# idiap/IdiapTTS

Measured on AMD Instinct MI355X. Metric: acoustic frames/sec (train), higher is better.
Workload: dtype f32

## Files before the change

### idiaptts_amd/csrc/context.h

```cpp
#pragma once
#include <cstdint>
#include <map>
#include <tuple>

#include "common.h"

namespace itts {

struct FreqtTables {
  double* fwdT = nullptr;
  double* invT = nullptr;
  double* frqT = nullptr;
  double* specT = nullptr;
  double* crT = nullptr;
  double* specP = nullptr;
  double* crP = nullptr;
  double* initP = nullptr;
  int kpad = 0;
  double* initT = nullptr;
  double* b1T = nullptr;
  double* p2T = nullptr;
  int m = 0, f2 = 0;
  double alpha = 0;
};

constexpr int RNG_CHUNK = 64;
constexpr int RNG_NJUMP = 26;
constexpr int RNG_TABLE_LOG2 = 20;
struct JumpTable {
  uint32_t col[RNG_NJUMP][128][4];
  uint4* states;
};

__device__ __forceinline__ uint4 rng_chunk_state(const JumpTable* __restrict__ jt, int64_t chunk) {
  uint4 st = jt->states[chunk & ((1 << RNG_TABLE_LOG2) - 1)];
  for (int k = RNG_TABLE_LOG2; k < RNG_NJUMP; ++k) {
    if ((chunk >> k) & 1) {
      const uint32_t s[4] = {st.x, st.y, st.z, st.w};
      uint32_t r0 = 0, r1 = 0, r2 = 0, r3 = 0;
      for (int j = 0; j < 128; ++j) {
        if ((s[j >> 5] >> (j & 31)) & 1u) {
          r0 ^= jt->col[k][j][0];
          r1 ^= jt->col[k][j][1];
          r2 ^= jt->col[k][j][2];
          r3 ^= jt->col[k][j][3];
        }
      }
      st = make_uint4(r0, r1, r2, r3);
    }
  }
  return st;
}

struct DeviceContext {
  int device = -1;
  double2* twiddles = nullptr;
  double2* tw_compact[16] = {nullptr};
  JumpTable* jump = nullptr;
  int64_t* pinned = nullptr;
  std::map<std::tuple<int, int, long long>, FreqtTables> freqt;
};

DeviceContext* get_context();
const FreqtTables* get_freqt(DeviceContext* ctx, int m, int f2, double alpha, bool need_fwd_frq,
                             bool need_mgc = false, bool need_spec = false);

int launch_gemm_f64_mgc2sp(const double* A, int64_t lda, const double* B, int64_t ldb, int64_t T, int N, int K,
                           float* o32, double* o64, double* opow, hipStream_t s);

const JumpTable* get_jump_table(DeviceContext* ctx);
int launch_randn_u32(DeviceContext* ctx, const int64_t* d_off, const int64_t* d_len, int n_utts,
                     int64_t max_len, uint32_t* d_R, hipStream_t s);

int launch_gemm_f64(const double* A, int64_t lda, const double* B, int64_t ldb, double* C, int64_t ldc,
                    int64_t T, int N, int K, const int* rows, hipStream_t s, bool a_has_slack = true);

int64_t* pinned_slot(DeviceContext* ctx);

int staged_upload(void* d_dst, const void* src, size_t bytes, hipStream_t s);

struct PinnedTable {
  void* p = nullptr;
  void* slot = nullptr;
};
int pinned_table_begin(const void* src, size_t bytes, PinnedTable* t);
int pinned_table_end(PinnedTable* t, hipStream_t s);

int upload_i64(const int64_t* h, int n, int64_t** d_out, hipStream_t s);

}
```

### idiaptts_amd/csrc/context.hip

```cpp
#include <cstdlib>

#include "context.h"

#include <algorithm>
#include <atomic>
#include <cmath>
#include <cstring>
#include <mutex>
#include <vector>

#include "world_dev.h"

namespace itts {

static std::mutex g_ctx_mutex;
static std::map<int, DeviceContext*> g_contexts;

static int create_context(DeviceContext* ctx) {
  const int n = wd::TW_N / 2;
  std::vector<double2> tw(n);
  for (int k = 0; k < n; ++k) {
    const long double a = 2.0L * 3.141592653589793238462643383279502884L * k / wd::TW_N;
    tw[k] = make_double2((double)cosl(a), (double)sinl(a));
  }
  ITTS_HIP_CHECK(hipMalloc((void**)&ctx->twiddles, n * sizeof(double2)));
  ITTS_HIP_CHECK(hipMemcpy(ctx->twiddles, tw.data(), n * sizeof(double2), hipMemcpyHostToDevice));
  for (int L = 5; (1 << L) <= wd::TW_N; ++L) {
    const int m = (1 << L) / 2, stride = wd::TW_N / (1 << L);
    std::vector<double2> c(m);
    for (int k = 0; k < m; ++k) c[k] = tw[(size_t)k * stride];
    ITTS_HIP_CHECK(hipMalloc((void**)&ctx->tw_compact[L], m * sizeof(double2)));
    ITTS_HIP_CHECK(hipMemcpy(ctx->tw_compact[L], c.data(), m * sizeof(double2), hipMemcpyHostToDevice));
  }
  ITTS_HIP_CHECK(hipHostMalloc((void**)&ctx->pinned, 64 * sizeof(int64_t), hipHostMallocDefault));
  return ITTS_OK;
}


}


namespace itts {

struct ScratchBlock {
  void* p;
  size_t bytes;
  hipEvent_t ev;
  hipStream_t last;
  bool busy;
};
struct ScratchCache {
  std::vector<ScratchBlock> blocks;
  size_t total = 0;
};
static std::mutex g_scratch_mutex;
static std::map<int, ScratchCache> g_scratch;

static size_t scratch_class(size_t n) {
  if (n <= ((size_t)1 << 20)) {
    size_t c = 256;
    while (c < n) c <<= 1;
    return c;
  }
  const size_t g = (size_t)2 << 20;
  return (n + g - 1) / g * g;
}

static size_t scratch_keep_bytes() {
  static const size_t keep = [] {
    size_t gb = 64;
    if (const char* e = getenv("ITTS_POOL_KEEP_GB")) gb = strtoull(e, nullptr, 10);
    return gb << 30;
  }();
  return keep;
}

static void scratch_evict(ScratchCache& c, size_t limit) {
  while (c.total > limit) {
    int pick = -1;
    for (int i = 0; i < (int)c.blocks.size(); ++i)
      if (!c.blocks[i].busy && (pick < 0 || c.blocks[i].bytes > c.blocks[pick].bytes)) pick = i;
    if (pick < 0) return;
    ScratchBlock b = c.blocks[pick];
    (void)hipEventSynchronize(b.ev);
    (void)hipFree(b.p);
    (void)hipEventDestroy(b.ev);
    c.total -= b.bytes;
    c.blocks.erase(c.blocks.begin() + pick);
  }
}

static thread_local ScratchScope* t_scope = nullptr;

ScratchScope::ScratchScope(hipStream_t s) : stream_(s), prev_(t_scope) { t_scope = this; }
ScratchScope::~ScratchScope() {
  t_scope = prev_;
  for (int i = 0; i < n_live_; ++i)
    if (live_[i]) (void)scratch_free(live_[i], stream_);
}
void ScratchScope::track(void* p) {
  if (n_live_ < 64) live_[n_live_++] = p;
}
void ScratchScope::untrack(void* p) {
  for (int i = n_live_ - 1; i >= 0; --i)
    if (live_[i] == p) {
      live_[i] = nullptr;
      while (n_live_ > 0 && live_[n_live_ - 1] == nullptr) --n_live_;
      return;
    }
  if (prev_) prev_->untrack(p);
}

static hipError_t scratch_malloc_impl(void** out, size_t bytes, hipStream_t s);
hipError_t scratch_malloc(void** out, size_t bytes, hipStream_t s) {
  const hipError_t e = scratch_malloc_impl(out, bytes, s);
  if (e == hipSuccess && *out && t_scope) t_scope->track(*out);
  return e;
}

static hipError_t scratch_malloc_impl(void** out, size_t bytes, hipStream_t s) {
  *out = nullptr;
  int dev = -1;
  hipError_t e = hipGetDevice(&dev);
  if (e != hipSuccess) return e;
  const size_t want = scratch_class(bytes);
  std::lock_guard<std::mutex> lock(g_scratch_mutex);
  ScratchCache& c = g_scratch[dev];
  int best = -1;
  for (int i = 0; i < (int)c.blocks.size(); ++i) {
    const ScratchBlock& b = c.blocks[i];
    if (b.busy || b.bytes < want) continue;
    if (want <= ((size_t)1 << 20) ? b.bytes != want : b.bytes > want + want / 4 + ((size_t)4 << 20)) continue;
    if (best < 0 || b.bytes < c.blocks[best].bytes) best = i;
  }
  if (best >= 0) {
    ScratchBlock& b = c.blocks[best];
    if (b.last != s && (e = hipStreamWaitEvent(s, b.ev, 0)) != hipSuccess) return e;
    b.busy = true;
    *out = b.p;
    return hipSuccess;
  }
  void* p = nullptr;
  e = hipMalloc(&p, want);
  if (e != hipSuccess) {
    (void)hipGetLastError();
    scratch_evict(c, 0);
    if ((e = hipMalloc(&p, want)) != hipSuccess) return e;
  }
  hipEvent_t ev;
  if ((e = hipEventCreateWithFlags(&ev, hipEventDisableTiming)) != hipSuccess) {
    (void)hipFree(p);
    return e;
  }
  c.blocks.push_back(ScratchBlock{p, want, ev, s, true});
  c.total += want;
  if (c.total > scratch_keep_bytes()) scratch_evict(c, scratch_keep_bytes());
  *out = p;
  return hipSuccess;
}

hipError_t scratch_free(void* p, hipStream_t s) {
  if (!p) return hipSuccess;
  if (t_scope) t_scope->untrack(p);
  std::lock_guard<std::mutex> lock(g_scratch_mutex);
  for (auto& kv : g_scratch)
    for (ScratchBlock& b : kv.second.blocks)
      if (b.p == p) {
        const hipError_t e = hipEventRecord(b.ev, s);
        b.last = s;
        b.busy = false;
        return e;
      }
  return hipErrorInvalidValue;
}

}

extern "C" int itts_scratch_pool_stats(int64_t* reserved, int64_t* used, int64_t* keep_threshold) {
  int dev = -1;
  ITTS_HIP_CHECK(hipGetDevice(&dev));
  size_t r = 0, u = 0;
  {
    std::lock_guard<std::mutex> lock(itts::g_scratch_mutex);
    auto it = itts::g_scratch.find(dev);
    if (it != itts::g_scratch.end())
      for (const itts::ScratchBlock& b : it->second.blocks) {
        r += b.bytes;
        if (b.busy) u += b.bytes;
      }
  }
  if (reserved) *reserved = (int64_t)r;
  if (used) *used = (int64_t)u;
  if (keep_threshold) *keep_threshold = (int64_t)itts::scratch_keep_bytes();
  return ITTS_OK;
}

extern "C" int itts_release_scratch(void) {
  int dev = -1;
  ITTS_HIP_CHECK(hipGetDevice(&dev));
  ITTS_HIP_CHECK(hipDeviceSynchronize());
  {
    std::lock_guard<std::mutex> lock(itts::g_scratch_mutex);
    auto it = itts::g_scratch.find(dev);
    if (it != itts::g_scratch.end()) itts::scratch_evict(it->second, 0);
  }
  return ITTS_OK;
}

namespace itts {

int64_t* pinned_slot(DeviceContext* ctx) {
  static std::atomic<unsigned> next{0};
  return ctx->pinned + (next.fetch_add(1) & 63u);
}

DeviceContext* get_context() {
  int dev = -1;
  if (hipGetDevice(&dev) != hipSuccess) {
    set_error("hipGetDevice failed: no HIP device (there is no CPU fallback)");
    return nullptr;
  }
  std::lock_guard<std::mutex> lock(g_ctx_mutex);
  auto it = g_contexts.find(dev);
  if (it != g_contexts.end()) return it->second;
  DeviceContext* ctx = new DeviceContext();
  ctx->device = dev;
  if (create_context(ctx) != ITTS_OK) {
    delete ctx;
    return nullptr;
  }
  g_contexts[dev] = ctx;
  return ctx;
}

struct Mat128 {
  uint32_t col[128][4];
};
static void mat_apply(const Mat128& m, const uint32_t* v, uint32_t* out) {
  uint32_t r[4] = {0, 0, 0, 0};
  for (int j = 0; j < 128; ++j)
    if ((v[j >> 5] >> (j & 31)) & 1u)
      for (int c = 0; c < 4; ++c) r[c] ^= m.col[j][c];
  std::memcpy(out, r, sizeof(r));
}
static void mat_mul(const Mat128& a, const Mat128& b, Mat128* out) {
  Mat128 r;
  for (int j = 0; j < 128; ++j) mat_apply(a, b.col[j], r.col[j]);
  *out = r;
}

__global__ __launch_bounds__(256) void rng_states_kernel(const JumpTable* __restrict__ jt) {
  const int chunk = blockIdx.x * 256 + threadIdx.x;
  uint32_t s[4] = {123456789u, 362436069u, 521288629u, 88675123u};
  for (int k = 0; k < RNG_TABLE_LOG2; ++k) {
    if ((chunk >> k) & 1) {
      uint32_t r0 = 0, r1 = 0, r2 = 0, r3 = 0;
      for (int j = 0; j < 128; ++j) {
        if ((s[j >> 5] >> (j & 31)) & 1u) {
          r0 ^= jt->col[k][j][0];
          r1 ^= jt->col[k][j][1];
          r2 ^= jt->col[k][j][2];
          r3 ^= jt->col[k][j][3];
        }
      }
      s[0] = r0; s[1] = r1; s[2] = r2; s[3] = r3;
    }
  }
  jt->states[chunk] = make_uint4(s[0], s[1], s[2], s[3]);
}

const JumpTable* get_jump_table(DeviceContext* ctx) {
  std::lock_guard<std::mutex> lock(g_ctx_mutex);
  if (ctx->jump) return ctx->jump;
  Mat128 step;
  for (int j = 0; j < 128; ++j) {
    uint32_t s[4] = {0, 0, 0, 0};
    s[j >> 5] = 1u << (j & 31);
    uint32_t x = s[0], y = s[1], z = s[2], w = s[3];
    const uint32_t t = x ^ (x << 11);
    x = y; y = z; z = w;
    w = (w ^ (w >> 19)) ^ (t ^ (t >> 8));
    step.col[j][0] = x; step.col[j][1] = y; step.col[j][2] = z; step.col[j][3] = w;
  }
  Mat128 B, pw = step;
  bool have = false;
  for (int e = 12 * RNG_CHUNK; e > 0; e >>= 1) {
    if (e & 1) {
      if (!have) { B = pw; have = true; } else mat_mul(pw, B, &B);
    }
    mat_mul(pw, pw, &pw);
  }
  std::vector<JumpTable> jt(1);
  Mat128 cur = B;
  for (int k = 0; k < RNG_NJUMP; ++k) {
    std::memcpy(jt[0].col[k], cur.col, sizeof(cur.col));
    mat_mul(cur, cur, &cur);
  }
  JumpTable* d = nullptr;
  uint4* states = nullptr;
  const int n_states = 1 << RNG_TABLE_LOG2;
  if (hipMalloc((void**)&states, sizeof(uint4) * n_states) != hipSuccess ||
      hipMalloc((void**)&d, sizeof(JumpTable)) != hipSuccess) {
    set_error("could not create the RNG jump table");
    return nullptr;
  }
  jt[0].states = states;
  if (hipMemcpy(d, jt.data(), sizeof(JumpTable), hipMemcpyHostToDevice) != hipSuccess) {
    set_error("could not create the RNG jump table");
    return nullptr;
  }
  hipLaunchKernelGGL(rng_states_kernel, dim3(n_states / 256), dim3(256), 0, 0, d);
  if (hipGetLastError() != hipSuccess || hipStreamSynchronize(0) != hipSuccess) {
    set_error("could not tabulate the RNG states");
    return nullptr;
  }
  ctx->jump = d;
  return d;
}

__global__ __launch_bounds__(256) void randn_u32_direct_kernel(const int64_t* __restrict__ off,
                                                               const int64_t* __restrict__ len,
                                                               const JumpTable* __restrict__ jt,
                                                               uint32_t* __restrict__ R) {
  const int u = blockIdx.y;
  const int64_t chunk = (int64_t)blockIdx.x * 256 + threadIdx.x;
  const int64_t n0 = chunk * RNG_CHUNK;
  const int64_t n = len[u];
  if (n0 >= n) return;
  const uint4 st = rng_chunk_state(jt, chunk);
  uint32_t x = st.x, y = st.y, z = st.z, w = st.w;
  uint32_t* out = R + off[u] + n0;
  const int cnt = (int)(n - n0 < RNG_CHUNK ? n - n0 : RNG_CHUNK);
  for (int i = 0; i < cnt; ++i) {
    uint32_t tmp = 0;
    for (int q = 0; q < 12; ++q) {
      const uint32_t t = x ^ (x << 11);
      x = y; y = z; z = w;
      w = (w ^ (w >> 19)) ^ (t ^ (t >> 8));
      tmp += w >> 4;
    }
    out[i] = tmp;
  }
}

__global__ __launch_bounds__(256) void randn_u32_kernel(const int64_t* __restrict__ off,
                                                        const int64_t* __restrict__ len,
                                                        const JumpTable* __restrict__ jt,
                                                        uint32_t* __restrict__ R) {
  constexpr int HALF = RNG_CHUNK / 2;
  __shared__ uint32_t tile[4][64 * (HALF + 1)];
  const int u = blockIdx.y;
  const int lane = threadIdx.x & 63, wv = threadIdx.x >> 6;
  const int64_t chunk0 = (int64_t)blockIdx.x * 256 + wv * 64;
  const int64_t n = len[u];
  if ((int64_t)blockIdx.x * 256 * RNG_CHUNK >= n) return;
  const int64_t chunk = chunk0 + lane;
  const bool live = chunk * RNG_CHUNK < n;
  uint32_t x = 0, y = 0, z = 0, w = 0;
  if (live) {
    const uint4 st = rng_chunk_state(jt, chunk);
    x = st.x; y = st.y; z = st.z; w = st.w;
  }
  uint32_t* t = tile[wv];
  uint32_t* out = R + off[u] + chunk0 * RNG_CHUNK;
  const int64_t rem = n - chunk0 * RNG_CHUNK;
  for (int h = 0; h < 2; ++h) {
    if (live) {
#pragma unroll 4
      for (int i = 0; i < HALF; ++i) {
        uint32_t tmp = 0;
        for (int q = 0; q < 12; ++q) {
          const uint32_t s = x ^ (x << 11);
          x = y; y = z; z = w;
          w = (w ^ (w >> 19)) ^ (s ^ (s >> 8));
          tmp += w >> 4;
        }
        t[lane * (HALF + 1) + i] = tmp;
      }
    }
    __syncthreads();
    const int col = lane & (HALF - 1), sub = lane / HALF;
    for (int r = 0; r < 64; r += 64 / HALF) {
      const int row = r + sub;
      const int64_t idx = (int64_t)row * RNG_CHUNK + h * HALF + col;
      if (idx < rem) out[idx] = t[row * (HALF + 1) + col];
    }
    __syncthreads();
  }
}

int launch_randn_u32(DeviceContext* ctx, const int64_t* d_off, const int64_t* d_len, int n_utts,
                     int64_t max_len, uint32_t* d_R, hipStream_t s) {
  const JumpTable* jt = get_jump_table(ctx);
  if (!jt) return ITTS_E_HIP;
  ITTS_REQUIRE(max_len < ((int64_t)RNG_CHUNK << RNG_NJUMP), "utterance too long for the RNG jump table");
  if (n_utts == 0 || max_len <= 0) return ITTS_OK;
  const int64_t chunks = (max_len + RNG_CHUNK - 1) / RNG_CHUNK;
  const char* direct = std::getenv("ITTS_RANDN_DIRECT");
  const dim3 grid((unsigned)((chunks + 255) / 256), n_utts);
  if (direct && direct[0] == '1')
    hipLaunchKernelGGL(randn_u32_direct_kernel, grid, dim3(256), 0, s, d_off, d_len, jt, d_R);
  else
    hipLaunchKernelGGL(randn_u32_kernel, grid, dim3(256), 0, s, d_off, d_len, jt, d_R);
  ITTS_LAUNCH_CHECK();
  return ITTS_OK;
}

static void freqt_unit(int idx, int m2, double a, double* g, double* d) {
  const double b = 1.0 - a * a;
  std::memset(g, 0, sizeof(double) * (m2 + 1));
  std::memset(d, 0, sizeof(double) * (m2 + 1));
  for (int i = -idx; i <= 0; ++i) {
    const double cin = (i == -idx) ? 1.0 : 0.0;
    d[0] = g[0];
    g[0] = cin + a * d[0];
    if (m2 >= 1) {
      d[1] = g[1];
      g[1] = b * d[0] + a * d[1];
    }
    for (int j = 2; j <= m2; ++j) {
      d[j] = g[j];
      g[j] = d[j - 1] + a * (d[j] - g[j - 1]);
    }
  }
}

static void frqtr_unit(int idx, int m2, double a, double* g, double* d) {
  std::memset(g, 0, sizeof(double) * (m2 + 1));
  std::memset(d, 0, sizeof(double) * (m2 + 1));
  for (int i = -idx; i <= 0; ++i) {
    const double cin = (i == -idx) ? 1.0 : 0.0;
    d[0] = g[0];
    g[0] = cin;
    for (int j = 1; j <= m2; ++j) {
      d[j] = g[j];
      g[j] = d[j - 1] + a * (d[j] - g[j - 1]);
    }
  }
}

static void b2c_unit(int idx, int m2, double a, double* g, double* d) {
  const double k = 1.0 - a * a;
  std::memset(g, 0, sizeof(double) * (m2 + 1));
  std::memset(d, 0, sizeof(double) * (m2 + 1));
  for (int i = -idx; i <= 0; ++i) {
    const double cin = (i == -idx) ? 1.0 : 0.0;
    d[0] = g[0];
    g[0] = cin;
    if (m2 >= 1) {
      d[1] = g[1];
      g[1] = k * d[0] + a * d[1];
    }
    for (int j = 2; j <= m2; ++j) {
      d[j] = g[j];
      g[j] = d[j - 1] + a * (d[j] - g[j - 1]);
    }
  }
}

static int upload(const std::vector<double>& h, double** d) {
  ITTS_HIP_CHECK(hipMalloc((void**)d, h.size() * sizeof(double)));
  ITTS_HIP_CHECK(hipMemcpy(*d, h.data(), h.size() * sizeof(double), hipMemcpyHostToDevice));
  return ITTS_OK;
}

const FreqtTables* get_freqt(DeviceContext* ctx, int m, int f2, double alpha, bool need_fwd_frq,
                             bool need_mgc, bool need_spec) {
  long long abits;
  std::memcpy(&abits, &alpha, sizeof(abits));
  const auto key = std::make_tuple(m, f2, abits);
  std::lock_guard<std::mutex> lock(g_ctx_mutex);
  FreqtTables& t = ctx->freqt[key];
  t.m = m;
  t.f2 = f2;
  t.alpha = alpha;
  const int m2 = 2 * m;
  std::vector<double> g(std::max(f2, m2) + 2), d(std::max(f2, m2) + 2);
  if (!t.invT) {
    std::vector<double> inv((size_t)(m + 1) * (f2 + 1));
    for (int j = 0; j <= m; ++j) {
      freqt_unit(j, f2, -alpha, g.data(), d.data());
      for (int i = 0; i <= f2; ++i) inv[(size_t)j * (f2 + 1) + i] = g[i];
    }
    if (upload(inv, &t.invT) != ITTS_OK) return nullptr;
  }
  if (need_fwd_frq && !t.fwdT) {
    std::vector<double> fwd((size_t)(f2 + 1) * (m + 1)), frq((size_t)(f2 + 1) * (m2 + 1));
    for (int i = 0; i <= f2; ++i) {
      freqt_unit(i, m, alpha, g.data(), d.data());
      for (int j = 0; j <= m; ++j) fwd[(size_t)i * (m + 1) + j] = g[j];
      frqtr_unit(i, m2, alpha, g.data(), d.data());
      for (int j = 0; j <= m2; ++j) frq[(size_t)i * (m2 + 1) + j] = g[j];
    }
    if (upload(fwd, &t.fwdT) != ITTS_OK) return nullptr;
    if (upload(frq, &t.frqT) != ITTS_OK) return nullptr;
    const int nfft = 2 * f2;
    std::vector<long double> cs(nfft);
    for (int i = 0; i < nfft; ++i) cs[i] = cosl(2.0L * 3.14159265358979323846264338327950288L * i / nfft);
    std::vector<double> crt((size_t)(f2 + 1) * (m2 + 1));
    std::vector<long double> accj(m2 + 1);
    for (int k = 0; k <= f2; ++k) {
      const long double wk = (k == 0 || k == f2) ? 1.0L : 2.0L;
      std::fill(accj.begin(), accj.end(), 0.0L);
      for (int n = 0; n <= f2; ++n) {
        const long double c = cs[(size_t)((int64_t)k * n % nfft)];
        const double* fr = frq.data() + (size_t)n * (m2 + 1);
        for (int j = 0; j <= m2; ++j) accj[j] += c * (long double)fr[j];
      }
      for (int j = 0; j <= m2; ++j) crt[(size_t)k * (m2 + 1) + j] = (double)(accj[j] * wk / nfft);
    }
    if (upload(crt, &t.crT) != ITTS_OK) return nullptr;
    if (m <= 63) {
      t.kpad = (f2 + 1 + 63) / 64 * 64;
      std::vector<double> crp((size_t)t.kpad * 128, 0.0);
      for (int k = 0; k <= f2; ++k)
        for (int j = 0; j <= m2; ++j) crp[(size_t)k * 128 + j] = crt[(size_t)k * (m2 + 1) + j];
      if (upload(crp, &t.crP) != ITTS_OK) return nullptr;
    }
    std::vector<double> ini((size_t)(f2 + 1) * (m + 1));
    std::vector<long double> accm(m + 1);
    for (int k = 0; k <= f2; ++k) {
      const long double wk = (k == 0 || k == f2) ? 1.0L : 2.0L;
      std::fill(accm.begin(), accm.end(), 0.0L);
      for (int n = 0; n <= f2; ++n) {
        const long double c = cs[(size_t)((int64_t)k * n % nfft)] * ((n == 0 || n == f2) ? 0.5L : 1.0L);
        const double* fw = fwd.data() + (size_t)n * (m + 1);
        for (int j = 0; j <= m; ++j) accm[j] += c * (long double)fw[j];
      }
      for (int j = 0; j <= m; ++j) ini[(size_t)k * (m + 1) + j] = (double)(accm[j] * wk / nfft);
    }
    if (upload(ini, &t.initT) != ITTS_OK) return nullptr;
    if (m <= 63) {
      const int kpad = (f2 + 1 + 63) / 64 * 64;
      std::vector<double> ip((size_t)kpad * 64, 0.0);
      for (int k = 0; k <= f2; ++k)
// ... 162 lines not shown
```

### idiaptts_amd/csrc/nn.hip

```cpp
#include <algorithm>
#include <atomic>
#include <cstdlib>

#include "common.h"
#include "gemm_ring.h"
#include "gemm_staged.h"

namespace itts {

constexpr int BN = 128;

template <bool ROWFORM, bool VEC, int NROWS>
__device__ __forceinline__ void load_tile(const float* __restrict__ P, int64_t ld, int64_t out0,
                                          int64_t out_dim, int64_t k0, int64_t k_end,
                                          float4 (&r)[NROWS / 32]) {
  const int tid = threadIdx.x;
#pragma unroll
  for (int i = 0; i < NROWS / 32; ++i) {
    const int idx = tid + 256 * i;
    int64_t o, k;
    if (ROWFORM) {
      o = out0 + (idx >> 3);
      k = k0 + ((idx & 7) << 2);
    } else {
      k = k0 + idx / (NROWS / 4);
      o = out0 + ((idx % (NROWS / 4)) << 2);
    }
    const int64_t c = ROWFORM ? k : o, c_end = ROWFORM ? k_end : out_dim;
    const int64_t t = ROWFORM ? o : k, t_end = ROWFORM ? out_dim : k_end;
    const bool t_ok = t < t_end;
    const int64_t tc = t_ok ? t : 0;
    if (VEC) {
      const bool ok = t_ok && (c < c_end);
      const float4 v = *reinterpret_cast<const float4*>(P + tc * ld + (ok ? c : 0));
      r[i] = ok ? v : make_float4(0.f, 0.f, 0.f, 0.f);
    } else {
      const float* row = P + tc * ld;
      const bool k0ok = t_ok && c < c_end, k1ok = t_ok && c + 1 < c_end, k2ok = t_ok && c + 2 < c_end,
                 k3ok = t_ok && c + 3 < c_end;
      const float a0 = row[k0ok ? c : 0], a1 = row[k1ok ? c + 1 : 0], a2 = row[k2ok ? c + 2 : 0],
                  a3 = row[k3ok ? c + 3 : 0];
      r[i] = make_float4(k0ok ? a0 : 0.f, k1ok ? a1 : 0.f, k2ok ? a2 : 0.f, k3ok ? a3 : 0.f);
    }
  }
}

template <bool A_ROW, bool B_ROW, bool VEC_A, bool VEC_B>
struct DenseLoader {
  const GemmArgs& g;
  template <int NROWS>
  __device__ __forceinline__ void load_a(int64_t out0, int64_t k0, int64_t k_end, float4 (&r)[NROWS / 32]) const {
    load_tile<A_ROW, VEC_A, NROWS>(g.A, g.lda, out0, g.M, k0, k_end, r);
  }
  template <int NROWS>
  __device__ __forceinline__ void load_b(int64_t out0, int64_t k0, int64_t k_end, float4 (&r)[NROWS / 32]) const {
    load_tile<B_ROW, VEC_B, NROWS>(g.B, g.ldb, out0, g.N, k0, k_end, r);
  }
};

template <bool A_ROW, bool B_ROW, int EPI, bool VEC_A, bool VEC_B, int TN, int STAGES = 2, int AF = AF_BASE>
__global__ __launch_bounds__(256, STAGES == 1 ? 4 : 2) void gemm_f32_kernel(GemmArgs g) {
  __shared__ __attribute__((aligned(16))) float lds[staged_lds_floats<B_ROW, TN, STAGES>()];
  f32x16 acc[2][TN];
  const StagedTile t =
      staged_gemm_tile<A_ROW, B_ROW, TN, STAGES>(g, DenseLoader<A_ROW, B_ROW, VEC_A, VEC_B>{g}, lds, acc);
  const int64_t m0 = t.m0;
  const int n0 = t.n0;
  const int lane = threadIdx.x & 63, wid = threadIdx.x >> 6;
  const int wm = wid >> 1, wn = wid & 1;
  float* C = g.C + (int64_t)blockIdx.z * g.slab_stride;
  const int cl = lane & 31, rh = lane >> 5;
  if (EPI == EPI_MSE) {
    float* stage = lds + wid * (32 * 36);
    const int c4 = (lane & 7) << 2, rq = lane >> 3;
    const int colb = n0 + wn * 32;
    double lsum = 0.0;
#pragma unroll
    for (int i = 0; i < 2; ++i) {
      if (i > 0) {
        __builtin_amdgcn_fence(__ATOMIC_RELEASE, "wavefront");
        __builtin_amdgcn_wave_barrier();
      }
#pragma unroll
      for (int r = 0; r < 16; ++r) stage[((r & 3) + 8 * (r >> 2) + 4 * rh) * 36 + cl] = acc[i][0][r];
      __builtin_amdgcn_fence(__ATOMIC_RELEASE, "wavefront");
      __builtin_amdgcn_wave_barrier();
      __builtin_amdgcn_fence(__ATOMIC_ACQUIRE, "wavefront");
      const int col = colb + c4;
#pragma unroll
      for (int q = 0; q < 4; ++q) {
        const int rl = rq + 8 * q;
        const int64_t row = m0 + wm * 64 + i * 32 + rl;
        const float4 v = *reinterpret_cast<const float4*>(stage + rl * 36 + c4);
        if (row >= g.M || col >= g.N) continue;
        const bool ok = g.row_valid[row] != 0;
        const float vv[4] = {v.x, v.y, v.z, v.w};
        float dz[4];
#pragma unroll
        for (int e = 0; e < 4; ++e) {
          float diff = 0.f;
          if (col + e < g.N && ok)
            diff = (vv[e] + (g.bias ? g.bias[col + e] : 0.f)) - g.aux[row * g.ldaux + col + e];
          lsum += (double)diff * (double)diff;
          dz[e] = g.gscale * diff;
        }
        if (col + 3 < g.N) {
          *reinterpret_cast<float4*>(C + row * g.ldc + col) = make_float4(dz[0], dz[1], dz[2], dz[3]);
        } else {
          for (int e = 0; e < 4 && col + e < g.N; ++e) C[row * g.ldc + col + e] = dz[e];
        }
      }
    }
    __shared__ double mse_red[16];
    lsum = block_sum(lsum, mse_red);
    if (threadIdx.x == 0) g.loss_partial[blockIdx.x] = lsum;
    return;
  }
  if (STAGES == 1 && TN == 1 && g.wide_out) {
    float* stage = lds + wid * (32 * 36);
    const int c4 = (lane & 7) << 2, rq = lane >> 3;
    const int colb = n0 + wn * 32;
#pragma unroll
    for (int i = 0; i < 2; ++i) {
      if (i > 0) {
        __builtin_amdgcn_fence(__ATOMIC_RELEASE, "wavefront");
        __builtin_amdgcn_wave_barrier();
      }
#pragma unroll
      for (int r = 0; r < 16; ++r) stage[((r & 3) + 8 * (r >> 2) + 4 * rh) * 36 + cl] = acc[i][0][r];
      __builtin_amdgcn_fence(__ATOMIC_RELEASE, "wavefront");
      __builtin_amdgcn_wave_barrier();
      __builtin_amdgcn_fence(__ATOMIC_ACQUIRE, "wavefront");
      const int col = colb + c4;
      float4 bv = make_float4(0.f, 0.f, 0.f, 0.f);
      const bool full = col + 3 < g.N;
      if (EPI == EPI_BIAS_ACT && g.bias && full) bv = *reinterpret_cast<const float4*>(g.bias + col);
#pragma unroll
      for (int q = 0; q < 4; ++q) {
        const int rl = rq + 8 * q;
        const int64_t row = m0 + wm * 64 + i * 32 + rl;
        float4 v = *reinterpret_cast<const float4*>(stage + rl * 36 + c4);
        if (row >= g.M || col >= g.N) continue;
        if (full) {
          if (EPI == EPI_BIAS_ACT) {
            v.x = act_fwd_af<AF>(v.x + bv.x, g.act); v.y = act_fwd_af<AF>(v.y + bv.y, g.act);
            v.z = act_fwd_af<AF>(v.z + bv.z, g.act); v.w = act_fwd_af<AF>(v.w + bv.w, g.act);
          }
          if (EPI == EPI_DACT) {
            const float4 a = *reinterpret_cast<const float4*>(g.aux + row * g.ldaux + col);
            v.x *= act_grad_af<AF>(a.x, g.act); v.y *= act_grad_af<AF>(a.y, g.act);
            v.z *= act_grad_af<AF>(a.z, g.act); v.w *= act_grad_af<AF>(a.w, g.act);
          }
          *reinterpret_cast<float4*>(C + row * g.ldc + col) = v;
        } else {
          const float vv[4] = {v.x, v.y, v.z, v.w};
          for (int e = 0; e < 4 && col + e < g.N; ++e) {
            float o = vv[e];
            if (EPI == EPI_BIAS_ACT) o = act_fwd_af<AF>(o + (g.bias ? g.bias[col + e] : 0.f), g.act);
            if (EPI == EPI_DACT) o *= act_grad_af<AF>(g.aux[row * g.ldaux + col + e], g.act);
            C[row * g.ldc + col + e] = o;
          }
        }
      }
    }
    return;
  }
  staged_epilogue<EPI, TN, AF>(g, t, acc, [](int64_t m) { return m; });
}

static std::atomic<int64_t> g_gemm_path[2][4];

template <bool A_ROW, bool B_ROW, int EPI, int TN, int STAGES, int AF = AF_BASE>
static int launch_gemm_tn(const GemmArgs& g, int splitk, hipStream_t s) {
  g_gemm_path[1][EPI].fetch_add(1, std::memory_order_relaxed);
  const int64_t tiles = ((g.M + BM - 1) / BM) * ((g.N + 64 * TN - 1) / (64 * TN));
  dim3 grid((unsigned)tiles, 1, (unsigned)splitk);
  const bool va = g.vecA, vb = g.vecB;
  if (va && vb)
    hipLaunchKernelGGL((gemm_f32_kernel<A_ROW, B_ROW, EPI, true, true, TN, STAGES, AF>), grid, dim3(256), 0, s, g);
  else if (va)
    hipLaunchKernelGGL((gemm_f32_kernel<A_ROW, B_ROW, EPI, true, false, TN, STAGES, AF>), grid, dim3(256), 0, s, g);
  else if (vb)
    hipLaunchKernelGGL((gemm_f32_kernel<A_ROW, B_ROW, EPI, false, true, TN, STAGES, AF>), grid, dim3(256), 0, s, g);
  else
    hipLaunchKernelGGL((gemm_f32_kernel<A_ROW, B_ROW, EPI, false, false, TN, STAGES, AF>), grid, dim3(256), 0, s, g);
  ITTS_LAUNCH_CHECK();
  return ITTS_OK;
}

static double tile_efficiency(int64_t M, int N, int splitk, int tn, double loop_eff) {
  const int bn = 64 * tn;
  const int64_t tiles = ((M + BM - 1) / BM) * ((N + bn - 1) / bn) * splitk;
  const int64_t rounds = (tiles + 511) / 512;
  const double useful = (double)N / (double)(((N + bn - 1) / bn) * bn);
  return loop_eff * useful * (double)tiles / (double)(rounds * 512);
}

constexpr int kRingGrid = 512;

template <bool A_ROW, bool B_ROW>
static bool ring_ok(const GemmArgs& g, int splitk, int epi) {
  if (!g.vecA || !g.vecB) return false;
  if (g.lda % 4 || g.ldb % 4 || g.ldc % 4 || g.slab_stride % 4 || !aligned16(g.C)) return false;
  if (epi == EPI_DACT && (g.ldaux % 4 || !aligned16(g.aux))) return false;
  const int64_t lim = (int64_t)1 << 30;
  if (g.M >= lim || g.K >= lim || g.lda >= lim / 256 || g.ldb >= lim / 256 || g.ldc >= lim / 256 ||
      g.ldaux >= lim / 256)
    return false;
  if (!A_ROW && (g.kchunk + 32) * g.lda >= lim) return false;
  if (!B_ROW && (g.kchunk + 32) * g.ldb >= lim) return false;
  if (splitk > 1 && g.kchunk % 32) return false;
  return true;
}

static int ring_group(int tiles_n, int bnt, int64_t K, bool row_row);

template <int WM>
static ring::Args ring_args(const GemmArgs& g, int splitk) {
  constexpr int BMT = 64 * WM, BNT = 32 * (4 / WM);
  ring::Args r{};
  r.A = g.A; r.B = g.B; r.C = g.C; r.bias = g.bias; r.aux = g.aux;
  r.row_valid = g.row_valid; r.loss_partial = g.loss_partial; r.bias_part = g.bias_part;
  r.slab_stride = g.slab_stride; r.bias_part_stride = g.bias_part_stride;
  r.lda = (int)g.lda; r.ldb = (int)g.ldb; r.ldc = (int)g.ldc; r.ldaux = (int)g.ldaux;
  r.M = (int)g.M; r.N = g.N; r.K = (int)g.K; r.kchunk = (int)g.kchunk; r.splitk = splitk;
  r.tiles_m = (int)((g.M + BMT - 1) / BMT);
  r.tiles_n = (g.N + BNT - 1) / BNT;
  r.gn = r.tiles_n;
  r.act = g.act; r.gscale = g.gscale;
  return r;
}

template <bool A_ROW, bool B_ROW, int EPI, int WM, int AF = AF_BASE>
static int launch_ring_wm(const GemmArgs& g, int splitk, hipStream_t s) {
  constexpr int BNT = 32 * (4 / WM);
  g_gemm_path[0][EPI].fetch_add(1, std::memory_order_relaxed);
  ring::Args r = ring_args<WM>(g, splitk);
  r.gn = ring_group(r.tiles_n, BNT, g.K, A_ROW && B_ROW);
  const int64_t ntiles = (int64_t)r.tiles_m * r.tiles_n * splitk;
  ITTS_REQUIRE(ntiles < ((int64_t)1 << 31), "too many tiles");
  const int grid = (int)std::min<int64_t>(kRingGrid, (ntiles + 7) / 8 * 8);
  if (A_ROW && B_ROW && EPI == ring::EPI_BIAS_ACT && r.gn < r.tiles_n)
    hipLaunchKernelGGL((ring::gemm_ring_kernel<A_ROW, B_ROW, EPI, WM, A_ROW && B_ROW && EPI == ring::EPI_BIAS_ACT, AF>),
                       dim3(grid), dim3(ring::THREADS), 0, s, r);
  else
    hipLaunchKernelGGL((ring::gemm_ring_kernel<A_ROW, B_ROW, EPI, WM, false, AF>), dim3(grid), dim3(ring::THREADS), 0, s, r);
  ITTS_LAUNCH_CHECK();
  return ITTS_OK;
}

static int ring_group(int tiles_n, int bnt, int64_t K, bool row_row) {
  if (!row_row) return tiles_n;
  const int64_t panel = (int64_t)bnt * K * 4;
  const int64_t gn = std::max<int64_t>(1, ((int64_t)4 << 20) / std::max<int64_t>(panel, 1));
  return (int)std::min<int64_t>(gn, tiles_n);
}

static int ring_wm(int64_t M, int N) {
  const double w2 = (double)(((M + 127) / 128) * 128) * (double)(((N + 63) / 64) * 64);
  const double w1 = (double)(((M + 63) / 64) * 64) * (double)(((N + 127) / 128) * 128);
  return w1 < w2 ? 1 : 2;
}

template <bool A_ROW, bool B_ROW, int EPI, int AF>
static int launch_ring(const GemmArgs& g, int splitk, hipStream_t s) {
  if (ring_wm(g.M, g.N) == 1) return launch_ring_wm<A_ROW, B_ROW, EPI, 1, AF>(g, splitk, s);
  return launch_ring_wm<A_ROW, B_ROW, EPI, 2, AF>(g, splitk, s);
}

template <int WM_W, int EPI_X, int AF_X = AF_BASE>
static int launch_ring_bwd_pair(const GemmArgs& gw, int splitk, const GemmArgs& gx, hipStream_t s) {
  g_gemm_path[0][EPI_STORE].fetch_add(1, std::memory_order_relaxed);
  g_gemm_path[0][EPI_X].fetch_add(1, std::memory_order_relaxed);
  const ring::Args rw = ring_args<WM_W>(gw, splitk), rx = ring_args<2>(gx, 1);
  hipLaunchKernelGGL((ring::gemm_ring_pair_kernel<false, false, EPI_STORE, WM_W, true, false, EPI_X, 2, AF_X>),
                     dim3(kRingGrid), dim3(ring::THREADS), 0, s, rw, rx);
  ITTS_LAUNCH_CHECK();
  return ITTS_OK;
}

template <bool A_ROW, bool B_ROW, int EPI, int AF = AF_BASE>
static int launch_gemm(GemmArgs g, int splitk, hipStream_t s) {
  if (g.M <= 0 || g.N <= 0) return ITTS_OK;
  if (ring_ok<A_ROW, B_ROW>(g, splitk, EPI)) return launch_ring<A_ROW, B_ROW, EPI, AF>(g, splitk, s);
  if (A_ROW) return launch_gemm_tn<A_ROW, B_ROW, EPI, 1, 1, AF>(g, splitk, s);
  const double e2 = tile_efficiency(g.M, g.N, splitk, 2, 1.0);
  const double e1 = tile_efficiency(g.M, g.N, splitk, 1, 0.90);
  if (e1 > e2) return launch_gemm_tn<A_ROW, B_ROW, EPI, 1, 2, AF>(g, splitk, s);
  return launch_gemm_tn<A_ROW, B_ROW, EPI, 2, 2, AF>(g, splitk, s);
}


__device__ __forceinline__ void reduce_slabs_vec_body(const float* __restrict__ slabs, int S, int64_t n,
                                                      float* __restrict__ out, int accumulate, int64_t block,
                                                      float4 (*part)[64]) {
  const int tx = threadIdx.x & 63, grp = threadIdx.x >> 6;
  const int64_t n4 = n >> 2;
  const int64_t c = block * 64 + tx;
  float4 s = make_float4(0.f, 0.f, 0.f, 0.f);
  if (c < n4) {
    const float4* p = reinterpret_cast<const float4*>(slabs) + c;
#pragma unroll 8
    for (int z = grp; z < S; z += 4) {
      const float4 v = p[(int64_t)z * n4];
      s.x += v.x; s.y += v.y; s.z += v.z; s.w += v.w;
    }
  }
  if (grp > 0) part[grp - 1][tx] = s;
  __syncthreads();
  if (grp == 0 && c < n4) {
#pragma unroll
    for (int g2 = 0; g2 < 3; ++g2) {
      const float4 v = part[g2][tx];
      s.x += v.x; s.y += v.y; s.z += v.z; s.w += v.w;
    }
    float4* o = reinterpret_cast<float4*>(out) + c;
    if (accumulate) {
      const float4 v = *o;
      s.x += v.x; s.y += v.y; s.z += v.z; s.w += v.w;
    }
    *o = s;
  }
}

__device__ __forceinline__ void reduce_slabs_scalar_body(const float* __restrict__ slabs, int S, int64_t n,
                                                         float* __restrict__ out, int accumulate,
                                                         int64_t block, float (*part)[64]) {
  const int tx = threadIdx.x & 63, grp = threadIdx.x >> 6;
  const int64_t c = block * 64 + tx;
  float s = 0.f;
  if (c < n) {
#pragma unroll 8
    for (int z = grp; z < S; z += 4) s += slabs[(int64_t)z * n + c];
  }
  if (grp > 0) part[grp - 1][tx] = s;
  __syncthreads();
  if (grp == 0 && c < n) {
    s += part[0][tx];
    s += part[1][tx];
    s += part[2][tx];
    out[c] = accumulate ? out[c] + s : s;
  }
}

__global__ __launch_bounds__(256) void reduce_slabs_kernel(const float* __restrict__ slabs, int S,
                                                           int64_t n, float* __restrict__ out,
                                                           int accumulate) {
  __shared__ float4 part[3][64];
  reduce_slabs_vec_body(slabs, S, n, out, accumulate, blockIdx.x, part);
}

__global__ __launch_bounds__(256) void reduce_slabs_scalar_kernel(const float* __restrict__ slabs, int S,
                                                                  int64_t n, float* __restrict__ out,
                                                                  int accumulate) {
  __shared__ float part[3][64];
  reduce_slabs_scalar_body(slabs, S, n, out, accumulate, blockIdx.x, part);
}

constexpr int kMaxDeferred = 16;
struct ReduceSeg {
  const void* src;
  void* out;
  int64_t n;
  double scale;
  int S;
  int accumulate;
  int kind;
  int first_block;
};
struct ReduceMulti {
  ReduceSeg seg[kMaxDeferred];
  int nseg;
};

__global__ __launch_bounds__(256) void reduce_multi_kernel(ReduceMulti d) {
  __shared__ float4 part4[3][64];
  __shared__ double red[16];
  int i = 0;
  while (i + 1 < d.nseg && (int)blockIdx.x >= d.seg[i + 1].first_block) ++i;
  const ReduceSeg& g = d.seg[i];
  const int64_t block = (int64_t)blockIdx.x - g.first_block;
  if (g.kind == 0) {
    reduce_slabs_vec_body(static_cast<const float*>(g.src), g.S, g.n, static_cast<float*>(g.out), g.accumulate,
                          block, part4);
  } else if (g.kind == 1) {
    reduce_slabs_scalar_body(static_cast<const float*>(g.src), g.S, g.n, static_cast<float*>(g.out),
                             g.accumulate, block, reinterpret_cast<float (*)[64]>(part4));
  } else {
    const double* partial = static_cast<const double*>(g.src);
    double s = 0.0;
    for (int k = threadIdx.x; k < (int)g.n; k += 256) s += partial[k];
    s = block_sum(s, red);
    if (threadIdx.x == 0) *static_cast<float*>(g.out) = (float)(s * g.scale);
  }
}

static thread_local bool t_defer = false;
static thread_local ReduceMulti t_pending{};

static int flush_deferred(hipStream_t s) {
  if (t_pending.nseg == 0) return ITTS_OK;
  const ReduceSeg& last = t_pending.seg[t_pending.nseg - 1];
  const int64_t per = last.kind == 0 ? (last.n / 4 + 63) / 64 : (last.kind == 1 ? (last.n + 63) / 64 : 1);
  const int64_t blocks = last.first_block + per;
  hipLaunchKernelGGL(reduce_multi_kernel, dim3((unsigned)blocks), dim3(256), 0, s, t_pending);
  t_pending.nseg = 0;
  ITTS_LAUNCH_CHECK();
  return ITTS_OK;
}

static int queue_deferred(ReduceSeg g, hipStream_t s) {
  if (t_pending.nseg == kMaxDeferred) {
    const int rc = flush_deferred(s);
    if (rc) return rc;
  }
  int64_t first = 0;
  if (t_pending.nseg > 0) {
    const ReduceSeg& p = t_pending.seg[t_pending.nseg - 1];
    first = p.first_block + (p.kind == 0 ? (p.n / 4 + 63) / 64 : (p.kind == 1 ? (p.n + 63) / 64 : 1));
  }
  ITTS_REQUIRE(first < ((int64_t)1 << 30), "too many deferred reduction blocks");
  g.first_block = (int)first;
  t_pending.seg[t_pending.nseg++] = g;
  return ITTS_OK;
}

static int launch_reduce_slabs(const float* slabs, int S, int64_t n, float* out, int accumulate,
                               hipStream_t s) {
  const bool vec = n % 4 == 0 && aligned16(slabs) && aligned16(out);
  if (t_defer) {
    ReduceSeg g{};
    g.src = slabs; g.out = out; g.n = n; g.S = S; g.accumulate = accumulate; g.kind = vec ? 0 : 1;
    return queue_deferred(g, s);
  }
  if (vec)
    hipLaunchKernelGGL(reduce_slabs_kernel, dim3((unsigned)((n / 4 + 63) / 64)), dim3(256), 0, s, slabs, S,
                       n, out, accumulate);
  else
    hipLaunchKernelGGL(reduce_slabs_scalar_kernel, dim3((unsigned)((n + 63) / 64)), dim3(256), 0, s, slabs,
                       S, n, out, accumulate);
  ITTS_LAUNCH_CHECK();
  return ITTS_OK;
}

extern "C" int itts_defer_reductions(int on) {
  ITTS_REQUIRE(on || t_pending.nseg == 0,
               "queued reductions must be run (itts_reduce_deferred) before deferral is switched off");
  t_defer = on != 0;
  return ITTS_OK;
}

extern "C" int itts_reduce_deferred(void* stream) {
  t_defer = false;
  return flush_deferred(as_stream(stream));
}

template <int AF>
__global__ void act_bwd_kernel(const float* __restrict__ dy, const float* __restrict__ y,
                               float* __restrict__ dz, int64_t n, int act) {
  if (AF == AF_BASE) {
    for (int64_t i = blockIdx.x * (int64_t)blockDim.x + threadIdx.x; i < n;
         i += (int64_t)gridDim.x * blockDim.x)
      dz[i] = dy[i] * act_grad_from_out(y[i], act);
  } else {
    with_ext_act(act, [&](auto a) {
      for (int64_t i = blockIdx.x * (int64_t)blockDim.x + threadIdx.x; i < n;
           i += (int64_t)gridDim.x * blockDim.x)
        dz[i] = dy[i] * dact1<decltype(a)::value>(y[i]);
    });
  }
}

__global__ __launch_bounds__(256) void masked_mse_kernel(
    const float* __restrict__ pred, int64_t ldp, const float* __restrict__ target, int64_t ldt,
    const uint8_t* __restrict__ valid, int64_t M, int D, float gscale, float* __restrict__ grad,
    int64_t ldg, double* __restrict__ partial) {
  __shared__ double red[16];
  const int64_t n = M * D;
  double s = 0.0;
  for (int64_t i = blockIdx.x * (int64_t)blockDim.x + threadIdx.x; i < n;
       i += (int64_t)gridDim.x * blockDim.x) {
    const int64_t r = i / D;
    const int c = (int)(i - r * D);
    float diff = 0.f;
    if (valid[r]) diff = pred[r * ldp + c] - target[r * ldt + c];
    s += (double)diff * (double)diff;
    if (grad) grad[r * ldg + c] = gscale * diff;
  }
  s = block_sum(s, red);
  if (threadIdx.x == 0) partial[blockIdx.x] = s;
}

__global__ __launch_bounds__(256) void masked_mse_final_kernel(const double* __restrict__ partial,
                                                               int nb, double scale,
                                                               float* __restrict__ loss) {
  __shared__ double red[16];
  double s = 0.0;
  for (int i = threadIdx.x; i < nb; i += 256) s += partial[i];
  s = block_sum(s, red);
  if (threadIdx.x == 0) *loss = (float)(s * scale);
}

static int launch_mse_final(const double* partial, int nb, double scale, float* loss, hipStream_t s) {
  if (t_defer) {
    ReduceSeg g{};
    g.src = partial; g.out = loss; g.n = nb; g.scale = scale; g.S = 1; g.kind = 2;
    return queue_deferred(g, s);
  }
  hipLaunchKernelGGL(masked_mse_final_kernel, dim3(1), dim3(256), 0, s, partial, nb, scale, loss);
  ITTS_LAUNCH_CHECK();
  return ITTS_OK;
}


__global__ __launch_bounds__(256) void weighted_loss_kernel(
    const float* __restrict__ pred, int64_t ldp, const float* __restrict__ target, int64_t ldt,
    const float* __restrict__ w, int64_t M, int D, int kind, float* __restrict__ grad, int64_t ldg,
    float* __restrict__ elem, int64_t lde, double* __restrict__ partial) {
  __shared__ double red[16];
  const int64_t n = M * D;
  double s = 0.0;
  for (int64_t i = blockIdx.x * (int64_t)blockDim.x + threadIdx.x; i < n;
       i += (int64_t)gridDim.x * blockDim.x) {
    const int64_t r = i / D;
    const int c = (int)(i - r * D);
    const float wr = w[r];
    const float diff = pred[r * ldp + c] - target[r * ldt + c];
    const float e = kind == 0 ? diff * diff : fabsf(diff);
    const float g = kind == 0 ? 2.f * diff : (diff > 0.f ? 1.f : (diff < 0.f ? -1.f : 0.f));
    const float v = wr == 0.f ? 0.f : wr * e;
    s += (double)v;
    if (grad) grad[r * ldg + c] = wr == 0.f ? 0.f : wr * g;
    if (elem) elem[r * lde + c] = v;
  }
  s = block_sum(s, red);
  if (threadIdx.x == 0) partial[blockIdx.x] = s;
}

__global__ void adam_kernel(float* __restrict__ p, const float* __restrict__ g,
                            float* __restrict__ m, float* __restrict__ v, int64_t n, float beta1,
                            float beta2, float eps, float wd, float step_size, float bc2_sqrt,
                            float gscale) {
  for (int64_t i = blockIdx.x * (int64_t)blockDim.x + threadIdx.x; i < n;
       i += (int64_t)gridDim.x * blockDim.x) {
    float gi = g[i] * gscale;
    float pi = p[i];
    if (wd != 0.f) gi += wd * pi;
    float mi = m[i], vi = v[i];
    mi = mi + (gi - mi) * (1.f - beta1);
    vi = vi * beta2 + (1.f - beta2) * gi * gi;
    const float denom = sqrtf(vi) / bc2_sqrt + eps;
    pi = pi - step_size * (mi / denom);
    p[i] = pi;
    m[i] = mi;
    v[i] = vi;
  }
}

__global__ void adam_fused_kernel(float* __restrict__ p, const float* __restrict__ g,
                                  float* __restrict__ m, float* __restrict__ v, int64_t n,
                                  float beta1, float beta2, float eps, float wd, float step_size,
                                  float bc2_sqrt, float gscale, const float* __restrict__ norm_accum,
                                  int norm_kind, float max_norm, float clip_value,
                                  float* __restrict__ shadow, float one_minus_decay) {
  float coef = gscale;
  if (norm_accum) {
    const float a = norm_accum[0];
    const float total = (norm_kind == 2 ? sqrtf(a) : a) * fabsf(gscale);
    coef *= fminf(1.f, max_norm / (total + 1e-6f));
  }
  for (int64_t i = blockIdx.x * (int64_t)blockDim.x + threadIdx.x; i < n;
       i += (int64_t)gridDim.x * blockDim.x) {
    float gi = g[i] * coef;
    if (clip_value > 0.f) gi = fminf(fmaxf(gi, -clip_value), clip_value);
    float pi = p[i];
    if (wd != 0.f) gi += wd * pi;
    float mi = m[i], vi = v[i];
    mi = mi + (gi - mi) * (1.f - beta1);
    vi = vi * beta2 + (1.f - beta2) * gi * gi;
    const float denom = sqrtf(vi) / bc2_sqrt + eps;
    pi = pi - step_size * (mi / denom);
    p[i] = pi;
    m[i] = mi;
    v[i] = vi;
    if (shadow) {
      const float si = shadow[i];
      shadow[i] = si - one_minus_decay * (si - pi);
    }
  }
}

constexpr int kNormBlocks = 1024;
__global__ __launch_bounds__(256) void grad_norm_partial_kernel(const float* __restrict__ x, int64_t n,
                                                               int kind, float* __restrict__ part) {
  __shared__ float red[4];
  float acc = 0.f;
  for (int64_t i = blockIdx.x * (int64_t)blockDim.x + threadIdx.x; i < n;
       i += (int64_t)gridDim.x * blockDim.x) {
    const float xi = x[i];
    acc = kind == 2 ? acc + xi * xi : fmaxf(acc, fabsf(xi));
  }
#pragma unroll
  for (int off = 32; off > 0; off >>= 1) {
    const float o = __shfl_xor(acc, off, 64);
    acc = kind == 2 ? acc + o : fmaxf(acc, o);
  }
  if ((threadIdx.x & 63) == 0) red[threadIdx.x >> 6] = acc;
  __syncthreads();
  if (threadIdx.x == 0)
    part[blockIdx.x] = kind == 2 ? (red[0] + red[1]) + (red[2] + red[3])
                                 : fmaxf(fmaxf(red[0], red[1]), fmaxf(red[2], red[3]));
}
__global__ __launch_bounds__(256) void grad_norm_final_kernel(const float* __restrict__ part, int nb,
                                                             int kind, float* __restrict__ out,
                                                             int accumulate) {
  __shared__ float red[4];
  float acc = 0.f;
  for (int i = threadIdx.x; i < nb; i += 256) acc = kind == 2 ? acc + part[i] : fmaxf(acc, part[i]);
#pragma unroll
  for (int off = 32; off > 0; off >>= 1) {
    const float o = __shfl_xor(acc, off, 64);
    acc = kind == 2 ? acc + o : fmaxf(acc, o);
  }
  if ((threadIdx.x & 63) == 0) red[threadIdx.x >> 6] = acc;
  __syncthreads();
  if (threadIdx.x == 0) {
    float r = kind == 2 ? (red[0] + red[1]) + (red[2] + red[3])
                        : fmaxf(fmaxf(red[0], red[1]), fmaxf(red[2], red[3]));
    if (accumulate) r = kind == 2 ? out[0] + r : fmaxf(out[0], r);
    out[0] = r;
  }
}

__global__ void sgd_kernel(float* __restrict__ p, const float* __restrict__ g,
                           float* __restrict__ buf, int64_t n, float lr, float momentum,
                           float dampening, float wd, int nesterov, int first, float gscale) {
  for (int64_t i = blockIdx.x * (int64_t)blockDim.x + threadIdx.x; i < n;
       i += (int64_t)gridDim.x * blockDim.x) {
    float gi = g[i] * gscale;
    float pi = p[i];
    if (wd != 0.f) gi += wd * pi;
    if (momentum != 0.f) {
      float bi = first ? gi : buf[i] * momentum + (1.f - dampening) * gi;
      buf[i] = bi;
      gi = nesterov ? gi + momentum * bi : bi;
    }
    p[i] = pi - lr * gi;
  }
}

__global__ void ema_kernel(float* __restrict__ shadow, const float* __restrict__ x, int64_t n,
                           float one_minus_decay) {
  for (int64_t i = blockIdx.x * (int64_t)blockDim.x + threadIdx.x; i < n;
       i += (int64_t)gridDim.x * blockDim.x) {
    const float sh = shadow[i];
    shadow[i] = sh - one_minus_decay * (sh - x[i]);
  }
}

constexpr int kColsumSlices = 256;

static int choose_splitk_ring(int64_t M, int N, int K) {
  const int wm = ring_wm(N, K);
  const int bmt = 64 * wm, bnt = 32 * (4 / wm);
  const int64_t tiles = (int64_t)((N + bmt - 1) / bmt) * ((K + bnt - 1) / bnt);
  int64_t s = std::max<int64_t>(1, kRingGrid / std::max<int64_t>(tiles, 1));
  s = std::min<int64_t>(s, std::max<int64_t>(1, (M + 255) / 256));
  return (int)std::min<int64_t>(s, 128);
}

static int choose_splitk(int64_t M, int N, int K) {
  const int64_t tiles = (int64_t)((N + BM - 1) / BM) * ((K + BN - 1) / BN);
  int64_t s = std::max<int64_t>(1, 512 / std::max<int64_t>(tiles, 1));
  const int64_t max_by_rows = std::max<int64_t>(1, (M + 511) / 512);
  s = std::min(s, max_by_rows);
  return (int)std::min<int64_t>(s, 128);
}

}

using namespace itts;

extern "C" int itts_linear_fwd(const float* d_x, int64_t ldx, const float* d_w, const float* d_b,
                               float* d_y, int64_t ldy, int64_t M, int N, int K, int act,
                               void* stream) {
  ITTS_REQUIRE(d_w && (M == 0 || (d_x && d_y)), "null pointer");
  ITTS_REQUIRE(M >= 0 && N > 0 && K > 0 && ldx >= K && ldy >= N, "bad sizes");
  ITTS_REQUIRE(act >= ITTS_ACT_NONE && act <= ITTS_ACT_HARDSIGMOID, "unknown activation");
  if (M == 0) return ITTS_OK;
  GemmArgs g{};
  g.A = d_x; g.lda = ldx; g.B = d_w; g.ldb = K; g.C = d_y; g.ldc = ldy;
  g.M = M; g.N = N; g.K = K; g.bias = d_b; g.act = act;
  g.kchunk = ((K + BK - 1) / BK) * BK; g.slab_stride = 0;
  g.vecA = (ldx % 4 == 0) && aligned16(d_x);
  g.vecB = (K % 4 == 0) && aligned16(d_w);
  g.wide_out = (ldy % 4 == 0) && aligned16(d_y) && (!d_b || aligned16(d_b));
  if (act_family(act) == AF_EXT) return launch_gemm<true, true, EPI_BIAS_ACT, AF_EXT>(g, 1, as_stream(stream));
  return launch_gemm<true, true, EPI_BIAS_ACT>(g, 1, as_stream(stream));
}

__global__ __launch_bounds__(256) void rows_gather_kernel(const float* __restrict__ src, int64_t ld_src, int64_t n_src,
                                                          const int64_t* __restrict__ idx, int64_t n_out, int width,
                                                          const float* __restrict__ fill, float* __restrict__ dst,
                                                          int64_t ld_dst, int dst_width, int vec) {
  const int lane = threadIdx.x & 63;
  const int64_t w0 = (int64_t)blockIdx.x * 4 + (threadIdx.x >> 6), wn = (int64_t)gridDim.x * 4;
  for (int64_t r = w0; r < n_out; r += wn) {
    const int64_t i = idx[r];
    const float* s = (i >= 0 && i < n_src) ? src + i * ld_src : fill;
    float* d = dst + r * ld_dst;
    if (vec) {
      const int w4 = width >> 2, d4 = dst_width >> 2;
      for (int c = lane; c < d4; c += 64) {
        float4 v = make_float4(0.f, 0.f, 0.f, 0.f);
        if (c < w4 && s) v = reinterpret_cast<const float4*>(s)[c];
        reinterpret_cast<float4*>(d)[c] = v;
      }
    } else {
      for (int c = lane; c < dst_width; c += 64) d[c] = (c < width && s) ? s[c] : 0.f;
    }
  }
}

extern "C" int itts_rows_gather_f32(const float* d_src, int64_t ld_src, int64_t n_src, const int64_t* d_idx,
                                    int64_t n_out, int width, const float* d_fill_row, float* d_dst, int64_t ld_dst,
                                    int dst_width, void* stream) {
  ITTS_REQUIRE(n_out == 0 || (d_idx && d_dst && (d_src || n_src == 0)), "null pointer");
  ITTS_REQUIRE(n_out >= 0 && n_src >= 0 && width >= 0 && dst_width >= width && ld_src >= width && ld_dst >= dst_width,
               "bad sizes");
  if (n_out == 0 || dst_width == 0) return ITTS_OK;
  const int vec = width % 4 == 0 && dst_width % 4 == 0 && ld_src % 4 == 0 && ld_dst % 4 == 0 && aligned16(d_src) &&
                  aligned16(d_dst) && (!d_fill_row || aligned16(d_fill_row));
  const unsigned grid = (unsigned)std::min<int64_t>((n_out + 3) / 4, 16384);
  hipLaunchKernelGGL(rows_gather_kernel, dim3(grid), dim3(256), 0, as_stream(stream), d_src, ld_src, n_src, d_idx, n_out,
                     width, d_fill_row, d_dst, ld_dst, dst_width, vec);
  ITTS_LAUNCH_CHECK();
  return ITTS_OK;
}

extern "C" int itts_gemm_path_counts(int64_t out[8]) {
  ITTS_REQUIRE(out != nullptr, "null pointer");
  for (int k = 0; k < 2; ++k)
    for (int e = 0; e < 4; ++e) out[4 * k + e] = g_gemm_path[k][e].load(std::memory_order_relaxed);
  return ITTS_OK;
}

extern "C" int64_t itts_linear_fwd_mse_workspace_bytes(int64_t M, int N) {
  const int64_t tiles = ((M + BM - 1) / BM) * ((N + 63) / 64);
  return std::max<int64_t>(tiles, kRingGrid) * 8;
}

extern "C" int itts_linear_fwd_mse(const float* d_x, int64_t ldx, const float* d_w, const float* d_b,
                                   const float* d_target, int64_t ldt, const uint8_t* d_row_valid,
                                   double n_valid, float loss_weight, int64_t M, int N, int K,
                                   float* d_loss, float* d_dz, int64_t lddz, void* d_workspace,
                                   void* stream) {
  ITTS_REQUIRE(d_w && d_loss && d_workspace && (M == 0 || (d_x && d_target && d_row_valid && d_dz)),
               "null pointer");
  ITTS_REQUIRE(M >= 0 && N > 0 && K > 0 && ldx >= K && ldt >= N && lddz >= N && n_valid > 0, "bad sizes");
  hipStream_t s = as_stream(stream);
  if (M == 0) {
    ITTS_HIP_CHECK(hipMemsetAsync(d_loss, 0, 4, s));
    return ITTS_OK;
  }
  ITTS_REQUIRE((ldx % 4 == 0) && aligned16(d_x) && (K % 4 == 0) && aligned16(d_w) && (lddz % 4 == 0) &&
                   aligned16(d_dz),
               "x, w and dz need 16-byte aligned rows (use itts_linear_fwd + itts_masked_mse otherwise)");
  GemmArgs g{};
  g.A = d_x; g.lda = ldx; g.B = d_w; g.ldb = K; g.C = d_dz; g.ldc = lddz;
  g.M = M; g.N = N; g.K = K; g.bias = d_b; g.act = 0;
  g.kchunk = ((K + BK - 1) / BK) * BK; g.slab_stride = 0;
  g.vecA = 1; g.vecB = 1; g.wide_out = 1;
  g.aux = d_target; g.ldaux = ldt; g.row_valid = d_row_valid;
  const double scale = (double)loss_weight / (n_valid * (double)N);
  g.gscale = (float)(2.0 * scale);
  g.loss_partial = reinterpret_cast<double*>(d_workspace);
  int64_t tiles = ((M + BM - 1) / BM) * ((N + 63) / 64);
  int rc;
  if (ring_ok<true, true>(g, 1, EPI_MSE)) {
    tiles = std::min<int64_t>(kRingGrid, (tiles + 7) / 8 * 8);
    rc = launch_ring_wm<true, true, EPI_MSE, 2>(g, 1, s);
  } else {
    rc = launch_gemm_tn<true, true, EPI_MSE, 1, 1>(g, 1, s);
  }
  if (rc) return rc;
  return launch_mse_final(reinterpret_cast<const double*>(d_workspace), (int)tiles, scale, d_loss, s);
}

extern "C" int itts_act_bwd(const float* d_dy, const float* d_y, float* d_dz, int64_t n_elem,
                            int act, void* stream) {
  ITTS_REQUIRE(d_dy && d_y && d_dz && n_elem >= 0, "bad arguments");
  ITTS_REQUIRE(act >= ITTS_ACT_NONE && act <= ITTS_ACT_HARDSIGMOID, "unknown activation");
  if (n_elem == 0) return ITTS_OK;
  const int blocks = (int)std::min<int64_t>((n_elem + 255) / 256, 4096);
  if (act_family(act) == AF_EXT)
    hipLaunchKernelGGL(act_bwd_kernel<AF_EXT>, dim3(blocks), dim3(256), 0, as_stream(stream), d_dy, d_y,
                       d_dz, n_elem, act);
  else
    hipLaunchKernelGGL(act_bwd_kernel<AF_BASE>, dim3(blocks), dim3(256), 0, as_stream(stream), d_dy, d_y,
                       d_dz, n_elem, act);
  ITTS_LAUNCH_CHECK();
  return ITTS_OK;
}

extern "C" int itts_linear_bwd_input(const float* d_dz, int64_t lddz, const float* d_w,
                                     float* d_dx, int64_t lddx, const float* d_yprev,
                                     int64_t ldyp, int act_prev, int64_t M, int N, int K,
                                     void* stream) {
  ITTS_REQUIRE(d_w && (M == 0 || (d_dz && d_dx)), "null pointer");
  ITTS_REQUIRE(M >= 0 && N > 0 && K > 0 && lddz >= N && lddx >= K, "bad sizes");
  ITTS_REQUIRE(!d_yprev || (act_prev >= ITTS_ACT_NONE && act_prev <= ITTS_ACT_HARDSIGMOID), "unknown activation");
  if (M == 0) return ITTS_OK;
  GemmArgs g{};
  g.A = d_dz; g.lda = lddz; g.B = d_w; g.ldb = K; g.C = d_dx; g.ldc = lddx;
  g.M = M; g.N = K; g.K = N; g.aux = d_yprev; g.ldaux = ldyp; g.act = act_prev;
  g.kchunk = ((N + BK - 1) / BK) * BK; g.slab_stride = 0;
  g.vecA = (lddz % 4 == 0) && aligned16(d_dz);
  g.vecB = (K % 4 == 0) && aligned16(d_w);
  g.wide_out = (lddx % 4 == 0) && aligned16(d_dx) && (!d_yprev || ((ldyp % 4 == 0) && aligned16(d_yprev)));
  if (d_yprev) {
    ITTS_REQUIRE(ldyp >= K, "ldyp too small");
    if (act_family(act_prev) == AF_EXT) return launch_gemm<true, false, EPI_DACT, AF_EXT>(g, 1, as_stream(stream));
    return launch_gemm<true, false, EPI_DACT>(g, 1, as_stream(stream));
  }
  return launch_gemm<true, false, EPI_STORE>(g, 1, as_stream(stream));
}

extern "C" int64_t itts_linear_bwd_weight_workspace_bytes(int64_t M, int N, int K) {
  if (M < 0 || N <= 0 || K <= 0) return 0;
  const int s = std::max(choose_splitk(M, N, K), choose_splitk_ring(M, N, K));
  return (int64_t)s * ((int64_t)N * K + N) * 4 + (int64_t)kColsumSlices * N * 4 + 8192;
}

extern "C" int itts_linear_bwd_weight(const float* d_dz, int64_t lddz, const float* d_x,
                                      int64_t ldx, float* d_dw, float* d_db, int64_t M, int N,
                                      int K, void* d_workspace, int accumulate, void* stream) {
  ITTS_REQUIRE(d_dw && d_workspace && (M == 0 || (d_dz && d_x)), "null pointer");
  ITTS_REQUIRE(M >= 0 && N > 0 && K > 0 && lddz >= N && ldx >= K, "bad sizes");
  hipStream_t s = as_stream(stream);
  if (M == 0) {
    if (!accumulate) {
      ITTS_HIP_CHECK(hipMemsetAsync(d_dw, 0, (size_t)N * K * 4, s));
      if (d_db) ITTS_HIP_CHECK(hipMemsetAsync(d_db, 0, (size_t)N * 4, s));
    }
    return ITTS_OK;
  }
  const bool vec_ok = (lddz % 4 == 0) && aligned16(d_dz) && (ldx % 4 == 0) && aligned16(d_x) && (K % 4 == 0);
  const int S = vec_ok ? choose_splitk_ring(M, N, K) : choose_splitk(M, N, K);
  int64_t kchunk = (M + S - 1) / S;
  kchunk = ((kchunk + BK - 1) / BK) * BK;
  const int S_eff = (int)((M + kchunk - 1) / kchunk);
  float* slabs = reinterpret_cast<float*>(d_workspace);
  GemmArgs g{};
  g.A = d_dz; g.lda = lddz; g.B = d_x; g.ldb = ldx; g.C = slabs; g.ldc = K;
  g.M = N; g.N = K; g.K = M; g.kchunk = kchunk; g.slab_stride = (int64_t)N * K;
  g.vecA = (lddz % 4 == 0) && aligned16(d_dz);
  g.vecB = (ldx % 4 == 0) && aligned16(d_x);
  const int64_t n = (int64_t)N * K;
  if (d_db) {
    const bool merged = d_db == d_dw + n && N % 4 == 0 && n % 4 == 0;
    const int64_t stride = merged ? n + N : n;
    g.slab_stride = stride;
    g.bias_part = merged ? slabs + n : slabs + (int64_t)S_eff * n;
    g.bias_part_stride = merged ? stride : N;
    int rc = launch_gemm<false, false, EPI_STORE>(g, S_eff, s);
    if (rc) return rc;
    if (merged) return launch_reduce_slabs(slabs, S_eff, n + N, d_dw, accumulate, s);
    rc = launch_reduce_slabs(slabs, S_eff, n, d_dw, accumulate, s);
    if (rc) return rc;
    return launch_reduce_slabs(g.bias_part, S_eff, (int64_t)N, d_db, accumulate, s);
  }
  int rc = launch_gemm<false, false, EPI_STORE>(g, S_eff, s);
  if (rc) return rc;
  return launch_reduce_slabs(slabs, S_eff, n, d_dw, accumulate, s);
}

extern "C" int itts_linear_bwd(const float* d_dz, int64_t lddz, const float* d_x, int64_t ldx,
                               const float* d_w, float* d_dw, float* d_db, float* d_dx, int64_t lddx,
                               const float* d_yprev, int64_t ldyp, int act_prev, int64_t M, int N, int K,
                               void* d_workspace, int accumulate, void* stream) {
  ITTS_REQUIRE(d_w && d_dw && d_workspace && (M == 0 || (d_dz && d_x && d_dx)), "null pointer");
  ITTS_REQUIRE(M >= 0 && N > 0 && K > 0 && lddz >= N && ldx >= K && lddx >= K, "bad sizes");
  ITTS_REQUIRE(!d_yprev || ldyp >= K, "ldyp too small");
  ITTS_REQUIRE(!d_yprev || (act_prev >= ITTS_ACT_NONE && act_prev <= ITTS_ACT_HARDSIGMOID), "unknown activation");
  hipStream_t s = as_stream(stream);
  const bool vec_ok = (lddz % 4 == 0) && aligned16(d_dz) && (ldx % 4 == 0) && aligned16(d_x) && (K % 4 == 0) &&
                      aligned16(d_w);
  const int64_t n = (int64_t)N * K;
  const bool merged = d_db && d_db == d_dw + n && N % 4 == 0 && n % 4 == 0;
  bool fused = vec_ok && M > 0 && (lddx % 4 == 0) && aligned16(d_dx) &&
               (!d_yprev || ((ldyp % 4 == 0) && aligned16(d_yprev)));
  GemmArgs gw{}, gx{};
  int S_eff = 1;
  if (fused) {
    const int S = choose_splitk_ring(M, N, K);
    int64_t kchunk = (M + S - 1) / S;
    kchunk = ((kchunk + BK - 1) / BK) * BK;
    S_eff = (int)((M + kchunk - 1) / kchunk);
    float* slabs = reinterpret_cast<float*>(d_workspace);
    gw.A = d_dz; gw.lda = lddz; gw.B = d_x; gw.ldb = ldx; gw.C = slabs; gw.ldc = K;
    gw.M = N; gw.N = K; gw.K = M; gw.kchunk = kchunk; gw.vecA = gw.vecB = 1;
    const int64_t stride = merged ? n + N : n;
    gw.slab_stride = stride;
    if (merged) { gw.bias_part = slabs + n; gw.bias_part_stride = stride; }
    else if (d_db) { gw.bias_part = slabs + (int64_t)S_eff * n; gw.bias_part_stride = N; }
    gx.A = d_dz; gx.lda = lddz; gx.B = d_w; gx.ldb = K; gx.C = d_dx; gx.ldc = lddx;
    gx.M = M; gx.N = K; gx.K = N; gx.aux = d_yprev; gx.ldaux = ldyp; gx.act = act_prev;
    gx.kchunk = ((N + BK - 1) / BK) * BK; gx.vecA = gx.vecB = 1;
    fused = ring_ok<false, false>(gw, S_eff, EPI_STORE) && ring_ok<true, false>(gx, 1, d_yprev ? EPI_DACT : EPI_STORE);
  }
  if (!fused) {
    int rc = itts_linear_bwd_weight(d_dz, lddz, d_x, ldx, d_dw, d_db, M, N, K, d_workspace, accumulate, stream);
    if (rc) return rc;
    return itts_linear_bwd_input(d_dz, lddz, d_w, d_dx, lddx, d_yprev, ldyp, act_prev, M, N, K, stream);
  }
  int rc;
  const int wm = ring_wm(gw.M, gw.N);
  if (d_yprev && act_family(act_prev) == AF_EXT)
    rc = wm == 1 ? launch_ring_bwd_pair<1, EPI_DACT, AF_EXT>(gw, S_eff, gx, s)
                 : launch_ring_bwd_pair<2, EPI_DACT, AF_EXT>(gw, S_eff, gx, s);
  else if (d_yprev) rc = wm == 1 ? launch_ring_bwd_pair<1, EPI_DACT>(gw, S_eff, gx, s) : launch_ring_bwd_pair<2, EPI_DACT>(gw, S_eff, gx, s);
  else rc = wm == 1 ? launch_ring_bwd_pair<1, EPI_STORE>(gw, S_eff, gx, s) : launch_ring_bwd_pair<2, EPI_STORE>(gw, S_eff, gx, s);
  if (rc) return rc;
  float* slabs = reinterpret_cast<float*>(d_workspace);
  rc = launch_reduce_slabs(slabs, S_eff, merged ? n + N : n, d_dw, accumulate, s);
  if (rc || merged || !d_db) return rc;
  return launch_reduce_slabs(slabs + (int64_t)S_eff * n, S_eff, (int64_t)N, d_db, accumulate, s);
}

static int mse_blocks(int64_t M, int D) {
  return (int)std::max<int64_t>(1, std::min<int64_t>((M * D + 255) / 256, 2048));
}

extern "C" int64_t itts_masked_mse_workspace_bytes(int64_t M, int D) {
  if (M < 0 || D <= 0) return 0;
  return (int64_t)mse_blocks(M, D) * 8;
}

extern "C" int itts_masked_mse(const float* d_pred, int64_t ldp, const float* d_target,
                               int64_t ldt, const uint8_t* d_row_valid, int64_t M, int D,
                               double n_valid, float loss_weight, float* d_loss, float* d_grad,
                               int64_t ldg, void* d_workspace, void* stream) {
  ITTS_REQUIRE(d_pred && d_target && d_row_valid && d_loss && d_workspace, "null pointer");
  ITTS_REQUIRE(M >= 0 && D > 0 && ldp >= D && ldt >= D && n_valid > 0, "bad sizes");
  ITTS_REQUIRE(!d_grad || ldg >= D, "ldg too small");
  hipStream_t s = as_stream(stream);
  if (M == 0) {
    ITTS_HIP_CHECK(hipMemsetAsync(d_loss, 0, 4, s));
    return ITTS_OK;
  }
  const int nb = mse_blocks(M, D);
  const double scale = (double)loss_weight / (n_valid * (double)D);
  hipLaunchKernelGGL(masked_mse_kernel, dim3(nb), dim3(256), 0, s, d_pred, ldp, d_target, ldt,
                     d_row_valid, M, D, (float)(2.0 * scale), d_grad, ldg,
                     reinterpret_cast<double*>(d_workspace));
  ITTS_LAUNCH_CHECK();
  return launch_mse_final(reinterpret_cast<const double*>(d_workspace), nb, scale, d_loss, s);
}

extern "C" int itts_weighted_loss(const float* d_pred, int64_t ldp, const float* d_target, int64_t ldt,
                                  const float* d_row_weight, int64_t M, int D, int kind,
                                  float* d_loss, float* d_grad, int64_t ldg, float* d_elem,
                                  int64_t lde, void* d_workspace, void* stream) {
  ITTS_REQUIRE(d_pred && d_target && d_row_weight && d_loss && d_workspace, "null pointer");
  ITTS_REQUIRE(M >= 0 && D > 0 && ldp >= D && ldt >= D && (kind == 0 || kind == 1), "bad sizes");
  ITTS_REQUIRE((!d_grad || ldg >= D) && (!d_elem || lde >= D), "leading dimension too small");
  hipStream_t s = as_stream(stream);
  if (M == 0) {
    ITTS_HIP_CHECK(hipMemsetAsync(d_loss, 0, 4, s));
    return ITTS_OK;
  }
  const int nb = mse_blocks(M, D);
  hipLaunchKernelGGL(weighted_loss_kernel, dim3(nb), dim3(256), 0, s, d_pred, ldp, d_target, ldt,
                     d_row_weight, M, D, kind, d_grad, ldg, d_elem, lde,
                     reinterpret_cast<double*>(d_workspace));
  ITTS_LAUNCH_CHECK();
  hipLaunchKernelGGL(masked_mse_final_kernel, dim3(1), dim3(256), 0, s,
                     reinterpret_cast<const double*>(d_workspace), nb, 1.0, d_loss);
  ITTS_LAUNCH_CHECK();
  return ITTS_OK;
}

extern "C" int itts_adam_step(float* d_param, const float* d_grad, float* d_exp_avg,
                              float* d_exp_avg_sq, int64_t n, float lr, float beta1, float beta2,
                              float eps, float weight_decay, int64_t step, float grad_scale,
                              void* stream) {
  ITTS_REQUIRE(d_param && d_grad && d_exp_avg && d_exp_avg_sq, "null pointer");
  ITTS_REQUIRE(n >= 0 && step >= 1, "bad sizes (step counts from 1)");
  if (n == 0) return ITTS_OK;
  const double bc1 = 1.0 - pow((double)beta1, (double)step);
  const double bc2 = 1.0 - pow((double)beta2, (double)step);
  const float step_size = (float)((double)lr / bc1);
  const float bc2_sqrt = (float)sqrt(bc2);
  const int blocks = (int)std::min<int64_t>((n + 255) / 256, 4096);
  hipLaunchKernelGGL(adam_kernel, dim3(blocks), dim3(256), 0, as_stream(stream), d_param, d_grad,
                     d_exp_avg, d_exp_avg_sq, n, beta1, beta2, eps, weight_decay, step_size,
                     bc2_sqrt, grad_scale);
  ITTS_LAUNCH_CHECK();
  return ITTS_OK;
}

extern "C" int itts_grad_norm_accum(const float* d_x, int64_t n, int norm_kind, float* d_accum,
                                    int accumulate, void* d_workspace, void* stream) {
  ITTS_REQUIRE(d_accum && d_workspace && (n == 0 || d_x), "null pointer");
  ITTS_REQUIRE(n >= 0 && (norm_kind == 2 || norm_kind == 0), "norm_kind must be 2 or 0 (infinity)");
  const int nb = (int)std::min<int64_t>((n + 255) / 256, kNormBlocks);
  hipStream_t s = as_stream(stream);
  float* part = static_cast<float*>(d_workspace);
  if (nb > 0) {
    hipLaunchKernelGGL(grad_norm_partial_kernel, dim3(nb), dim3(256), 0, s, d_x, n, norm_kind, part);
    ITTS_LAUNCH_CHECK();
  }
  hipLaunchKernelGGL(grad_norm_final_kernel, dim3(1), dim3(256), 0, s, part, nb, norm_kind, d_accum,
                     accumulate);
  ITTS_LAUNCH_CHECK();
  return ITTS_OK;
}

extern "C" int itts_adam_step_fused(float* d_param, const float* d_grad, float* d_exp_avg,
                                    float* d_exp_avg_sq, int64_t n, float lr, float beta1,
                                    float beta2, float eps, float weight_decay, int64_t step,
                                    float grad_scale, const float* d_norm_accum, int norm_kind,
                                    float clip_max_norm, float clip_value, float* d_ema_shadow,
                                    float ema_decay, void* stream) {
  ITTS_REQUIRE(d_param && d_grad && d_exp_avg && d_exp_avg_sq, "null pointer");
  ITTS_REQUIRE(n >= 0 && step >= 1, "bad sizes (step counts from 1)");
  ITTS_REQUIRE(!d_norm_accum || ((norm_kind == 2 || norm_kind == 0) && clip_max_norm > 0.f),
               "norm clipping needs norm_kind 2 or 0 and a positive max norm");
  if (n == 0) return ITTS_OK;
  const double bc1 = 1.0 - pow((double)beta1, (double)step);
  const double bc2 = 1.0 - pow((double)beta2, (double)step);
  const int blocks = (int)std::min<int64_t>((n + 255) / 256, 4096);
  hipLaunchKernelGGL(adam_fused_kernel, dim3(blocks), dim3(256), 0, as_stream(stream), d_param,
                     d_grad, d_exp_avg, d_exp_avg_sq, n, beta1, beta2, eps, weight_decay,
                     (float)(lr / bc1), (float)sqrt(bc2), grad_scale, d_norm_accum, norm_kind,
                     clip_max_norm, clip_value, d_ema_shadow, 1.f - ema_decay);
  ITTS_LAUNCH_CHECK();
  return ITTS_OK;
}

extern "C" int itts_sgd_step(float* d_param, const float* d_grad, float* d_momentum_buf, int64_t n,
                             float lr, float momentum, float dampening, float weight_decay,
                             int nesterov, int first_step, float grad_scale, void* stream) {
  ITTS_REQUIRE(d_param && d_grad, "null pointer");
  ITTS_REQUIRE(momentum == 0.f || d_momentum_buf, "momentum needs a buffer");
  ITTS_REQUIRE(n >= 0, "bad size");
  if (n == 0) return ITTS_OK;
  const int blocks = (int)std::min<int64_t>((n + 255) / 256, 4096);
  hipLaunchKernelGGL(sgd_kernel, dim3(blocks), dim3(256), 0, as_stream(stream), d_param, d_grad,
                     d_momentum_buf, n, lr, momentum, dampening, weight_decay, nesterov,
                     first_step, grad_scale);
  ITTS_LAUNCH_CHECK();
  return ITTS_OK;
}

extern "C" int itts_ema_update(float* d_shadow, const float* d_param, int64_t n, float decay,
                               void* stream) {
  ITTS_REQUIRE(d_shadow && d_param, "null pointer");
  ITTS_REQUIRE(n >= 0, "bad size");
  if (n == 0) return ITTS_OK;
  const int blocks = (int)std::min<int64_t>((n + 255) / 256, 4096);
  hipLaunchKernelGGL(ema_kernel, dim3(blocks), dim3(256), 0, as_stream(stream), d_shadow, d_param,
                     n, 1.f - decay);
  ITTS_LAUNCH_CHECK();
  return ITTS_OK;
}
```

### idiaptts_amd/lib.py

```python
import ctypes
import os
from ctypes import POINTER, c_char_p, c_double, c_float, c_int, c_int64, c_uint8, c_void_p

_HERE = os.path.dirname(os.path.abspath(__file__))
LIB_PATH = os.path.join(_HERE, "_lib", "libidiaptts_amd.so")

_lib = None


class IttsError(RuntimeError):
    pass


_P = c_void_p

_SIGNATURES = {
    "itts_abi_version": (c_int, []),
    "itts_last_error": (c_char_p, []),
    "itts_device_count": (c_int, []),
    "itts_release_scratch": (c_int, []),
    "itts_defer_reductions": (c_int, [c_int]),
    "itts_reduce_deferred": (c_int, [_P]),
    "itts_scratch_pool_stats": (c_int, [POINTER(c_int64), POINTER(c_int64), POINTER(c_int64)]),
    "itts_comm_version": (c_int, []),
    "itts_comm_unique_id": (c_int, [_P]),
    "itts_comm_init_rank": (c_int, [_P, c_int, c_int, POINTER(c_void_p)]),
    "itts_comm_destroy": (c_int, [c_void_p]),
    "itts_allreduce_flat": (c_int, [_P, c_int64, c_int, c_int, c_void_p, _P]),
    "itts_cheaptrick_fft_size": (c_int, [c_int, c_double]),
    "itts_num_aperiodicities": (c_int, [c_int]),
    "itts_mcep_alpha": (c_double, [c_int]),
    "itts_world_num_frames": (c_int64, [c_int64, c_int, c_double]),
    "itts_world_synth_length": (c_int64, [c_int64, c_int, c_double]),
    "itts_wav_info": (c_int, [c_char_p, POINTER(c_int), POINTER(c_int64)]),
    "itts_wav_read_batch": (c_int, [POINTER(c_char_p), c_int, POINTER(c_int64), c_double, _P,
                                    c_int]),
    "itts_write_feature_archives": (c_int, [_P, c_int64, POINTER(c_int64), c_int,
                                            POINTER(c_char_p), c_int, POINTER(c_int),
                                            POINTER(c_int), POINTER(c_int), POINTER(c_char_p),
                                            c_int, _P]),
    "itts_questions_load": (c_int, [c_char_p, POINTER(c_void_p), POINTER(c_int), POINTER(c_int)]),
    "itts_questions_free": (None, [c_void_p]),
    "itts_questions_vector": (c_int, [c_void_p, c_char_p, _P]),
    "itts_labels_count_frames": (c_int, [POINTER(c_char_p), c_int, POINTER(c_int64), c_int]),
    "itts_labels_generate": (c_int, [c_void_p, POINTER(c_char_p), c_int, POINTER(c_int64), _P,
                                     c_int64, c_int]),
    "itts_normalise_rows_f32": (c_int, [_P, c_int64, c_int, _P, _P, _P]),
    "itts_mlpg_scratch_bytes": (c_int64, [c_int64, c_int]),
    "itts_mlpg_generation": (c_int, [_P, c_int64, c_int, c_int, _P, POINTER(c_int64), c_int, _P,
                                     c_int64, c_int, _P, _P]),
    "itts_mlpg_scratch_bytes_f32": (c_int64, [c_int64, c_int]),
    "itts_mlpg_generation_f32": (c_int, [_P, c_int64, c_int, c_int, _P, POINTER(c_int64), c_int, _P,
                                         c_int64, c_int, _P, _P]),
    "itts_lf0_vuv": (c_int, [_P, POINTER(c_int64), c_int, c_double, c_float, _P, _P, _P]),
    "itts_interpolate_lin_f32": (c_int, [_P, POINTER(c_int64), c_int, _P, _P, _P]),
    "itts_assemble_cmp_f32": (c_int, [_P, c_int64, c_int, _P, _P, _P, c_int64, c_int,
                                      POINTER(c_int64), c_int, c_int, _P, c_int64, _P]),
    "itts_feature_stats_workspace_bytes": (c_int64, [c_int, c_int]),
    "itts_feature_stats": (c_int, [_P, c_int64, c_int64, c_int, c_int, c_int, c_int, _P, _P, _P,
                                   _P]),
    "itts_linear_fwd": (c_int, [_P, c_int64, _P, _P, _P, c_int64, c_int64, c_int, c_int, c_int,
                                _P]),
    "itts_rows_gather_f32": (c_int, [_P, c_int64, c_int64, _P, c_int64, c_int, _P, _P, c_int64, c_int, _P]),
    "itts_mlpg_plan_create": (c_int, [_P, c_int, POINTER(c_void_p)]),
    "itts_mlpg_plan_destroy": (None, [_P]),
    "itts_mlpg_plan_frames": (c_int64, [_P]),
    "itts_mlpg_generation_planned": (c_int, [_P, _P, c_int, c_int64, c_int, c_int, _P, _P, c_int64, c_int, _P, _P]),
    "itts_mlpg_choose_form": (c_int, [c_int, c_int, c_int64, c_int64, c_int]),
    "itts_mlpg_set_override": (c_int, [c_int, c_int, c_int]),
    "itts_mlpg_get_override": (c_int, [POINTER(c_int), POINTER(c_int), POINTER(c_int)]),
    "itts_mlpg_last_form": (c_int, []),
    "itts_sqrt_inplace_f64": (c_int, [_P, c_int64, _P]),
    "itts_square_inplace_f64": (c_int, [_P, c_int64, _P]),
    "itts_stft": (c_int, [_P, POINTER(c_int64), POINTER(c_int64), POINTER(c_int64), c_int, c_int, c_int, c_int, _P,
                          c_int, _P, c_int64, _P]),
    "itts_stft_mel": (c_int, [_P, POINTER(c_int64), POINTER(c_int64), POINTER(c_int64), c_int, c_int, c_int, c_int,
                              _P, _P, _P, c_int, _P, c_int64, _P]),
    "itts_mel_project": (c_int, [_P, c_int64, c_int, c_int64, _P, _P, c_int, _P, c_int64, _P]),
    "itts_griffinlim": (c_int, [_P, _P, _P, _P, POINTER(c_int64), c_int, c_int, c_int, c_int, _P, c_int, c_double,
                                c_int, _P, _P]),
    "itts_griffinlim_tile_frames": (c_int, [c_int, c_int]),
    "itts_mel_inverse": (c_int, [_P, c_int64, c_int, c_int64, c_int, c_int, _P, _P, _P, _P, c_double, c_double, c_int,
                                 c_int, _P, c_int64, c_int, _P, _P]),
    "itts_batch_pad_gather_f32": (c_int, [_P, c_int64, c_int64, _P, _P, c_int, c_int64, c_int, c_int, _P, c_int64, _P,
                                          _P, c_int64, _P, _P]),
    "itts_batch_pack_rows_f32": (c_int, [_P, c_int64, _P, _P, c_int, c_int64, c_int, c_int, _P, c_int64, c_int,
                                         c_int64, c_int64, _P]),
    "itts_batch_concat_rows_f32": (c_int, [_P, c_int64, c_int64, _P, _P, _P, c_int, c_int64, c_int, _P, c_int64, c_int,
                                           _P]),
    "itts_batch_pad_colsum_workspace_bytes": (c_int64, [c_int64, c_int]),
    "itts_batch_pad_colsum_f32": (c_int, [_P, c_int64, _P, c_int, c_int64, c_int, c_int, _P, c_int, _P, _P]),
    "itts_linear_fwd_mse_workspace_bytes": (c_int64, [c_int64, c_int]),
    "itts_linear_fwd_mse": (c_int, [_P, c_int64, _P, _P, _P, c_int64, _P, c_double, c_float, c_int64,
                                    c_int, c_int, _P, _P, c_int64, _P, _P]),
    "itts_act_bwd": (c_int, [_P, _P, _P, c_int64, c_int, _P]),
    "itts_linear_bwd_input": (c_int, [_P, c_int64, _P, _P, c_int64, _P, c_int64, c_int, c_int64,
                                      c_int, c_int, _P]),
    "itts_linear_bwd_weight_workspace_bytes": (c_int64, [c_int64, c_int, c_int]),
    "itts_linear_bwd_weight": (c_int, [_P, c_int64, _P, c_int64, _P, _P, c_int64, c_int, c_int,
                                       _P, c_int, _P]),
    "itts_linear_bwd": (c_int, [_P, c_int64, _P, c_int64, _P, _P, _P, _P, c_int64, _P, c_int64, c_int,
                                c_int64, c_int, c_int, _P, c_int, _P]),
    "itts_conv1d_fwd": (c_int, [_P, c_int64, _P, _P, _P, c_int64, c_int, c_int, c_int, c_int, c_int,
                                c_int, c_int, c_int, c_int, _P]),
    "itts_conv1d_bwd_input": (c_int, [_P, c_int64, _P, _P, c_int64, _P, c_int64, c_int, c_int, c_int,
                                      c_int, c_int, c_int, c_int, c_int, c_int, _P]),
    "itts_conv1d_bwd_weight_workspace_bytes": (c_int64, [c_int, c_int, c_int, c_int, c_int, c_int,
                                                         c_int]),
    "itts_conv1d_bwd_weight": (c_int, [_P, c_int64, _P, c_int64, _P, _P, c_int, c_int, c_int, c_int,
                                       c_int, c_int, c_int, c_int, _P, c_int, _P]),
    "itts_conv1d_plan": (c_int, [c_int, c_int, c_int, c_int, c_int, c_int, c_int, c_int, c_int, POINTER(c_int),
                                 POINTER(c_int), POINTER(c_int64)]),
    "itts_layernorm_fwd": (c_int, [_P, c_int64, _P, _P, _P, c_int64, _P, _P, c_int64, c_int, c_double, c_int, _P]),
    "itts_layernorm_workspace_bytes": (c_int64, [c_int64, c_int]),
    "itts_layernorm_bwd": (c_int, [_P, c_int64, _P, c_int64, _P, c_int64, _P, _P, _P, _P, c_int64, _P, _P, c_int64,
                                   c_int, c_int, _P, _P]),
    "itts_masked_mse_workspace_bytes": (c_int64, [c_int64, c_int]),
    "itts_masked_mse": (c_int, [_P, c_int64, _P, c_int64, _P, c_int64, c_int, c_double, c_float,
                                _P, _P, c_int64, _P, _P]),
    "itts_weighted_loss": (c_int, [_P, c_int64, _P, c_int64, _P, c_int64, c_int, c_int, _P, _P,
                                   c_int64, _P, c_int64, _P, _P]),
    "itts_cheaptrick_mcep": (c_int, [_P, POINTER(c_int64), _P, POINTER(c_int64), c_int, c_int,
                                     c_double, c_int, c_double, _P, c_int, c_double, c_double,
                                     c_int, c_int, c_double, _P, c_int64, _P, _P, _P]),
    "itts_mcep": (c_int, [_P, c_int64, c_int, c_int, c_double, c_double, c_int, c_int, c_double,
                          _P, c_int64, _P, _P, _P]),
    "itts_mgc2sp": (c_int, [_P, c_int64, c_int, c_double, c_int, _P, _P, _P, _P]),
    "itts_mgcep": (c_int, [_P, c_int, c_int64, c_int, c_int, c_double, c_double, c_double, c_int,
                           c_int, c_double, _P, c_int64, _P, _P, _P]),
    "itts_mgc2sp_gamma": (c_int, [_P, c_int64, c_int, c_double, c_double, c_int, _P, _P, _P, _P]),
    "itts_code_aperiodicity": (c_int, [_P, c_int64, c_int, c_int, _P, _P, _P]),
    "itts_decode_aperiodicity": (c_int, [_P, c_int64, c_int, c_int, _P, _P]),
    "itts_decode_aperiodicity_voiced": (c_int, [_P, _P, c_int64, c_int, c_int, _P, _P]),
    "itts_stonemask": (c_int, [_P, POINTER(c_int64), _P, POINTER(c_int64), c_int, c_int, c_double,
                               _P, _P]),
    "itts_d4c": (c_int, [_P, POINTER(c_int64), _P, POINTER(c_int64), c_int, c_int, c_double, c_int,
                         c_double, _P, _P, _P, c_int64, _P]),
    "itts_dio": (c_int, [_P, POINTER(c_int64), POINTER(c_int64), c_int, c_int, c_double, c_double,
                         c_double, c_double, c_double, _P, _P]),
    "itts_harvest_num_frames": (c_int64, [c_int64, c_int, c_double]),
    "itts_harvest": (c_int, [_P, POINTER(c_int64), POINTER(c_int64), c_int, c_int, c_double, c_double,
                             c_double, _P, _P, _P, _P, _P, _P]),
    "itts_wav2world": (c_int, [_P, POINTER(c_int64), POINTER(c_int64), c_int, c_int, c_double, c_int,
                               _P, _P, _P, _P]),
    "itts_world_synthesize": (c_int, [_P, _P, _P, POINTER(c_int64), POINTER(c_int64), c_int, c_int,
                                      c_double, c_int, c_double, _P, _P, _P]),
    "itts_world_synthesize_after": (c_int, [_P, _P, _P, POINTER(c_int64), POINTER(c_int64), c_int, c_int,
                                      c_double, c_int, c_double, _P, _P, _P, _P, _P]),
    "itts_lstm_state_bytes": (c_int64, [c_int, c_int, c_int]),
    "itts_lstm_layer_fwd": (c_int, [_P, _P, _P, _P, _P, _P, _P, _P, c_int, c_int, c_int, c_int, _P,
                                    _P, _P, _P, _P, _P, _P]),
    "itts_lstm_layer_bwd": (c_int, [_P, _P, _P, _P, _P, _P, _P, _P, c_int, c_int, c_int, c_int, _P,
                                    _P, _P, _P]),
    "itts_gru_state_bytes": (c_int64, [c_int, c_int, c_int]),
    "itts_gru_layer_fwd": (c_int, [_P, _P, _P, _P, _P, _P, _P, _P, c_int, c_int, c_int, c_int, _P,
                                   _P, _P, _P, _P]),
    "itts_gru_layer_bwd": (c_int, [_P, _P, _P, _P, _P, _P, _P, c_int, c_int, c_int, c_int, _P,
                                   _P, _P, _P, _P]),
    "itts_rnn_path_counts": (c_int, [POINTER(c_int64)]),
    "itts_gemm_path_counts": (c_int, [POINTER(c_int64)]),
    "itts_adam_step": (c_int, [_P, _P, _P, _P, c_int64, c_float, c_float, c_float, c_float,
                               c_float, c_int64, c_float, _P]),
    "itts_grad_norm_accum": (c_int, [_P, c_int64, c_int, _P, c_int, _P, _P]),
    "itts_adam_step_fused": (c_int, [_P, _P, _P, _P, c_int64, c_float, c_float, c_float, c_float,
                                     c_float, c_int64, c_float, _P, c_int, c_float, c_float, _P,
                                     c_float, _P]),
    "itts_sgd_step": (c_int, [_P, _P, _P, c_int64, c_float, c_float, c_float, c_float, c_int,
                              c_int, c_float, _P]),
    "itts_ema_update": (c_int, [_P, _P, c_int64, c_float, _P]),
}


def declared_symbols():
    return sorted(_SIGNATURES)


def load():
    global _lib
    if _lib is not None:
        return _lib
    if not os.path.exists(LIB_PATH):
        raise IttsError(
            "HIP library {} is missing. Build it with `python -m idiaptts_amd.build` "
            "(there is no CPU fallback).".format(LIB_PATH))
    try:
        import torch
    except ImportError:
        pass
    lib = ctypes.CDLL(LIB_PATH)
    for name, (res, args) in _SIGNATURES.items():
        fn = getattr(lib, name)
        fn.restype = res
        fn.argtypes = args
    _lib = lib
    return lib


def check(status, what=""):
    if status != 0:
        msg = load().itts_last_error()
        raise IttsError("{} failed with status {}: {}".format(
            what or "libidiaptts_amd call", status, msg.decode() if msg else ""))


def offsets_array(offsets):
    import numpy as np
    arr = np.array(offsets, dtype=np.int64, order="C", ndmin=1)
    if arr.ndim != 1:
        raise ValueError("offsets must be one-dimensional")
    return (c_int64 * arr.shape[0]).from_buffer(arr)


def normalise_rows(sample, sub, div):
    import numpy as np
    sub, div = np.asarray(sub), np.asarray(div)
    if (isinstance(sample, np.ndarray) and sample.dtype == np.float32 and sample.ndim == 2
            and sample.flags.c_contiguous and sub.dtype == np.float64 and div.dtype == np.float64
            and sub.shape == (sample.shape[1],) and div.shape == (sample.shape[1],)):
        try:
            L = load()
        except Exception:
            L = None
        if L is not None:
            sub, div = np.ascontiguousarray(sub), np.ascontiguousarray(div)
            out = np.empty_like(sample)
            check(L.itts_normalise_rows_f32(sample.ctypes.data, sample.shape[0], sample.shape[1],
                                            sub.ctypes.data, div.ctypes.data, out.ctypes.data),
                  "itts_normalise_rows_f32")
            return out
    return ((sample - sub) / div).astype(np.float32, copy=False)


def current_stream():
    import torch
    return torch.cuda.current_stream().cuda_stream


def require_gpu():
    import torch
    if not torch.cuda.is_available():
        raise IttsError("No HIP device visible: the idiaptts_amd hot path only runs on an "
                        "MI355X-class GPU (there is no CPU fallback).")
    load()
```

### idiaptts_amd/native_ff.py

```python
import math

import torch

from . import ops


def _pad4(n):
    return (n + 3) // 4 * 4


class FlatFFModel:

    def __init__(self, dims=(425, 512, 512, 187), acts=("tanh", "tanh", None), device="cuda",
                 seed=0, state_dict=None):
        assert len(acts) == len(dims) - 1
        self.dims = tuple(int(d) for d in dims)
        self.acts = [ops.act_code(a) for a in acts]
        self.device = torch.device(device)
        self.in_pitch = _pad4(self.dims[0])
        self.layout = []
        off = 0
        for li, (K, N) in enumerate(zip(self.dims[:-1], self.dims[1:])):
            kp = _pad4(K) if li == 0 else K
            w_off = off
            off += _pad4(N * kp)
            b_off = off
            off += _pad4(N)
            self.layout.append((w_off, b_off, N, K, kp))
        self.numel = off
        self.params = torch.zeros(off, dtype=torch.float32, device=self.device)
        self.grads = torch.zeros_like(self.params)
        self.exp_avg = torch.zeros_like(self.params)
        self.exp_avg_sq = torch.zeros_like(self.params)
        self.step_count = 0
        self._buffers = {}
        if state_dict is None:
            state_dict = self.reference_init(self.dims, seed)
        self.load_layers(state_dict)

    @staticmethod
    def reference_init(dims, seed):
        g = torch.Generator().manual_seed(seed)
        layers = []
        for K, N in zip(dims[:-1], dims[1:]):
            bound = 1.0 / math.sqrt(K)
            w = (torch.rand(N, K, generator=g) * 2 - 1) * bound
            b = (torch.rand(N, generator=g) * 2 - 1) * bound
            layers.append((w, b))
        return layers

    @staticmethod
    def from_module(model, device=None):
        from .nn.modules import LinearAct
        inner = getattr(model, "model", model)
        layers, acts = [], []
        for group in getattr(inner, "layer_groups", []):
            seq = getattr(group, "module", None)
            if not isinstance(seq, torch.nn.Sequential):
                return None
            for m in seq:
                if isinstance(m, LinearAct):
                    layers.append((m.weight.detach(), m.bias.detach()))
                    acts.append(ops.ACT_TORCH_NAME.get(m.act))
                elif isinstance(m, (torch.nn.Dropout, torch.nn.Conv1d)):
                    return None
                elif type(m).__name__ != "FusedActivation":
                    return None
        if not layers:
            return None
        dims = [layers[0][0].shape[1]] + [w.shape[0] for w, _ in layers]
        device = device if device is not None else layers[0][0].device
        return FlatFFModel(dims, acts, device=device, state_dict=layers)

    def store_to_module(self, model, buf=None):
        from .nn.modules import LinearAct
        inner = getattr(model, "model", model)
        mods = [m for g in inner.layer_groups for m in g.module if isinstance(m, LinearAct)]
        with torch.no_grad():
            for i, m in enumerate(mods):
                m.weight.copy_(self.weight(i, buf))
                m.bias.copy_(self.bias(i, buf))
        return mods

    def load_layers(self, layers):
        for i, (w, b) in enumerate(layers):
            self.weight(i).copy_(w.to(self.device))
            self.bias(i).copy_(b.to(self.device))

    def weight_padded(self, i, buf=None):
        w_off, _, N, K, kp = self.layout[i]
        return (self.params if buf is None else buf)[w_off:w_off + N * kp].view(N, kp)

    def weight(self, i, buf=None):
        K = self.layout[i][3]
        return self.weight_padded(i, buf)[:, :K]

    def bias(self, i, buf=None):
        _, b_off, N, _, _ = self.layout[i]
        return (self.params if buf is None else buf)[b_off:b_off + N]

    def pack_input(self, x):
        if x.shape[1] == self.in_pitch:
            return x
        xp = torch.zeros((x.shape[0], self.in_pitch), dtype=torch.float32, device=x.device)
        xp[:, :x.shape[1]] = x
        return xp

    def layers(self):
        return [(self.weight(i).clone(), self.bias(i).clone()) for i in range(len(self.layout))]

    def _rows_buffer(self, name, M, width):
        pitch = _pad4(width)
        buf = self._buffers.get(name)
        if buf is None or buf.shape[0] < M:
            buf = torch.zeros((M, pitch), dtype=torch.float32, device=self.device)
            self._buffers[name] = buf
        return buf[:M, :width]

    def forward(self, x, n_layers=None):
        acts = []
        h = self.pack_input(x)
        M = h.shape[0]
        for i in range(len(self.layout) if n_layers is None else n_layers):
            h = ops.linear_fwd(h, self.weight_padded(i), self.bias(i), self.acts[i],
                               out=self._rows_buffer("h%d" % i, M, self.layout[i][2]))
            acts.append(h)
        return acts

    def loss_and_backward(self, x, target, row_valid, n_valid_global, reduce_group=None, reduce=False):
        self._pending = []
        x = self.pack_input(x)
        if reduce:
            return self._loss_and_backward(x, target, row_valid, n_valid_global, reduce_group, reduce)
        with ops.deferred_reductions():
            return self._loss_and_backward(x, target, row_valid, n_valid_global, reduce_group, False)

    def _loss_and_backward(self, x, target, row_valid, n_valid_global, reduce_group, reduce):
        M = x.shape[0]
        n = len(self.layout)
        if self.acts[-1] in (None, ops.ACT_NONE) and n > 1:
            hs = self.forward(x, n_layers=n - 1)
            loss, dz = ops.linear_fwd_mse(hs[-1], self.weight_padded(n - 1), self.bias(n - 1), target,
                                          row_valid, n_valid_global,
                                          grad=self._rows_buffer("dz_out", M, self.dims[-1]))
            hs.append(None)
        else:
            hs = self.forward(x)
            loss, dz = ops.masked_mse(hs[-1], target, row_valid, n_valid_global,
                                      grad=self._rows_buffer("dz_out", M, self.dims[-1]))
            if self.acts[-1] != ops.ACT_NONE:
                dz = ops.act_bwd(dz, hs[-1], self.acts[-1])
        for i in range(n - 1, -1, -1):
            inp = hs[i - 1] if i > 0 else x
            dz_in = None
            if i > 0:
                dz_in = self._rows_buffer("dz%d" % (i & 1), M, self.layout[i][3])
                ops.linear_bwd(dz, inp, self.weight_padded(i), self.weight_padded(i, self.grads),
                               self.bias(i, self.grads), dz_in, yprev=hs[i - 1], act_prev=self.acts[i - 1])
            else:
                ops.linear_bwd_weight(dz, inp, dw=self.weight_padded(i, self.grads),
                                      db=self.bias(i, self.grads))
            if reduce:
                from .parallel import allreduce_flat_
                w_off, b_off, N, _, _ = self.layout[i]
                work = allreduce_flat_(self.grads[w_off:b_off + _pad4(N)], reduce_group, async_op=True)
                if work is not None:
                    self._pending.append(work)
            if i > 0:
                dz = dz_in
        return loss

    def train_step(self, x, target, row_valid, n_valid_global, lr=1e-3, betas=(0.9, 0.999),
                   eps=1e-8, weight_decay=0.0, process_group=None, world_size=1,
                   clip_norm_kind=None, clip_max_norm=0.0, clip_value=None, ema_shadow=None,
                   ema_decay=0.0):
        from . import parallel
        dist_on = world_size > 1 or parallel._active(process_group)
        loss = self.loss_and_backward(x, target, row_valid, n_valid_global, reduce_group=process_group,
                                      reduce=dist_on)
        for work in self._pending:
            work.wait()
        self._pending = []
        self.step_count += 1
        if clip_norm_kind is None and not clip_value and ema_shadow is None:
            ops.adam_step(self.params, self.grads, self.exp_avg, self.exp_avg_sq, self.step_count,
                          lr=lr, betas=betas, eps=eps, weight_decay=weight_decay)
            return loss
        accum = None
        if clip_norm_kind is not None:
            if getattr(self, "_norm_accum", None) is None:
                self._norm_accum = torch.zeros(1, dtype=torch.float32, device=self.device)
            accum = ops.grad_norm_accum(self.grads, self._norm_accum, clip_norm_kind)
        ops.adam_step_fused(self.params, self.grads, self.exp_avg, self.exp_avg_sq,
                            self.step_count, lr=lr, betas=betas, eps=eps,
                            weight_decay=weight_decay, norm_accum=accum,
                            norm_kind=clip_norm_kind if clip_norm_kind is not None else 2,
                            clip_max_norm=clip_max_norm, clip_value=clip_value or 0.0,
                            ema_shadow=ema_shadow, ema_decay=ema_decay)
        return loss


def flops_per_frame(dims, skip_first_dgrad=True):
    f = 0
    for i, (K, N) in enumerate(zip(dims[:-1], dims[1:])):
        f += 2 * N * K * (2 if (i == 0 and skip_first_dgrad) else 3)
    return f
```

### idiaptts_amd/ops.py

```python
import collections
import contextlib
import ctypes
import threading

import torch

from . import lib as _lib

ACT_NONE, ACT_TANH, ACT_RELU = 0, 1, 2
(ACT_SIGMOID, ACT_LOGSIGMOID, ACT_SOFTPLUS, ACT_SOFTSIGN, ACT_LEAKY_RELU, ACT_ELU, ACT_CELU, ACT_SELU, ACT_HARDTANH,
 ACT_RELU6, ACT_HARDSIGMOID) = range(3, 14)
ACT_TORCH_NAME = {ACT_TANH: "Tanh", ACT_RELU: "ReLU", ACT_SIGMOID: "Sigmoid", ACT_LOGSIGMOID: "LogSigmoid",
                  ACT_SOFTPLUS: "Softplus", ACT_SOFTSIGN: "Softsign", ACT_LEAKY_RELU: "LeakyReLU", ACT_ELU: "ELU",
                  ACT_CELU: "CELU", ACT_SELU: "SELU", ACT_HARDTANH: "Hardtanh", ACT_RELU6: "ReLU6",
                  ACT_HARDSIGMOID: "Hardsigmoid"}
ACT_BY_NAME = {None: ACT_NONE, "none": ACT_NONE, "linear": ACT_NONE}
ACT_BY_NAME.update({name.lower(): code for code, name in ACT_TORCH_NAME.items()})
CONV_ACTS = (ACT_NONE, ACT_TANH, ACT_RELU)


def act_code(act, allowed=None, where="Linear"):
    code = act if isinstance(act, int) else ACT_BY_NAME.get(act.lower() if isinstance(act, str) else act)
    if code is None or code not in (allowed if allowed is not None else range(ACT_HARDSIGMOID + 1)):
        raise NotImplementedError("{} activation {!r} is not implemented".format(where, act))
# ... 394 lines not shown
def batch_pad_gather(rows, starts, lens, n_utts, t_max, batch_first, fill_row=None, want_mask=False, width=None,
                     rep_pos=-1, rep_row=None):
    L = _lib.load()
    _need(rows, torch.float32, "rows")
    assert rows.dim() == 2 and (rows.shape[1] <= 1 or rows.stride(1) == 1)
    assert starts.dtype == torch.int64 and lens.dtype == torch.int64 and starts.is_cuda and lens.is_cuda
    assert starts.numel() >= n_utts and lens.numel() >= n_utts and starts.is_contiguous() and lens.is_contiguous()
    width = rows.shape[1] if width is None else int(width)
    shape = (n_utts, int(t_max), width) if batch_first else (int(t_max), n_utts, width)
    out = torch.empty(shape, dtype=torch.float32, device=rows.device)
    mask = torch.empty(shape[:2] + (1,), dtype=torch.float32, device=rows.device) if want_mask else None
    fill = fill_row.contiguous() if fill_row is not None else None
    rep = rep_row.contiguous() if rep_row is not None and rep_pos >= 0 else None
    ld_src = rows.stride(0) if rows.shape[0] > 1 else max(rows.shape[1], 1)
    _lib.check(L.itts_batch_pad_gather_f32(_ptr(rows), ld_src, rows.shape[0], _ptr(starts), _ptr(lens), n_utts,
                                           int(t_max), width, 1 if batch_first else 0,
                                           _ptr(fill) if fill is not None else None,
                                           int(rep_pos) if rep is not None else -1, _ptr(rep), _ptr(out), max(width, 1),
                                           _ptr(mask) if mask is not None else None, _stream()),
               "itts_batch_pad_gather_f32")
    return out, mask


def batch_pack_rows(padded, starts, lens, batch_first, n_rows, out_width=None, out=None, rep_pos=-1, rep_dst_row=-1):
    L = _lib.load()
    _need(padded, torch.float32, "padded")
    ld = _batch_rows_2d(padded, "padded")
    n_utts, t_max = (padded.shape[0], padded.shape[1]) if batch_first else (padded.shape[1], padded.shape[0])
    width = padded.shape[2]
    out_width = width if out_width is None else int(out_width)
    if out is None:
        out = torch.empty((int(n_rows), out_width), dtype=torch.float32, device=padded.device)
    assert out.dim() == 2 and out.shape[0] >= n_rows and out.shape[1] >= out_width and \
        (out.shape[1] <= 1 or out.stride(1) == 1)
    ld_dst = out.stride(0) if out.shape[0] > 1 else max(out.shape[1], 1)
    _lib.check(L.itts_batch_pack_rows_f32(_ptr(padded), ld, _ptr(starts), _ptr(lens), n_utts, t_max, width,
                                          1 if batch_first else 0, _ptr(out), ld_dst, out_width, int(rep_pos),
                                          int(rep_dst_row), _stream()),
               "itts_batch_pack_rows_f32")
    return out


def batch_concat_rows(rows, table, n_out, t_max, width=None, out_width=None):
    L = _lib.load()
    _need(rows, torch.float32, "rows")
    assert rows.dim() == 2 and (rows.shape[1] <= 1 or rows.stride(1) == 1)
    assert table.dtype == torch.int64 and table.is_cuda and table.dim() == 2 and table.shape[0] == 3 and \
        table.is_contiguous()
    width = rows.shape[1] if width is None else int(width)
    out_width = width if out_width is None else int(out_width)
    out = torch.empty((int(n_out), out_width), dtype=torch.float32, device=rows.device)
    ld_src = rows.stride(0) if rows.shape[0] > 1 else max(rows.shape[1], 1)
    _lib.check(L.itts_batch_concat_rows_f32(_ptr(rows), ld_src, rows.shape[0], _ptr(table[0]), _ptr(table[1]),
                                            _ptr(table[2]), table.shape[1], int(t_max), width, _ptr(out),
                                            max(out_width, 1), out_width, _stream()), "itts_batch_concat_rows_f32")
    return out


def batch_pad_colsum(padded, lens, batch_first, out=None):
    L = _lib.load()
    _need(padded, torch.float32, "padded")
    ld = _batch_rows_2d(padded, "padded")
    n_utts, t_max = (padded.shape[0], padded.shape[1]) if batch_first else (padded.shape[1], padded.shape[0])
    width = padded.shape[2]
    if out is None:
        out = torch.empty(width, dtype=torch.float32, device=padded.device)
    assert out.dim() == 1 and out.is_contiguous() and out.numel() >= width
    ws = torch.empty(max(int(L.itts_batch_pad_colsum_workspace_bytes(n_utts * t_max, width)), 4), dtype=torch.uint8,
                     device=padded.device)
    _lib.check(L.itts_batch_pad_colsum_f32(_ptr(padded), ld, _ptr(lens), n_utts, t_max, width,
                                           1 if batch_first else 0, _ptr(out), out.numel(), _ptr(ws), _stream()),
               "itts_batch_pad_colsum_f32")
    return out


def linear_bwd_input(dz, w, yprev=None, act_prev=ACT_NONE, out=None):
    L = _lib.load()
    _need(dz, torch.float32, "dz")
    M, N = dz.shape
    K = w.shape[1]
    if out is None:
        out = torch.empty((M, K), dtype=torch.float32, device=dz.device)
    _lib.check(L.itts_linear_bwd_input(_ptr(dz), _rows(dz, "dz"), _ptr(w), _ptr(out),
                                       _rows(out, "out"), _ptr(yprev),
                                       _rows(yprev, "yprev") if yprev is not None else 0,
                                       act_prev, M, N, K, _stream()), "itts_linear_bwd_input")
    return out


_ws_cache = {}
class _DeferState(threading.local):
    on = False
    next = 0


_defer = _DeferState()


def _workspace(nbytes, device):
    key = (device.index if device.index is not None else torch.cuda.current_device(),
           torch.cuda.current_stream(device).cuda_stream)
    if _defer.on:
        key = key + (_defer.next,)
        _defer.next += 1
    buf = _ws_cache.get(key)
    if buf is None or buf.numel() < nbytes:
        buf = torch.empty(max(int(nbytes), 1 << 20), dtype=torch.uint8, device=device)
        _ws_cache[key] = buf
    return buf


class deferred_reductions:

    def __enter__(self):
        if _defer.on:
            raise RuntimeError("deferred_reductions() blocks do not nest")
        _lib.check(_lib.load().itts_defer_reductions(1), "itts_defer_reductions")
        _defer.on, _defer.next = True, 0
        return self

    def __exit__(self, exc_type, exc, tb):
        _defer.on = False
        _lib.check(_lib.load().itts_reduce_deferred(_stream()), "itts_reduce_deferred")
        return False


def linear_bwd_weight(dz, x, dw=None, db=None, accumulate=False, want_bias=True):
    L = _lib.load()
    _need(dz, torch.float32, "dz")
    _need(x, torch.float32, "x")
    M, N = dz.shape
    K = x.shape[1]
    if dw is None:
        dw = torch.empty((N, K), dtype=torch.float32, device=dz.device)
    if db is None and want_bias:
        db = torch.empty((N,), dtype=torch.float32, device=dz.device)
    ws = _workspace(L.itts_linear_bwd_weight_workspace_bytes(M, N, K), dz.device)
    _lib.check(L.itts_linear_bwd_weight(_ptr(dz), _rows(dz, "dz"), _ptr(x), _rows(x, "x"),
                                        _ptr(dw), _ptr(db), M, N, K, _ptr(ws),
                                        1 if accumulate else 0, _stream()),
               "itts_linear_bwd_weight")
    return dw, db


def conv1d_out_len(T_in, kernel_size, padding, dilation):
    return T_in + 2 * padding - dilation * (kernel_size - 1)


def _conv_rows(t, name):
    if t.dim() != 3:
        raise ValueError("{} must be 3-D [B, T, C] (batch_first) or [T, B, C]".format(name))
    C = t.shape[2]
    ld = t.stride(1) if t.shape[1] > 1 else (t.stride(0) if t.shape[0] > 1 else C)
    ok = (t.stride(2) == 1 or C == 1) and ld >= C and (t.shape[0] == 1 or t.stride(0) == t.shape[1] * ld)
    if ok and ld != C and ld % 4 == 0:
        ok = t.storage_offset() + t.shape[0] * t.shape[1] * ld <= t.untyped_storage().nbytes() // 4
    if ok:
        return t, ld
    return t.clone(memory_format=torch.contiguous_format), C


def _conv_dims(x, batch_first):
    return (x.shape[0], x.shape[1]) if batch_first else (x.shape[1], x.shape[0])


def _conv_geometry(w, padding, dilation, T_in):
    if w.dim() != 3 or not w.is_contiguous():
        raise ValueError("w must be contiguous [Cout, Cin, Kw]")
    Cout, Cin, Kw = w.shape
    padding, dilation = int(padding), int(dilation)
    if padding < 0 or dilation < 1:
        raise ValueError("padding must be >= 0 and dilation >= 1, got {} / {}".format(padding, dilation))
    T_out = conv1d_out_len(T_in, Kw, padding, dilation)
    if T_out <= 0:
        raise ValueError("Conv1d output length T_in + 2 padding - dilation (kernel_size - 1) = {} + 2 * {} - {} * {} "
                         "= {} is not positive".format(T_in, padding, dilation, Kw - 1, T_out))
    return Cout, Cin, Kw, padding, dilation, T_out


def _conv_out(like, batch_first, B, T, C):
    shape = (B, T, C) if batch_first else (T, B, C)
    return torch.empty(shape, dtype=torch.float32, device=like.device)


def _conv_out_rows(out, shape, name="out"):
    C = shape[2]
    if tuple(out.shape) == tuple(shape) and out.dtype == torch.float32:
        ld = out.stride(1) if shape[1] > 1 else (out.stride(0) if shape[0] > 1 else C)
        if (out.stride(2) == 1 or C == 1) and ld >= C and (shape[0] == 1 or out.stride(0) == shape[1] * ld):
            return ld
    raise ValueError("{} must be a float32 {} tensor with contiguous rows of one pitch".format(name, tuple(shape)))


CONV_FWD, CONV_BWD_INPUT, CONV_BWD_WEIGHT = 0, 1, 2


def conv1d_plan(product, B, T_in, Cin, Cout, kernel_size, padding, dilation, vec=True):
    tile, slabs, kchunk = ctypes.c_int(0), ctypes.c_int(0), ctypes.c_int64(0)
    rc = _lib.load().itts_conv1d_plan(int(product), int(B), int(T_in), int(Cin), int(Cout), int(kernel_size),
                                      int(padding), int(dilation), 1 if vec else 0, ctypes.byref(tile),
                                      ctypes.byref(slabs), ctypes.byref(kchunk))
    if rc != 0:
        raise ValueError("no Conv1d plan for product {} B {} T_in {} Cin {} Cout {} kernel {} padding {} dilation {}"
                         .format(product, B, T_in, Cin, Cout, kernel_size, padding, dilation))
    return tile.value, slabs.value, kchunk.value


def conv1d_fwd(x, w, b, padding, dilation, batch_first, act=ACT_NONE, out=None):
    L = _lib.load()
    _need(x, torch.float32, "x")
    _need(w, torch.float32, "w")
    B, T_in = _conv_dims(x, batch_first)
    Cout, Cin, Kw, padding, dilation, T_out = _conv_geometry(w, padding, dilation, T_in)
    if x.shape[2] != Cin:
        raise ValueError("x has {} channels, w expects {}".format(x.shape[2], Cin))
    if b is not None:
        _need(b, torch.float32, "b")
        if b.shape != (Cout,) or not b.is_contiguous():
            raise ValueError("b must be contiguous [Cout]")
    x, ldx = _conv_rows(x, "x")
    shape = (B, T_out, Cout) if batch_first else (T_out, B, Cout)
    if out is None:
        out = _conv_out(x, batch_first, B, T_out, Cout)
    ldy = _conv_out_rows(out, shape)
    _lib.check(L.itts_conv1d_fwd(_ptr(x), ldx, _ptr(w), _ptr(b), _ptr(out), ldy, B, T_in, Cin, Cout, Kw, padding,
                                 dilation, 1 if batch_first else 0, act, _stream()), "itts_conv1d_fwd")
    return out


def conv1d_bwd_input(dz, w, T_in, padding, dilation, batch_first, yprev=None, act_prev=ACT_NONE, out=None):
    L = _lib.load()
    _need(dz, torch.float32, "dz")
    _need(w, torch.float32, "w")
    B, T_dz = _conv_dims(dz, batch_first)
    Cout, Cin, Kw, padding, dilation, T_out = _conv_geometry(w, padding, dilation, int(T_in))
    if T_dz != T_out or dz.shape[2] != Cout:
        raise ValueError("dz must have {} steps and {} channels, got {}".format(T_out, Cout, tuple(dz.shape)))
    shape = (B, T_in, Cin) if batch_first else (T_in, B, Cin)
    dz, lddz = _conv_rows(dz, "dz")
    ldyp = 0
    if yprev is not None:
        _need(yprev, torch.float32, "yprev")
        if tuple(yprev.shape) != shape:
            raise ValueError("yprev must be {}".format(shape))
        yprev, ldyp = _conv_rows(yprev, "yprev")
    if out is None:
        out = _conv_out(dz, batch_first, B, T_in, Cin)
    lddx = _conv_out_rows(out, shape)
    _lib.check(L.itts_conv1d_bwd_input(_ptr(dz), lddz, _ptr(w), _ptr(out), lddx, _ptr(yprev), ldyp, act_prev, B,
                                       int(T_in), Cin, Cout, Kw, padding, dilation, 1 if batch_first else 0,
                                       _stream()), "itts_conv1d_bwd_input")
    return out


def conv1d_bwd_weight(dz, x, kernel_size, padding, dilation, batch_first, dw=None, db=None, accumulate=False,
                      want_bias=True):
    L = _lib.load()
    _need(dz, torch.float32, "dz")
    _need(x, torch.float32, "x")
    B, T_in = _conv_dims(x, batch_first)
    Cin, Cout, Kw = x.shape[2], dz.shape[2], int(kernel_size)
    T_out = conv1d_out_len(T_in, Kw, int(padding), int(dilation))
    if Kw < 1 or int(padding) < 0 or int(dilation) < 1 or T_out <= 0:
        raise ValueError("Conv1d output length {} (T_in {}, kernel {}, padding {}, dilation {}) is not positive"
                         .format(T_out, T_in, Kw, padding, dilation))
    if _conv_dims(dz, batch_first) != (B, T_out):
        raise ValueError("dz must have batch {} and {} steps, got {}".format(B, T_out, tuple(dz.shape)))
    x, ldx = _conv_rows(x, "x")
    dz, lddz = _conv_rows(dz, "dz")
    if dw is None:
        dw = (torch.zeros if accumulate else torch.empty)((Cout, Cin, Kw), dtype=torch.float32, device=dz.device)
    if db is None and want_bias:
        db = (torch.zeros if accumulate else torch.empty)((Cout,), dtype=torch.float32, device=dz.device)
    if tuple(dw.shape) != (Cout, Cin, Kw) or not dw.is_contiguous():
        raise ValueError("dw must be contiguous [{}, {}, {}]".format(Cout, Cin, Kw))
    if db is not None and (tuple(db.shape) != (Cout,) or not db.is_contiguous()):
        raise ValueError("db must be contiguous [{}]".format(Cout))
    ws = _workspace(L.itts_conv1d_bwd_weight_workspace_bytes(B, T_in, Cin, Cout, Kw, int(padding), int(dilation)),
                    dz.device)
    _lib.check(L.itts_conv1d_bwd_weight(_ptr(dz), lddz, _ptr(x), ldx, _ptr(dw), _ptr(db), B, T_in, Cin, Cout, Kw,
                                        int(padding), int(dilation), 1 if batch_first else 0, _ptr(ws),
                                        1 if accumulate else 0, _stream()), "itts_conv1d_bwd_weight")
    return dw, db


def linear_bwd(dz, x, w, dw, db, dx, yprev=None, act_prev=ACT_NONE, accumulate=False):
    L = _lib.load()
    _need(dz, torch.float32, "dz")
    _need(x, torch.float32, "x")
    _need(w, torch.float32, "w")
    M, N = dz.shape
    K = x.shape[1]
    if w.shape != (N, K) or not w.is_contiguous() or not dw.is_contiguous() or dw.shape != (N, K):
        raise ValueError("w and dw must be contiguous [N, K]")
    ws = _workspace(L.itts_linear_bwd_weight_workspace_bytes(M, N, K), dz.device)
    _lib.check(L.itts_linear_bwd(_ptr(dz), _rows(dz, "dz"), _ptr(x), _rows(x, "x"), _ptr(w), _ptr(dw),
                                 _ptr(db), _ptr(dx), _rows(dx, "dx"), _ptr(yprev),
                                 _rows(yprev, "yprev") if yprev is not None else 0,
                                 int(act_prev if act_prev is not None else ACT_NONE), M, N, K, _ptr(ws),
                                 1 if accumulate else 0, _stream()), "itts_linear_bwd")
    return dw, db, dx


def masked_mse(pred, target, row_valid, n_valid, loss_weight=1.0, want_grad=True, grad=None):
    L = _lib.load()
    _need(pred, torch.float32, "pred")
    _need(target, torch.float32, "target")
    _need(row_valid, torch.uint8, "row_valid")
    M, D = pred.shape
    loss = torch.empty((1,), dtype=torch.float32, device=pred.device)
    if want_grad and grad is None:
        grad = torch.empty((M, D), dtype=torch.float32, device=pred.device)
    ws = _workspace(max(L.itts_masked_mse_workspace_bytes(M, D), 8), pred.device)
    _lib.check(L.itts_masked_mse(_ptr(pred), _rows(pred, "pred"), _ptr(target),
                                 _rows(target, "target"), _ptr(row_valid), M, D, float(n_valid),
                                 float(loss_weight), _ptr(loss),
                                 _ptr(grad) if want_grad else None,
                                 _rows(grad, "grad") if want_grad else 0, _ptr(ws), _stream()),
               "itts_masked_mse")
    return loss, (grad if want_grad else None)


LAYER_NORM_MAX_WIDTH = 4096


def layer_norm_fwd(x, gamma, beta, eps=1e-5, act=ACT_NONE, out=None):
    L = _lib.load()
    _need(x, torch.float32, "x")
    ldx = _rows(x, "x")
    N, D = x.shape
    for name, t in (("gamma", gamma), ("beta", beta)):
        if t is not None:
            _need(t, torch.float32, name)
            if t.shape != (D,) or not t.is_contiguous():
                raise ValueError("{} must be a contiguous [{}] vector".format(name, D))
    if out is None:
        out = torch.empty((N, D), dtype=torch.float32, device=x.device)
    stats = torch.empty((2, N), dtype=torch.float32, device=x.device)
    _lib.check(L.itts_layernorm_fwd(_ptr(x), ldx, _ptr(gamma), _ptr(beta), _ptr(out), _rows(out, "out"),
                                    _ptr(stats[0]), _ptr(stats[1]), N, D, float(eps), int(act), _stream()),
               "itts_layernorm_fwd")
    return out, stats[0], stats[1]


def layer_norm_bwd(dy, x, mean, rstd, gamma, y=None, act=ACT_NONE, want_gamma=True, want_beta=True, dx=None):
    L = _lib.load()
    _need(dy, torch.float32, "dy")
    _need(x, torch.float32, "x")
    N, D = x.shape
    if dy.shape != x.shape:
        raise ValueError("dy must have the shape of x")
    if act != ACT_NONE and y is None:
        raise ValueError("layer_norm_bwd under an activation needs the forward's output y")
    if dx is None:
        dx = torch.empty((N, D), dtype=torch.float32, device=x.device)
    dgamma = torch.empty((D,), dtype=torch.float32, device=x.device) if want_gamma else None
    dbeta = torch.empty((D,), dtype=torch.float32, device=x.device) if want_beta else None
    ws = None
    if want_gamma or want_beta:
        ws = _workspace(max(L.itts_layernorm_workspace_bytes(N, D), 8), x.device)
    _lib.check(L.itts_layernorm_bwd(_ptr(dy), _rows(dy, "dy"), _ptr(x), _rows(x, "x"),
                                    _ptr(y) if act != ACT_NONE else None,
                                    _rows(y, "y") if act != ACT_NONE else 0, _ptr(mean), _ptr(rstd), _ptr(gamma),
                                    _ptr(dx), _rows(dx, "dx"), _ptr(dgamma), _ptr(dbeta), N, D, int(act), _ptr(ws),
                                    _stream()), "itts_layernorm_bwd")
    return dx, dgamma, dbeta


def weighted_loss(pred, target, row_weight, kind, want_grad=True, want_elem=False):
    L = _lib.load()
    _need(pred, torch.float32, "pred")
    _need(target, torch.float32, "target")
    _need(row_weight, torch.float32, "row_weight")
    M, D = pred.shape
    loss = torch.empty((1,), dtype=torch.float32, device=pred.device)
    grad = torch.empty((M, D), dtype=torch.float32, device=pred.device) if want_grad else None
    elem = torch.empty((M, D), dtype=torch.float32, device=pred.device) if want_elem else None
    ws = torch.empty(max(L.itts_masked_mse_workspace_bytes(M, D), 8), dtype=torch.uint8,
                     device=pred.device)
    _lib.check(L.itts_weighted_loss(_ptr(pred), _rows(pred, "pred"), _ptr(target),
                                    _rows(target, "target"), _ptr(row_weight.contiguous()), M, D,
                                    int(kind), _ptr(loss), _ptr(grad), D if want_grad else 0,
                                    _ptr(elem), D if want_elem else 0, _ptr(ws), _stream()),
               "itts_weighted_loss")
    return loss, grad, elem


def adam_step(param, grad, exp_avg, exp_avg_sq, step, lr=1e-3, betas=(0.9, 0.999), eps=1e-8,
              weight_decay=0.0, grad_scale=1.0):
    L = _lib.load()
    for t, n in ((param, "param"), (grad, "grad"), (exp_avg, "exp_avg"),
                 (exp_avg_sq, "exp_avg_sq")):
        _need(t, torch.float32, n)
        if not t.is_contiguous():
            raise ValueError(n + " must be contiguous")
    _lib.check(L.itts_adam_step(_ptr(param), _ptr(grad), _ptr(exp_avg), _ptr(exp_avg_sq),
                                param.numel(), lr, betas[0], betas[1], eps, weight_decay,
                                int(step), grad_scale, _stream()), "itts_adam_step")


def grad_norm_accum(x, accum, norm_kind=2, accumulate=False):
    L = _lib.load()
    _need(x, torch.float32, "x")
    _need(accum, torch.float32, "accum")
    if not x.is_contiguous():
        raise ValueError("x must be contiguous")
    _lib.check(L.itts_grad_norm_accum(_ptr(x), x.numel(), int(norm_kind), _ptr(accum),
                                      int(bool(accumulate)), _ptr(_workspace(4096, x.device)),
                                      _stream()), "itts_grad_norm_accum")
    return accum


def adam_step_fused(param, grad, exp_avg, exp_avg_sq, step, lr=1e-3, betas=(0.9, 0.999), eps=1e-8,
                    weight_decay=0.0, grad_scale=1.0, norm_accum=None, norm_kind=2,
                    clip_max_norm=0.0, clip_value=0.0, ema_shadow=None, ema_decay=0.0):
    L = _lib.load()
    for t, n in ((param, "param"), (grad, "grad"), (exp_avg, "exp_avg"),
                 (exp_avg_sq, "exp_avg_sq")) + \
            (((ema_shadow, "ema_shadow"),) if ema_shadow is not None else ()):
        _need(t, torch.float32, n)
        if not t.is_contiguous() or t.numel() != param.numel():
            raise ValueError(n + " must be contiguous and as long as param")
    _lib.check(L.itts_adam_step_fused(
        _ptr(param), _ptr(grad), _ptr(exp_avg), _ptr(exp_avg_sq), param.numel(), lr, betas[0],
        betas[1], eps, weight_decay, int(step), grad_scale,
        _ptr(norm_accum) if norm_accum is not None else None, int(norm_kind),
        float(clip_max_norm), float(clip_value or 0.0),
        _ptr(ema_shadow) if ema_shadow is not None else None, float(ema_decay), _stream()),
        "itts_adam_step_fused")


def sgd_step(param, grad, momentum_buf=None, first_step=False, lr=1e-3, momentum=0.0,
             dampening=0.0, weight_decay=0.0, nesterov=False, grad_scale=1.0):
    L = _lib.load()
    for t, n in ((param, "param"), (grad, "grad")) + \
            (((momentum_buf, "momentum_buf"),) if momentum_buf is not None else ()):
        _need(t, torch.float32, n)
        if not t.is_contiguous():
            raise ValueError(n + " must be contiguous")
    _lib.check(L.itts_sgd_step(_ptr(param), _ptr(grad),
                               _ptr(momentum_buf) if momentum_buf is not None else None,
                               param.numel(), lr, momentum, dampening, weight_decay,
                               int(bool(nesterov)), int(bool(first_step)), grad_scale,
                               _stream()), "itts_sgd_step")


def ema_update(shadow, param, decay):
    L = _lib.load()
    for t, n in ((shadow, "shadow"), (param, "param")):
        _need(t, torch.float32, n)
        if not t.is_contiguous():
            raise ValueError(n + " must be contiguous")
    _lib.check(L.itts_ema_update(_ptr(shadow), _ptr(param), shadow.numel(), float(decay),
                                 _stream()), "itts_ema_update")


GemmPathCounts = collections.namedtuple("GemmPathCounts", "ring staged")


def gemm_path_counts():
    out = (ctypes.c_int64 * 8)()
    _lib.check(_lib.load().itts_gemm_path_counts(out), "itts_gemm_path_counts")
    v = [int(x) for x in out]
    return GemmPathCounts(tuple(v[:4]), tuple(v[4:]))


RnnPathCounts = collections.namedtuple("RnnPathCounts", "fwd_ran fwd_declined fwd_gave_up bwd_ran bwd_declined bwd_gave_up")


def rnn_path_counts():
    out = (ctypes.c_int64 * 6)()
    _lib.check(_lib.load().itts_rnn_path_counts(out), "itts_rnn_path_counts")
    return RnnPathCounts(*[int(v) for v in out])



def _c_int_ptr(t):
    return ctypes.c_void_p(t.data_ptr()) if t is not None else None


def cheaptrick_mcep(x, x_off, f0, f_off, fs, frame_period=5.0, fft_size=None, q1=-0.15,
                    want_sp=True, order=None, alpha=None, eps=1e-8, miniter=2, maxiter=30,
                    threshold=1e-3, mc_dtype=torch.float32, want_iters=False):
    L = _lib.load()
    _need(x, torch.float64, "x")
    _need(f0, torch.float64, "f0")
    fft_size = fft_size or L.itts_cheaptrick_fft_size(fs, 71.0)
    T = int(f_off[-1])
    K = fft_size // 2 + 1
    sp = torch.empty((T, K), dtype=torch.float64, device=x.device) if want_sp else None
    mc32 = mc64 = iters = None
    if order is not None:
        if mc_dtype == torch.float32:
            mc32 = torch.empty((T, order + 1), dtype=torch.float32, device=x.device)
        else:
            mc64 = torch.empty((T, order + 1), dtype=torch.float64, device=x.device)
        if want_iters:
            iters = torch.empty((T,), dtype=torch.int32, device=x.device)
    _lib.check(L.itts_cheaptrick_mcep(_ptr(x), _lib.offsets_array(x_off), _ptr(f0),
                                      _lib.offsets_array(f_off), len(x_off) - 1, fs,
                                      float(frame_period), fft_size, q1, _ptr(sp),
                                      order if order is not None else 0,
                                      float(alpha) if alpha is not None else 0.0, eps, miniter,
                                      maxiter, threshold, _ptr(mc32), (order or 0) + 1, _ptr(mc64),
                                      _ptr(iters), _stream()), "itts_cheaptrick_mcep")
    return sp, (mc32 if mc32 is not None else mc64), iters


def mcep(amp_sp, order, alpha, eps=1e-8, miniter=2, maxiter=30, threshold=1e-3,
         dtype=torch.float32, want_iters=False):
    L = _lib.load()
    _need(amp_sp, torch.float64, "amp_sp")
    amp_sp = amp_sp.contiguous()
    T, K = amp_sp.shape
    out = torch.empty((T, order + 1), dtype=dtype, device=amp_sp.device)
    iters = torch.empty((T,), dtype=torch.int32, device=amp_sp.device) if want_iters else None
    f32 = out if dtype == torch.float32 else None
    f64 = out if dtype == torch.float64 else None
    _lib.check(L.itts_mcep(_ptr(amp_sp), T, K, order, float(alpha), eps, miniter, maxiter,
                           threshold, _ptr(f32), order + 1, _ptr(f64), _ptr(iters), _stream()),
               "itts_mcep")
    return (out, iters) if want_iters else out


def mgc2sp(mc, alpha, fftlen, want_logamp=False, want_pow=False):
    L = _lib.load()
    _need(mc, torch.float64, "mc")
    mc = mc.contiguous()
    T, m1 = mc.shape
    K = fftlen // 2 + 1
    out32 = None if (want_logamp or want_pow) else torch.empty((T, K), dtype=torch.float32,
                                                               device=mc.device)
    out64 = torch.empty((T, K), dtype=torch.float64, device=mc.device) if want_logamp else None
    outpw = torch.empty((T, K), dtype=torch.float64, device=mc.device) if want_pow else None
    _lib.check(L.itts_mgc2sp(_ptr(mc), T, m1 - 1, float(alpha), fftlen, _ptr(out32), _ptr(out64),
                             _ptr(outpw), _stream()), "itts_mgc2sp")
    return out64 if want_logamp else (outpw if want_pow else out32)


def mgcep(sp, order, alpha, gamma, eps=1e-8, miniter=2, maxiter=30, threshold=1e-3,
          dtype=torch.float32, want_iters=False, input_is_power=False):
    L = _lib.load()
    _need(sp, torch.float64, "sp")
    sp = sp.contiguous()
    T, K = sp.shape
    out = torch.empty((T, order + 1), dtype=dtype, device=sp.device)
    iters = torch.empty((T,), dtype=torch.int32, device=sp.device) if want_iters else None
    f32 = out if dtype == torch.float32 else None
    f64 = out if dtype == torch.float64 else None
    _lib.check(L.itts_mgcep(_ptr(sp), 1 if input_is_power else 0, T, K, order, float(alpha),
                            float(gamma), eps, miniter, maxiter, threshold, _ptr(f32), order + 1,
                            _ptr(f64), _ptr(iters), _stream()), "itts_mgcep")
    return (out, iters) if want_iters else out


def mgc2sp_gamma(mgc, alpha, gamma, fftlen, want_logamp=False, want_pow=False):
    L = _lib.load()
    _need(mgc, torch.float64, "mgc")
    mgc = mgc.contiguous()
    T, m1 = mgc.shape
    K = fftlen // 2 + 1
    out32 = None if (want_logamp or want_pow) else torch.empty((T, K), dtype=torch.float32,
                                                               device=mgc.device)
    out64 = torch.empty((T, K), dtype=torch.float64, device=mgc.device) if want_logamp else None
    outpw = torch.empty((T, K), dtype=torch.float64, device=mgc.device) if want_pow else None
    _lib.check(L.itts_mgc2sp_gamma(_ptr(mgc), T, m1 - 1, float(alpha), float(gamma), fftlen,
                                   _ptr(out32), _ptr(out64), _ptr(outpw), _stream()),
               "itts_mgc2sp_gamma")
    return out64 if want_logamp else (outpw if want_pow else out32)


def code_aperiodicity(ap, fs, dtype=torch.float64):
    L = _lib.load()
    _need(ap, torch.float64, "ap")
    ap = ap.contiguous()
    T, K = ap.shape
    nap = L.itts_num_aperiodicities(fs)
    out = torch.empty((T, nap), dtype=dtype, device=ap.device)
    _lib.check(L.itts_code_aperiodicity(_ptr(ap), T, (K - 1) * 2, fs,
                                        _ptr(out) if dtype == torch.float64 else None,
                                        _ptr(out) if dtype == torch.float32 else None, _stream()),
               "itts_code_aperiodicity")
    return out


def decode_aperiodicity(bap, fs, fft_size, voiced_f0=None):
    L = _lib.load()
    _need(bap, torch.float64, "bap")
    bap = bap.contiguous()
    T = bap.shape[0]
    out = torch.empty((T, fft_size // 2 + 1), dtype=torch.float64, device=bap.device)
    if voiced_f0 is not None:
        _need(voiced_f0, torch.float64, "voiced_f0")
        if voiced_f0.numel() != T:
            raise ValueError("voiced_f0 and bap differ in frames")
        _lib.check(L.itts_decode_aperiodicity_voiced(_ptr(bap), _ptr(voiced_f0.contiguous()), T, fs, fft_size,
                                                     _ptr(out), _stream()), "itts_decode_aperiodicity_voiced")
        return out
    _lib.check(L.itts_decode_aperiodicity(_ptr(bap), T, fs, fft_size, _ptr(out), _stream()),
               "itts_decode_aperiodicity")
    return out


def dio(x, x_off, f_off, fs, frame_period=5.0, f0_floor=71.0, f0_ceil=800.0,
        channels_in_octave=2.0, allowed_range=0.1):
    L = _lib.load()
# ... 118 lines not shown
```

### include/idiaptts_amd.h

```cpp
#ifndef IDIAPTTS_AMD_H
#define IDIAPTTS_AMD_H

#include <stdint.h>

#ifdef __cplusplus
extern "C" {
#endif

#define ITTS_OK 0
#define ITTS_E_INVALID (-1)
#define ITTS_E_HIP (-2)
#define ITTS_E_UNSUPPORTED (-3)

int itts_abi_version(void);
const char* itts_last_error(void);
int itts_device_count(void);
int itts_scratch_pool_stats(int64_t* reserved, int64_t* used, int64_t* keep_threshold);

int itts_release_scratch(void);

int itts_defer_reductions(int on);
int itts_reduce_deferred(void* stream);

#define ITTS_F32 0
#define ITTS_F64 1
#define ITTS_REDUCE_SUM 0
#define ITTS_REDUCE_MAX 1
#define ITTS_REDUCE_AVG 2
int itts_comm_version(void);
int itts_comm_unique_id(void* h_id128);
int itts_comm_init_rank(const void* h_id128, int n_ranks, int rank, void** comm_out);
int itts_comm_destroy(void* comm);
int itts_allreduce_flat(void* d_buf, int64_t n, int dtype, int op, void* comm, void* stream);

int itts_cheaptrick_fft_size(int fs, double f0_floor);
int itts_num_aperiodicities(int fs);
double itts_mcep_alpha(int fs);
int64_t itts_world_num_frames(int64_t n_samples, int fs, double frame_period_ms);
int64_t itts_world_synth_length(int64_t n_frames, int fs, double frame_period_ms);

int itts_wav_info(const char* h_path, int* fs, int64_t* n_samples);
int itts_wav_read_batch(const char* const* h_paths, int n_files, const int64_t* h_offsets,
                        double preemphasis, double* h_out, int n_threads);
int itts_write_feature_archives(const float* h_feat, int64_t ld, const int64_t* h_f_off, int n_utts,
                                const char* const* h_paths, int n_streams, const int* h_col0,
                                const int* h_width, const int* h_parts, const char* const* h_keys,
                                int n_threads, unsigned char* h_needs_merge);

int itts_normalise_rows_f32(const float* h_x, int64_t rows, int cols, const double* h_sub,
                            const double* h_div, float* h_out);

int itts_questions_load(const char* h_path, void** handle, int* n_binary, int* n_continuous);
void itts_questions_free(void* handle);
int itts_questions_vector(void* handle, const char* h_label, double* h_out);
int itts_labels_count_frames(const char* const* h_paths, int n_files, int64_t* h_frames, int n_threads);
int itts_labels_generate(void* handle, const char* const* h_paths, int n_files,
                         const int64_t* h_frame_off, double* h_out, int64_t ld_out, int n_threads);

int64_t itts_mlpg_scratch_bytes(int64_t t_total, int dim);
int itts_mlpg_generation(const double* d_feat, int64_t ld_feat, int col0, int dim,
                         const double* d_var, const int64_t* h_offsets, int n_utts,
                         double* d_out, int64_t ld_out, int ocol0, void* d_scratch,
                         void* stream);
int64_t itts_mlpg_scratch_bytes_f32(int64_t t_total, int dim);
int itts_mlpg_generation_f32(const float* d_feat, int64_t ld_feat, int col0, int dim,
                             const double* d_var, const int64_t* h_offsets, int n_utts,
                             double* d_out, int64_t ld_out, int ocol0, void* d_scratch,
                             void* stream);

int itts_mlpg_plan_create(const int64_t* h_offsets, int n_utts, void** plan_out);
void itts_mlpg_plan_destroy(void* plan);
int64_t itts_mlpg_plan_frames(const void* plan);
int itts_mlpg_generation_planned(const void* plan, const void* d_feat, int feat_is_f32, int64_t ld_feat, int col0,
                                 int dim, const double* d_var, double* d_out, int64_t ld_out, int ocol0,
                                 void* d_scratch, void* stream);

#define ITTS_MLPG_FORM_SWEEPS 1
#define ITTS_MLPG_FORM_STREAM 2
#define ITTS_MLPG_FORM_RING 3
#define ITTS_MLPG_FORM_SOLVE_MASK 3
#define ITTS_MLPG_FORM_WIDE 4
#define ITTS_MLPG_FORM_F32_ROWS 8
#define ITTS_MLPG_FORM_NT_IN 16
#define ITTS_MLPG_FORM_WIDENED_COPY 32
int itts_mlpg_choose_form(int n_utts, int dim, int64_t t_max, int64_t t_total, int rows_f32);
#define ITTS_MLPG_FORCE_OFF 1
#define ITTS_MLPG_FORCE_ON 2
int itts_mlpg_set_override(int solve, int width, int nt);
int itts_mlpg_get_override(int* solve, int* width, int* nt);
int itts_mlpg_last_form(void);


int itts_lf0_vuv(const double* d_f0, const int64_t* h_f_off, int n_utts,
                 double f0_silence_threshold, float lf0_zero, float* d_lf0, float* d_vuv,
                 void* stream);
int itts_sqrt_inplace_f64(double* d_x, int64_t n, void* stream);
int itts_square_inplace_f64(double* d_x, int64_t n, void* stream);

int itts_stft(const double* d_x, const int64_t* h_x_off, const int64_t* h_f_off, const int64_t* h_first,
              int n_utts, int n_fft, int hop, int pad_mode, const double* d_window, int out_kind,
              void* d_out, int64_t ld_out, void* stream);
int itts_stft_mel(const double* d_x, const int64_t* h_x_off, const int64_t* h_f_off, const int64_t* h_first,
                  int n_utts, int n_fft, int hop, int pad_mode, const double* d_window,
                  const int* d_mel_tab, const float* d_mel_w, int n_mels, float* d_out, int64_t ld_out,
                  void* stream);
int itts_mel_project(const double* d_amp, int64_t T, int K, int64_t ld_amp, const int* d_mel_tab,
                     const float* d_mel_w, int n_mels, float* d_out, int64_t ld_out, void* stream);

int itts_griffinlim(const void* d_S, void* d_ang_a, void* d_ang_b, void* d_tprev, const int64_t* h_f_off,
                    int n_utts, int n_fft, int hop, int pad_mode, const double* d_window, int n_iter,
                    double momentum, int is_f64, void* d_y, void* stream);
int itts_griffinlim_tile_frames(int n_fft, int hop);

int itts_mel_inverse(const void* d_mel, int64_t n_frames, int n_mels, int64_t ld_mel, int mel_f64, int n_fft,
                     const int* d_bin_j, const double* d_bin_w, const int* d_filt, const double* d_pinv_t,
                     double inv_lipschitz, double tol, int max_iter, int check_every, void* d_out, int64_t ld_out,
                     int out_f64, int* d_iters, void* stream);

int itts_interpolate_lin_f32(const float* d_in, const int64_t* h_off, int n_utts, float* d_ip,
                             float* d_vuv, void* stream);
int itts_assemble_cmp_f32(const float* d_sp, int64_t ld_sp, int n_sp, const float* d_lf0,
                          const float* d_vuv, const float* d_bap, int64_t ld_bap, int n_bap,
                          const int64_t* h_f_off, int n_utts, int add_deltas, float* d_out,
                          int64_t ld_out, void* stream);
int64_t itts_feature_stats_workspace_bytes(int width, int want_cov);
int itts_feature_stats(const float* d_x, int64_t ld_x, int64_t n_rows, int col0, int width,
                       int want_cov, int accumulate, double* d_sum, double* d_second,
                       void* d_workspace, void* stream);

int itts_rows_gather_f32(const float* d_src, int64_t ld_src, int64_t n_src, const int64_t* d_idx, int64_t n_out,
                         int width, const float* d_fill_row, float* d_dst, int64_t ld_dst, int dst_width,
                         void* stream);

int itts_batch_pad_gather_f32(const float* d_src, int64_t ld_src, int64_t n_src, const int64_t* d_starts,
                              const int64_t* d_lens, int n_utts, int64_t t_max, int width, int batch_first,
                              const float* d_fill_row, int64_t rep_pos, const float* d_rep_row, float* d_dst,
                              int64_t ld_dst, float* d_mask, void* stream);
int itts_batch_pack_rows_f32(const float* d_src, int64_t ld_src, const int64_t* d_starts, const int64_t* d_lens,
                             int n_utts, int64_t t_max, int width, int batch_first, float* d_dst, int64_t ld_dst,
                             int dst_width, int64_t rep_pos, int64_t rep_dst_row, void* stream);
int itts_batch_concat_rows_f32(const float* d_src, int64_t ld_src, int64_t n_src, const int64_t* d_src_starts,
                               const int64_t* d_dst_starts, const int64_t* d_lens, int n_utts, int64_t t_max, int width,
                               float* d_dst, int64_t ld_dst, int dst_width, void* stream);
int64_t itts_batch_pad_colsum_workspace_bytes(int64_t n_rows, int width);
int itts_batch_pad_colsum_f32(const float* d_x, int64_t ld_x, const int64_t* d_lens, int n_utts, int64_t t_max,
                              int width, int batch_first, float* d_out, int out_width, void* d_workspace,
                              void* stream);

#define ITTS_ACT_NONE 0
#define ITTS_ACT_TANH 1
#define ITTS_ACT_RELU 2
#define ITTS_ACT_SIGMOID 3
#define ITTS_ACT_LOGSIGMOID 4
#define ITTS_ACT_SOFTPLUS 5
#define ITTS_ACT_SOFTSIGN 6
#define ITTS_ACT_LEAKY_RELU 7
#define ITTS_ACT_ELU 8
#define ITTS_ACT_CELU 9
#define ITTS_ACT_SELU 10
#define ITTS_ACT_HARDTANH 11
#define ITTS_ACT_RELU6 12
#define ITTS_ACT_HARDSIGMOID 13
int itts_linear_fwd(const float* d_x, int64_t ldx, const float* d_w, const float* d_b,
                    float* d_y, int64_t ldy, int64_t M, int N, int K, int act, void* stream);
int64_t itts_linear_fwd_mse_workspace_bytes(int64_t M, int N);
int itts_linear_fwd_mse(const float* d_x, int64_t ldx, const float* d_w, const float* d_b,
                        const float* d_target, int64_t ldt, const uint8_t* d_row_valid, double n_valid,
                        float loss_weight, int64_t M, int N, int K, float* d_loss, float* d_dz,
                        int64_t lddz, void* d_workspace, void* stream);

int itts_act_bwd(const float* d_dy, const float* d_y, float* d_dz, int64_t n_elem, int act,
                 void* stream);
int itts_linear_bwd_input(const float* d_dz, int64_t lddz, const float* d_w, float* d_dx,
                          int64_t lddx, const float* d_yprev, int64_t ldyp, int act_prev,
                          int64_t M, int N, int K, void* stream);
int64_t itts_linear_bwd_weight_workspace_bytes(int64_t M, int N, int K);
int itts_linear_bwd_weight(const float* d_dz, int64_t lddz, const float* d_x, int64_t ldx,
                           float* d_dw, float* d_db, int64_t M, int N, int K,
                           void* d_workspace, int accumulate, void* stream);
int itts_linear_bwd(const float* d_dz, int64_t lddz, const float* d_x, int64_t ldx, const float* d_w,
                    float* d_dw, float* d_db, float* d_dx, int64_t lddx, const float* d_yprev,
                    int64_t ldyp, int act_prev, int64_t M, int N, int K, void* d_workspace,
                    int accumulate, void* stream);

int itts_conv1d_fwd(const float* d_x, int64_t ldx, const float* d_w, const float* d_b, float* d_y,
                    int64_t ldy, int B, int T_in, int Cin, int Cout, int Kw, int pad, int dil,
                    int batch_first, int act, void* stream);
int itts_conv1d_bwd_input(const float* d_dz, int64_t lddz, const float* d_w, float* d_dx, int64_t lddx,
                          const float* d_yprev, int64_t ldyp, int act_prev, int B, int T_in, int Cin,
                          int Cout, int Kw, int pad, int dil, int batch_first, void* stream);
int64_t itts_conv1d_bwd_weight_workspace_bytes(int B, int T_in, int Cin, int Cout, int Kw, int pad, int dil);
int itts_conv1d_bwd_weight(const float* d_dz, int64_t lddz, const float* d_x, int64_t ldx, float* d_dw,
                           float* d_db, int B, int T_in, int Cin, int Cout, int Kw, int pad, int dil,
                           int batch_first, void* d_workspace, int accumulate, void* stream);
int itts_conv1d_plan(int product, int B, int T_in, int Cin, int Cout, int Kw, int pad, int dil, int vec,
                     int* tile_cols, int* slabs, int64_t* kchunk);

int itts_layernorm_fwd(const float* d_x, int64_t ldx, const float* d_gamma, const float* d_beta,
                       float* d_y, int64_t ldy, float* d_mean, float* d_rstd, int64_t N, int D,
                       double eps, int act, void* stream);
int64_t itts_layernorm_workspace_bytes(int64_t N, int D);
int itts_layernorm_bwd(const float* d_dy, int64_t lddy, const float* d_x, int64_t ldx,
                       const float* d_y, int64_t ldy, const float* d_mean, const float* d_rstd,
                       const float* d_gamma, float* d_dx, int64_t lddx, float* d_dgamma,
                       float* d_dbeta, int64_t N, int D, int act, void* d_workspace, void* stream);

int64_t itts_masked_mse_workspace_bytes(int64_t M, int D);
int itts_masked_mse(const float* d_pred, int64_t ldp, const float* d_target, int64_t ldt,
                    const uint8_t* d_row_valid, int64_t M, int D, double n_valid,
                    float loss_weight, float* d_loss, float* d_grad, int64_t ldg,
                    void* d_workspace, void* stream);

int itts_weighted_loss(const float* d_pred, int64_t ldp, const float* d_target, int64_t ldt,
                       const float* d_row_weight, int64_t M, int D, int kind, float* d_loss,
                       float* d_grad, int64_t ldg, float* d_elem, int64_t lde, void* d_workspace,
                       void* stream);

int itts_adam_step(float* d_param, const float* d_grad, float* d_exp_avg, float* d_exp_avg_sq,
                   int64_t n, float lr, float beta1, float beta2, float eps, float weight_decay,
                   int64_t step, float grad_scale, void* stream);

int itts_grad_norm_accum(const float* d_x, int64_t n, int norm_kind, float* d_accum,
                         int accumulate, void* d_workspace, void* stream);

int itts_adam_step_fused(float* d_param, const float* d_grad, float* d_exp_avg,
                         float* d_exp_avg_sq, int64_t n, float lr, float beta1, float beta2,
                         float eps, float weight_decay, int64_t step, float grad_scale,
                         const float* d_norm_accum, int norm_kind, float clip_max_norm,
                         float clip_value, float* d_ema_shadow, float ema_decay, void* stream);

int itts_sgd_step(float* d_param, const float* d_grad, float* d_momentum_buf, int64_t n, float lr,
                  float momentum, float dampening, float weight_decay, int nesterov,
                  int first_step, float grad_scale, void* stream);

int itts_ema_update(float* d_shadow, const float* d_param, int64_t n, float decay, void* stream);


int itts_cheaptrick_mcep(const double* d_x, const int64_t* h_x_off, const double* d_f0,
                         const int64_t* h_f_off, int n_utts, int fs, double frame_period_ms,
                         int fft_size, double q1, double* d_sp, int order, double alpha, double eps,
                         int miniter, int maxiter, double threshold, float* d_mc_f32, int64_t ld_mc,
                         double* d_mc_f64, int* d_iters, void* stream);

int itts_mcep(const double* d_amp_sp, int64_t T, int K, int order, double alpha, double eps,
              int miniter, int maxiter, double threshold, float* d_mc_f32, int64_t ld_mc,
              double* d_mc_f64, int* d_iters, void* stream);

int itts_mgc2sp(const double* d_mc, int64_t T, int order, double alpha, int fftlen,
                float* d_amp_f32, double* d_logamp_f64, double* d_pow_f64, void* stream);

int itts_mgcep(const double* d_amp_sp, int input_is_power, int64_t T, int K, int order, double alpha,
               double gamma, double eps, int miniter, int maxiter, double threshold,
               float* d_mgc_f32, int64_t ld_mgc, double* d_mgc_f64, int* d_iters, void* stream);
int itts_mgc2sp_gamma(const double* d_mgc, int64_t T, int order, double alpha, double gamma,
                      int fftlen, float* d_amp_f32, double* d_logamp_f64, double* d_pow_f64,
                      void* stream);

int itts_code_aperiodicity(const double* d_ap, int64_t T, int fft_size, int fs, double* d_bap_f64,
                           float* d_bap_f32, void* stream);
int itts_decode_aperiodicity(const double* d_bap, int64_t T, int fs, int fft_size, double* d_ap,
                             void* stream);
int itts_decode_aperiodicity_voiced(const double* d_bap, const double* d_f0, int64_t T, int fs,
                                    int fft_size, double* d_ap, void* stream);

int itts_stonemask(const double* d_x, const int64_t* h_x_off, const double* d_f0_in,
                   const int64_t* h_f_off, int n_utts, int fs, double frame_period_ms,
                   double* d_f0_out, void* stream);

int itts_d4c(const double* d_x, const int64_t* h_x_off, const double* d_f0, const int64_t* h_f_off,
             int n_utts, int fs, double frame_period_ms, int fft_size, double threshold,
             double* d_ap, double* d_bap_f64, float* d_bap_f32, int64_t ld_bap, void* stream);

int itts_dio(const double* d_x, const int64_t* h_x_off, const int64_t* h_f_off, int n_utts, int fs,
             double frame_period_ms, double f0_floor, double f0_ceil, double channels_in_octave,
             double allowed_range, double* d_f0, void* stream);

int64_t itts_harvest_num_frames(int64_t n_samples, int fs, double frame_period_ms);
int itts_harvest(const double* d_x, const int64_t* h_x_off, const int64_t* h_f_off, int n_utts,
                 int fs, double frame_period_ms, double f0_floor, double f0_ceil, double* d_f0,
                 double* d_dbg_raw, double* d_dbg_cand, double* d_dbg_score, double* d_dbg_best,
                 void* stream);

int itts_wav2world(const double* d_x, const int64_t* h_x_off, const int64_t* h_f_off, int n_utts,
                   int fs, double frame_period_ms, int fft_size, double* d_f0, double* d_sp,
                   double* d_ap, void* stream);

int itts_world_synthesize(const double* d_f0, const double* d_sp, const double* d_ap,
                          const int64_t* h_f_off, const int64_t* h_y_off, int n_utts, int fs,
                          double frame_period_ms, int fft_size, double preemphasis, float* d_y_f32,
                          double* d_y_f64, void* stream);
int itts_world_synthesize_after(const double* d_f0, const double* d_sp, const double* d_ap,
                                const int64_t* h_f_off, const int64_t* h_y_off, int n_utts, int fs,
                                double frame_period_ms, int fft_size, double preemphasis,
                                float* d_y_f32, double* d_y_f64, void* stream, void* envelope_ready_event,
                                void* aperiodicity_ready_event);

int64_t itts_lstm_state_bytes(int B, int H, int ndir);
int itts_lstm_layer_fwd(const float* d_gin, const float* d_whh, const float* d_h0, const float* d_c0,
                        const int* d_lengths, const int* h_lengths, const int* d_row_off,
                        const int* d_rev_row, int T, int B, int H, int ndir, float* d_y,
                        float* d_gates, float* d_csave, float* d_hn, float* d_cn, void* d_state,
                        void* stream);
int itts_lstm_layer_bwd(const float* d_dy, const float* d_whh, const float* d_c0,
                        const float* d_gates, const float* d_csave, const int* h_lengths,
                        const int* d_row_off, const int* d_rev_row, int T, int B, int H, int ndir,
                        float* d_dg, float* d_dc0, void* d_state, void* stream);

int64_t itts_gru_state_bytes(int B, int H, int ndir);
int itts_gru_layer_fwd(const float* d_gin, const float* d_whh, const float* d_bhh,
                       const float* d_h0, const int* d_lengths, const int* h_lengths,
                       const int* d_row_off, const int* d_rev_row, int T, int B, int H, int ndir,
                       float* d_y, float* d_gates, float* d_hn, void* d_state, void* stream);
int itts_gru_layer_bwd(const float* d_dy, const float* d_whh, const float* d_gates,
                       const float* d_hprev, const int* h_lengths,
                       const int* d_row_off, const int* d_rev_row, int T, int B, int H, int ndir,
                       float* d_dgi, float* d_dgh, float* d_dh0, void* d_state, void* stream);

int itts_gemm_path_counts(int64_t out[8]);

int itts_rnn_path_counts(int64_t out[6]);

#ifdef __cplusplus
}
#endif
#endif
```

Measured before the change: 38.60 million.

## Add native fused feed-forward train step with optional two-range side-stream split

Adds a single native entry point that runs the whole feed-forward training step (forward, fused output MSE, backward GEMMs and slab reductions) in one call. The Python model uses it by default for fused-output models, which replaces many per-layer Python and ctypes launches and batches the final loss and gradient reductions. An optional mode splits the rows into two ranges run on a side stream with a thread-local ring grid size; by default it is off because the auto part count is 1. The cost is a large new code path with its own workspace planning, slab placement offsets, and a cached layer table keyed on buffer pointers.

```diff
diff --git a/idiaptts_amd/csrc/context.h b/idiaptts_amd/csrc/context.h
--- a/idiaptts_amd/csrc/context.h
+++ b/idiaptts_amd/csrc/context.h
@@ -58,6 +58,9 @@
   double2* tw_compact[16] = {nullptr};
   JumpTable* jump = nullptr;
   int64_t* pinned = nullptr;
+  hipStream_t side_stream = nullptr;
+  hipEvent_t side_fork = nullptr, side_join = nullptr;
+  bool side_busy = false;
   std::map<std::tuple<int, int, long long>, FreqtTables> freqt;
 };
 
@@ -75,6 +78,14 @@
 int launch_gemm_f64(const double* A, int64_t lda, const double* B, int64_t ldb, double* C, int64_t ldc,
                     int64_t T, int N, int K, const int* rows, hipStream_t s, bool a_has_slack = true);
 
+struct SideStream {
+  hipStream_t stream = nullptr;
+  hipEvent_t fork = nullptr, join = nullptr;
+  DeviceContext* ctx = nullptr;
+};
+int side_stream_acquire(SideStream* out);
+void side_stream_release(SideStream* s);
+
 int64_t* pinned_slot(DeviceContext* ctx);
 
 int staged_upload(void* d_dst, const void* src, size_t bytes, hipStream_t s);
diff --git a/idiaptts_amd/csrc/context.hip b/idiaptts_amd/csrc/context.hip
--- a/idiaptts_amd/csrc/context.hip
+++ b/idiaptts_amd/csrc/context.hip
@@ -5,6 +5,7 @@
 #include <algorithm>
 #include <atomic>
 #include <cmath>
+#include <condition_variable>
 #include <cstring>
 #include <mutex>
 #include <vector>
@@ -231,6 +232,49 @@
   }
   g_contexts[dev] = ctx;
   return ctx;
+}
+
+static std::mutex g_side_mutex;
+static std::condition_variable g_side_free;
+
+int side_stream_acquire(SideStream* out) {
+  DeviceContext* ctx = get_context();
+  if (!ctx) return ITTS_E_HIP;
+  std::unique_lock<std::mutex> lock(g_side_mutex);
+  g_side_free.wait(lock, [&] { return !ctx->side_busy; });
+  if (!ctx->side_stream) {
+    hipStream_t st = nullptr;
+    hipEvent_t fork = nullptr, join = nullptr;
+    hipError_t e = hipStreamCreateWithFlags(&st, hipStreamNonBlocking);
+    if (e == hipSuccess) e = hipEventCreateWithFlags(&fork, hipEventDisableTiming);
+    if (e == hipSuccess) e = hipEventCreateWithFlags(&join, hipEventDisableTiming);
+    if (e != hipSuccess) {
+      if (join) (void)hipEventDestroy(join);
+      if (fork) (void)hipEventDestroy(fork);
+      if (st) (void)hipStreamDestroy(st);
+      set_error(std::string("side_stream_acquire: could not create the side stream: ") + hipGetErrorString(e));
+      return ITTS_E_HIP;
+    }
+    ctx->side_stream = st;
+    ctx->side_fork = fork;
+    ctx->side_join = join;
+  }
+  ctx->side_busy = true;
+  out->stream = ctx->side_stream;
+  out->fork = ctx->side_fork;
+  out->join = ctx->side_join;
+  out->ctx = ctx;
+  return ITTS_OK;
+}
+
+void side_stream_release(SideStream* s) {
+  if (!s->ctx) return;
+  {
+    std::lock_guard<std::mutex> lock(g_side_mutex);
+    s->ctx->side_busy = false;
+  }
+  s->ctx = nullptr;
+  g_side_free.notify_all();
 }
 
 struct Mat128 {
diff --git a/idiaptts_amd/csrc/nn.hip b/idiaptts_amd/csrc/nn.hip
--- a/idiaptts_amd/csrc/nn.hip
+++ b/idiaptts_amd/csrc/nn.hip
@@ -1,8 +1,10 @@
 #include <algorithm>
 #include <atomic>
 #include <cstdlib>
+#include <vector>
 
 #include "common.h"
+#include "context.h"
 #include "gemm_ring.h"
 #include "gemm_staged.h"
 
@@ -197,6 +199,7 @@
 }
 
 constexpr int kRingGrid = 512;
+static thread_local int t_ring_grid = kRingGrid;
 
 template <bool A_ROW, bool B_ROW>
 static bool ring_ok(const GemmArgs& g, int splitk, int epi) {
@@ -239,7 +242,7 @@
   r.gn = ring_group(r.tiles_n, BNT, g.K, A_ROW && B_ROW);
   const int64_t ntiles = (int64_t)r.tiles_m * r.tiles_n * splitk;
   ITTS_REQUIRE(ntiles < ((int64_t)1 << 31), "too many tiles");
-  const int grid = (int)std::min<int64_t>(kRingGrid, (ntiles + 7) / 8 * 8);
+  const int grid = (int)std::min<int64_t>(t_ring_grid, (ntiles + 7) / 8 * 8);
   if (A_ROW && B_ROW && EPI == ring::EPI_BIAS_ACT && r.gn < r.tiles_n)
     hipLaunchKernelGGL((ring::gemm_ring_kernel<A_ROW, B_ROW, EPI, WM, A_ROW && B_ROW && EPI == ring::EPI_BIAS_ACT, AF>),
                        dim3(grid), dim3(ring::THREADS), 0, s, r);
@@ -274,7 +277,7 @@
   g_gemm_path[0][EPI_X].fetch_add(1, std::memory_order_relaxed);
   const ring::Args rw = ring_args<WM_W>(gw, splitk), rx = ring_args<2>(gx, 1);
   hipLaunchKernelGGL((ring::gemm_ring_pair_kernel<false, false, EPI_STORE, WM_W, true, false, EPI_X, 2, AF_X>),
-                     dim3(kRingGrid), dim3(ring::THREADS), 0, s, rw, rx);
+                     dim3(t_ring_grid), dim3(ring::THREADS), 0, s, rw, rx);
   ITTS_LAUNCH_CHECK();
   return ITTS_OK;
 }
@@ -750,17 +753,18 @@
   return std::max<int64_t>(tiles, kRingGrid) * 8;
 }
 
-extern "C" int itts_linear_fwd_mse(const float* d_x, int64_t ldx, const float* d_w, const float* d_b,
-                                   const float* d_target, int64_t ldt, const uint8_t* d_row_valid,
-                                   double n_valid, float loss_weight, int64_t M, int N, int K,
-                                   float* d_loss, float* d_dz, int64_t lddz, void* d_workspace,
-                                   void* stream) {
-  ITTS_REQUIRE(d_w && d_loss && d_workspace && (M == 0 || (d_x && d_target && d_row_valid && d_dz)),
+static int linear_fwd_mse_impl(const float* d_x, int64_t ldx, const float* d_w, const float* d_b,
+                               const float* d_target, int64_t ldt, const uint8_t* d_row_valid,
+                               double n_valid, float loss_weight, int64_t M, int N, int K,
+                               float* d_loss, float* d_dz, int64_t lddz, void* d_workspace,
+                               void* stream, int* n_partial) {
+  ITTS_REQUIRE(d_w && (d_loss || n_partial) && d_workspace && (M == 0 || (d_x && d_target && d_row_valid && d_dz)),
                "null pointer");
   ITTS_REQUIRE(M >= 0 && N > 0 && K > 0 && ldx >= K && ldt >= N && lddz >= N && n_valid > 0, "bad sizes");
   hipStream_t s = as_stream(stream);
   if (M == 0) {
-    ITTS_HIP_CHECK(hipMemsetAsync(d_loss, 0, 4, s));
+    if (n_partial) *n_partial = 0;
+    else ITTS_HIP_CHECK(hipMemsetAsync(d_loss, 0, 4, s));
     return ITTS_OK;
   }
   ITTS_REQUIRE((ldx % 4 == 0) && aligned16(d_x) && (K % 4 == 0) && aligned16(d_w) && (lddz % 4 == 0) &&
@@ -778,13 +782,26 @@
   int64_t tiles = ((M + BM - 1) / BM) * ((N + 63) / 64);
   int rc;
   if (ring_ok<true, true>(g, 1, EPI_MSE)) {
-    tiles = std::min<int64_t>(kRingGrid, (tiles + 7) / 8 * 8);
+    tiles = std::min<int64_t>(t_ring_grid, (tiles + 7) / 8 * 8);
     rc = launch_ring_wm<true, true, EPI_MSE, 2>(g, 1, s);
   } else {
     rc = launch_gemm_tn<true, true, EPI_MSE, 1, 1>(g, 1, s);
   }
   if (rc) return rc;
+  if (n_partial) {
+    *n_partial = (int)tiles;
+    return ITTS_OK;
+  }
   return launch_mse_final(reinterpret_cast<const double*>(d_workspace), (int)tiles, scale, d_loss, s);
+}
+
+extern "C" int itts_linear_fwd_mse(const float* d_x, int64_t ldx, const float* d_w, const float* d_b,
+                                   const float* d_target, int64_t ldt, const uint8_t* d_row_valid,
+                                   double n_valid, float loss_weight, int64_t M, int N, int K,
+                                   float* d_loss, float* d_dz, int64_t lddz, void* d_workspace,
+                                   void* stream) {
+  return linear_fwd_mse_impl(d_x, ldx, d_w, d_b, d_target, ldt, d_row_valid, n_valid, loss_weight, M, N, K, d_loss,
+                             d_dz, lddz, d_workspace, stream, nullptr);
 }
 
 extern "C" int itts_act_bwd(const float* d_dy, const float* d_y, float* d_dz, int64_t n_elem,
@@ -832,9 +849,21 @@
   return (int64_t)s * ((int64_t)N * K + N) * 4 + (int64_t)kColsumSlices * N * 4 + 8192;
 }
 
-extern "C" int itts_linear_bwd_weight(const float* d_dz, int64_t lddz, const float* d_x,
-                                      int64_t ldx, float* d_dw, float* d_db, int64_t M, int N,
-                                      int K, void* d_workspace, int accumulate, void* stream) {
+struct SlabPlace {
+  int z0, total;
+};
+
+static int bwd_weight_slabs(int64_t M, int N, int K, bool ring, int64_t* kchunk) {
+  const int S = ring ? choose_splitk_ring(M, N, K) : choose_splitk(M, N, K);
+  int64_t kc = (M + S - 1) / S;
+  kc = ((kc + BK - 1) / BK) * BK;
+  *kchunk = kc;
+  return (int)((M + kc - 1) / kc);
+}
+
+static int linear_bwd_weight_impl(const float* d_dz, int64_t lddz, const float* d_x,
+                                  int64_t ldx, float* d_dw, float* d_db, int64_t M, int N,
+                                  int K, void* d_workspace, int accumulate, void* stream, const SlabPlace* place) {
   ITTS_REQUIRE(d_dw && d_workspace && (M == 0 || (d_dz && d_x)), "null pointer");
   ITTS_REQUIRE(M >= 0 && N > 0 && K > 0 && lddz >= N && ldx >= K, "bad sizes");
   hipStream_t s = as_stream(stream);
@@ -846,13 +875,12 @@
     return ITTS_OK;
   }
   const bool vec_ok = (lddz % 4 == 0) && aligned16(d_dz) && (ldx % 4 == 0) && aligned16(d_x) && (K % 4 == 0);
-  const int S = vec_ok ? choose_splitk_ring(M, N, K) : choose_splitk(M, N, K);
-  int64_t kchunk = (M + S - 1) / S;
-  kchunk = ((kchunk + BK - 1) / BK) * BK;
-  const int S_eff = (int)((M + kchunk - 1) / kchunk);
+  int64_t kchunk;
+  const int S_eff = bwd_weight_slabs(M, N, K, vec_ok, &kchunk);
+  const int z0 = place ? place->z0 : 0, S_all = place ? place->total : S_eff;
   float* slabs = reinterpret_cast<float*>(d_workspace);
   GemmArgs g{};
-  g.A = d_dz; g.lda = lddz; g.B = d_x; g.ldb = ldx; g.C = slabs; g.ldc = K;
+  g.A = d_dz; g.lda = lddz; g.B = d_x; g.ldb = ldx; g.ldc = K;
   g.M = N; g.N = K; g.K = M; g.kchunk = kchunk; g.slab_stride = (int64_t)N * K;
   g.vecA = (lddz % 4 == 0) && aligned16(d_dz);
   g.vecB = (ldx % 4 == 0) && aligned16(d_x);
@@ -861,24 +889,33 @@
     const bool merged = d_db == d_dw + n && N % 4 == 0 && n % 4 == 0;
     const int64_t stride = merged ? n + N : n;
     g.slab_stride = stride;
-    g.bias_part = merged ? slabs + n : slabs + (int64_t)S_eff * n;
+    g.C = slabs + z0 * stride;
+    float* bias_slabs = merged ? slabs + n : slabs + (int64_t)S_all * n;
     g.bias_part_stride = merged ? stride : N;
+    g.bias_part = bias_slabs + z0 * g.bias_part_stride;
     int rc = launch_gemm<false, false, EPI_STORE>(g, S_eff, s);
-    if (rc) return rc;
+    if (rc || place) return rc;
     if (merged) return launch_reduce_slabs(slabs, S_eff, n + N, d_dw, accumulate, s);
     rc = launch_reduce_slabs(slabs, S_eff, n, d_dw, accumulate, s);
     if (rc) return rc;
-    return launch_reduce_slabs(g.bias_part, S_eff, (int64_t)N, d_db, accumulate, s);
-  }
+    return launch_reduce_slabs(bias_slabs, S_eff, (int64_t)N, d_db, accumulate, s);
+  }
+  g.C = slabs + z0 * n;
   int rc = launch_gemm<false, false, EPI_STORE>(g, S_eff, s);
-  if (rc) return rc;
+  if (rc || place) return rc;
   return launch_reduce_slabs(slabs, S_eff, n, d_dw, accumulate, s);
 }
 
-extern "C" int itts_linear_bwd(const float* d_dz, int64_t lddz, const float* d_x, int64_t ldx,
-                               const float* d_w, float* d_dw, float* d_db, float* d_dx, int64_t lddx,
-                               const float* d_yprev, int64_t ldyp, int act_prev, int64_t M, int N, int K,
-                               void* d_workspace, int accumulate, void* stream) {
+extern "C" int itts_linear_bwd_weight(const float* d_dz, int64_t lddz, const float* d_x,
+                                      int64_t ldx, float* d_dw, float* d_db, int64_t M, int N,
+                                      int K, void* d_workspace, int accumulate, void* stream) {
+  return linear_bwd_weight_impl(d_dz, lddz, d_x, ldx, d_dw, d_db, M, N, K, d_workspace, accumulate, stream, nullptr);
+}
+
+static int linear_bwd_impl(const float* d_dz, int64_t lddz, const float* d_x, int64_t ldx,
+                           const float* d_w, float* d_dw, float* d_db, float* d_dx, int64_t lddx,
+                           const float* d_yprev, int64_t ldyp, int act_prev, int64_t M, int N, int K,
+                           void* d_workspace, int accumulate, void* stream, const SlabPlace* place) {
   ITTS_REQUIRE(d_w && d_dw && d_workspace && (M == 0 || (d_dz && d_x && d_dx)), "null pointer");
   ITTS_REQUIRE(M >= 0 && N > 0 && K > 0 && lddz >= N && ldx >= K && lddx >= K, "bad sizes");
   ITTS_REQUIRE(!d_yprev || ldyp >= K, "ldyp too small");
@@ -891,26 +928,26 @@
   bool fused = vec_ok && M > 0 && (lddx % 4 == 0) && aligned16(d_dx) &&
                (!d_yprev || ((ldyp % 4 == 0) && aligned16(d_yprev)));
   GemmArgs gw{}, gx{};
-  int S_eff = 1;
+  int S_eff = 1, S_all = 1;
   if (fused) {
-    const int S = choose_splitk_ring(M, N, K);
-    int64_t kchunk = (M + S - 1) / S;
-    kchunk = ((kchunk + BK - 1) / BK) * BK;
-    S_eff = (int)((M + kchunk - 1) / kchunk);
+    int64_t kchunk;
+    S_eff = bwd_weight_slabs(M, N, K, true, &kchunk);
+    const int z0 = place ? place->z0 : 0;
+    S_all = place ? place->total : S_eff;
     float* slabs = reinterpret_cast<float*>(d_workspace);
-    gw.A = d_dz; gw.lda = lddz; gw.B = d_x; gw.ldb = ldx; gw.C = slabs; gw.ldc = K;
+    const int64_t stride = merged ? n + N : n;
+    gw.A = d_dz; gw.lda = lddz; gw.B = d_x; gw.ldb = ldx; gw.C = slabs + z0 * stride; gw.ldc = K;
     gw.M = N; gw.N = K; gw.K = M; gw.kchunk = kchunk; gw.vecA = gw.vecB = 1;
-    const int64_t stride = merged ? n + N : n;
     gw.slab_stride = stride;
-    if (merged) { gw.bias_part = slabs + n; gw.bias_part_stride = stride; }
-    else if (d_db) { gw.bias_part = slabs + (int64_t)S_eff * n; gw.bias_part_stride = N; }
+    if (merged) { gw.bias_part = slabs + n + z0 * stride; gw.bias_part_stride = stride; }
+    else if (d_db) { gw.bias_part = slabs + (int64_t)S_all * n + (int64_t)z0 * N; gw.bias_part_stride = N; }
     gx.A = d_dz; gx.lda = lddz; gx.B = d_w; gx.ldb = K; gx.C = d_dx; gx.ldc = lddx;
     gx.M = M; gx.N = K; gx.K = N; gx.aux = d_yprev; gx.ldaux = ldyp; gx.act = act_prev;
     gx.kchunk = ((N + BK - 1) / BK) * BK; gx.vecA = gx.vecB = 1;
     fused = ring_ok<false, false>(gw, S_eff, EPI_STORE) && ring_ok<true, false>(gx, 1, d_yprev ? EPI_DACT : EPI_STORE);
   }
   if (!fused) {
-    int rc = itts_linear_bwd_weight(d_dz, lddz, d_x, ldx, d_dw, d_db, M, N, K, d_workspace, accumulate, stream);
+    int rc = linear_bwd_weight_impl(d_dz, lddz, d_x, ldx, d_dw, d_db, M, N, K, d_workspace, accumulate, stream, place);
     if (rc) return rc;
     return itts_linear_bwd_input(d_dz, lddz, d_w, d_dx, lddx, d_yprev, ldyp, act_prev, M, N, K, stream);
   }
@@ -921,11 +958,241 @@
                  : launch_ring_bwd_pair<2, EPI_DACT, AF_EXT>(gw, S_eff, gx, s);
   else if (d_yprev) rc = wm == 1 ? launch_ring_bwd_pair<1, EPI_DACT>(gw, S_eff, gx, s) : launch_ring_bwd_pair<2, EPI_DACT>(gw, S_eff, gx, s);
   else rc = wm == 1 ? launch_ring_bwd_pair<1, EPI_STORE>(gw, S_eff, gx, s) : launch_ring_bwd_pair<2, EPI_STORE>(gw, S_eff, gx, s);
-  if (rc) return rc;
+  if (rc || place) return rc;
   float* slabs = reinterpret_cast<float*>(d_workspace);
   rc = launch_reduce_slabs(slabs, S_eff, merged ? n + N : n, d_dw, accumulate, s);
   if (rc || merged || !d_db) return rc;
   return launch_reduce_slabs(slabs + (int64_t)S_eff * n, S_eff, (int64_t)N, d_db, accumulate, s);
+}
+
+extern "C" int itts_linear_bwd(const float* d_dz, int64_t lddz, const float* d_x, int64_t ldx,
+                               const float* d_w, float* d_dw, float* d_db, float* d_dx, int64_t lddx,
+                               const float* d_yprev, int64_t ldyp, int act_prev, int64_t M, int N, int K,
+                               void* d_workspace, int accumulate, void* stream) {
+  return linear_bwd_impl(d_dz, lddz, d_x, ldx, d_w, d_dw, d_db, d_dx, lddx, d_yprev, ldyp, act_prev, M, N, K,
+                         d_workspace, accumulate, stream, nullptr);
+}
+
+constexpr int kFFStepRanges = 2;
+constexpr int kFFStepAutoParts = 1;
+static std::atomic<int64_t> g_ff_steps[kFFStepRanges];
+
+struct FFStepPlan {
+  int parts = 1;
+  int64_t m0[kFFStepRanges + 1] = {0, 0, 0};
+};
+
+static int64_t ff_step_split(int64_t M) {
+  const int64_t m = (M / 2 + 64) / 128 * 128;
+  return (m <= 0 || m >= M) ? 0 : m;
+}
+
+static bool ff_step_feeds_chip(const itts_ff_layer* layers, int n_layers, int64_t rows) {
+  int n_min = layers[0].N;
+  for (int i = 1; i < n_layers; ++i) n_min = std::min(n_min, layers[i].N);
+  const int64_t tiles = ((rows + 127) / 128) * ((n_min + 63) / 64);
+  return tiles >= kRingGrid / kFFStepRanges;
+}
+
+static FFStepPlan ff_step_plan(const itts_ff_layer* layers, int n_layers, int64_t M, int parts) {
+  FFStepPlan p;
+  const int64_t m = ff_step_split(M);
+  if (parts == 0)
+    parts = (kFFStepAutoParts > 1 && m > 0 && ff_step_feeds_chip(layers, n_layers, std::min(m, M - m))) ? kFFStepAutoParts
+                                                                                                       : 1;
+  p.parts = (parts > 1 && m > 0) ? kFFStepRanges : 1;
+  p.m0[1] = p.parts > 1 ? m : M;
+  p.m0[2] = M;
+  return p;
+}
+
+static int64_t align64f(int64_t floats) { return (floats + 63) / 64 * 64; }
+
+extern "C" int64_t itts_ff_train_step_workspace_bytes(const itts_ff_layer* layers, int n_layers, int64_t M,
+                                                      int parts) {
+  if (!layers || n_layers < 1 || M < 0 || parts < 0 || parts > kFFStepRanges) return 0;
+  const FFStepPlan p = ff_step_plan(layers, n_layers, M, parts);
+  int64_t floats = 0, partials = 0;
+  for (int r = 0; r < p.parts; ++r) {
+    const int64_t rows = p.m0[r + 1] - p.m0[r];
+    for (int i = 0; i < n_layers; ++i) {
+      const int S = std::max(choose_splitk(rows, layers[i].N, layers[i].K), choose_splitk_ring(rows, layers[i].N, layers[i].K));
+      floats += (int64_t)S * ((int64_t)layers[i].N * layers[i].K + layers[i].N);
+    }
+    partials += itts_linear_fwd_mse_workspace_bytes(rows, layers[n_layers - 1].N) / 8;
+  }
+  return (floats + 64 * (int64_t)n_layers) * 4 + partials * 8 + 256;
+}
+
+extern "C" int itts_ff_step_counts(int64_t out[2]) {
+  ITTS_REQUIRE(out != nullptr, "null pointer");
+  for (int k = 0; k < kFFStepRanges; ++k) out[k] = g_ff_steps[k].load(std::memory_order_relaxed);
+  return ITTS_OK;
+}
+
+namespace {
+struct FFStepArgs {
+  const itts_ff_layer* layers;
+  int n;
+  const float* params;
+  float* grads;
+  const float* x;
+  int64_t ldx;
+  const float* target;
+  int64_t ldt;
+  const uint8_t* row_valid;
+  double n_valid;
+};
+}
+
+static int ff_step_issue(const FFStepArgs& a, const FFStepPlan& p, const std::vector<SlabPlace>* place,
+                         const std::vector<float*>& slabs, double* partial, int* n_partial_all, const int* grid,
+                         hipStream_t const* streams) {
+  const int n = a.n;
+  int rc = ITTS_OK;
+  for (int i = 0; i < n && !rc; ++i) {
+    const itts_ff_layer& L = a.layers[i];
+    for (int r = 0; r < p.parts && !rc; ++r) {
+      const int64_t r0 = p.m0[r], rows = p.m0[r + 1] - r0;
+      const float* in = i == 0 ? a.x + r0 * a.ldx : a.layers[i - 1].h + r0 * a.layers[i - 1].ldh;
+      const int64_t ldin = i == 0 ? a.ldx : a.layers[i - 1].ldh;
+      t_ring_grid = grid[r];
+      if (i < n - 1) {
+        rc = itts_linear_fwd(in, ldin, a.params + L.w_off, a.params + L.b_off, L.h + r0 * L.ldh, L.ldh, rows, L.N,
+                             L.K, L.act, streams[r]);
+      } else {
+        int np = 0;
+        rc = linear_fwd_mse_impl(in, ldin, a.params + L.w_off, a.params + L.b_off, a.target + r0 * a.ldt, a.ldt,
+                                 a.row_valid + r0, a.n_valid, 1.0f, rows, L.N, L.K, nullptr, L.dz + r0 * L.lddz,
+                                 L.lddz, partial + *n_partial_all, streams[r], &np);
+        *n_partial_all += np;
+      }
+    }
+  }
+  for (int i = n - 1; i >= 0 && !rc; --i) {
+    const itts_ff_layer& L = a.layers[i];
+    for (int r = 0; r < p.parts && !rc; ++r) {
+      const int64_t r0 = p.m0[r], rows = p.m0[r + 1] - r0;
+      const float* dz = L.dz + r0 * L.lddz;
+      t_ring_grid = grid[r];
+      if (i > 0) {
+        const itts_ff_layer& P = a.layers[i - 1];
+        rc = linear_bwd_impl(dz, L.lddz, P.h + r0 * P.ldh, P.ldh, a.params + L.w_off, a.grads + L.w_off,
+                             a.grads + L.b_off, P.dz + r0 * P.lddz, P.lddz, P.h + r0 * P.ldh, P.ldh, P.act, rows, L.N,
+                             L.K, slabs[i], 0, streams[r], &place[r][i]);
+      } else {
+        rc = linear_bwd_weight_impl(dz, L.lddz, a.x + r0 * a.ldx, a.ldx, a.grads + L.w_off, a.grads + L.b_off, rows,
+                                    L.N, L.K, slabs[i], 0, streams[r], &place[r][i]);
+      }
+    }
+  }
+  t_ring_grid = kRingGrid;
+  return rc;
+}
+
+extern "C" int itts_ff_train_step(const itts_ff_layer* layers, int n_layers, const float* d_params, float* d_grads,
+                                  const float* d_x, int64_t ldx, const float* d_target, int64_t ldt,
+                                  const uint8_t* d_row_valid, int64_t M, double n_valid, float* d_loss,
+                                  void* d_workspace, int64_t workspace_bytes, int parts, int grid, void* stream) {
+  ITTS_REQUIRE(layers && d_params && d_grads && d_x && d_target && d_row_valid && d_loss && d_workspace, "null pointer");
+  ITTS_REQUIRE(n_layers >= 2 && M > 0 && n_valid > 0, "bad sizes");
+  ITTS_REQUIRE(parts >= 0 && parts <= kFFStepRanges, "parts must be 0 (the library chooses), 1 or 2");
+  ITTS_REQUIRE(grid == 0 || (grid > 0 && grid <= kRingGrid && grid % 8 == 0),
+               "grid must be 0 or a multiple of 8 up to the number of persistent workgroups");
+  ITTS_REQUIRE(!t_defer && t_pending.nseg == 0, "not inside a deferred-reduction block");
+  ITTS_REQUIRE(aligned16(d_workspace), "workspace must be 16-byte aligned");
+  for (int i = 0; i < n_layers; ++i) {
+    const itts_ff_layer& L = layers[i];
+    ITTS_REQUIRE(L.N > 0 && L.K > 0 && L.w_off >= 0 && L.b_off >= 0 && L.dz && L.lddz >= L.N, "bad layer table");
+    ITTS_REQUIRE(L.act >= ITTS_ACT_NONE && L.act <= ITTS_ACT_HARDSIGMOID, "unknown activation");
+    ITTS_REQUIRE(i == n_layers - 1 ? L.act == ITTS_ACT_NONE : (L.h && L.ldh >= L.N),
+                 "hidden layers need an output buffer, the output layer has no activation (its loss is fused)");
+    ITTS_REQUIRE(i == 0 ? ldx >= L.K : L.K == layers[i - 1].N, "layer widths do not chain");
+  }
+  ITTS_REQUIRE(ldt >= layers[n_layers - 1].N, "ldt too small");
+  hipStream_t s = as_stream(stream);
+  const FFStepPlan p = ff_step_plan(layers, n_layers, M, parts);
+
+  std::vector<SlabPlace> place[kFFStepRanges];
+  std::vector<float*> slabs(n_layers);
+  std::vector<int> s_all(n_layers);
+  float* ws = reinterpret_cast<float*>(d_workspace);
+  int64_t off = 0;
+  for (int i = 0; i < n_layers; ++i) {
+    const itts_ff_layer& L = layers[i];
+    const float* in = i == 0 ? d_x : layers[i - 1].h;
+    const int64_t ldin = i == 0 ? ldx : layers[i - 1].ldh;
+    const bool vec_ok = (L.lddz % 4 == 0) && aligned16(L.dz) && (ldin % 4 == 0) && aligned16(in) && (L.K % 4 == 0);
+    int total = 0;
+    for (int r = 0; r < p.parts; ++r) {
+      int64_t kchunk;
+      place[r].push_back(SlabPlace{total, 0});
+      total += bwd_weight_slabs(p.m0[r + 1] - p.m0[r], L.N, L.K, vec_ok, &kchunk);
+    }
+    for (int r = 0; r < p.parts; ++r) place[r][i].total = total;
+    s_all[i] = total;
+    slabs[i] = ws + off;
+    off = align64f(off + (int64_t)total * ((int64_t)L.N * L.K + L.N));
+  }
+  double* partial = reinterpret_cast<double*>(ws + off);
+  int64_t need = off * 4;
+  for (int r = 0; r < p.parts; ++r)
+    need += itts_linear_fwd_mse_workspace_bytes(p.m0[r + 1] - p.m0[r], layers[n_layers - 1].N);
+  ITTS_REQUIRE(need <= workspace_bytes, "workspace too small (itts_ff_train_step_workspace_bytes)");
+
+  const FFStepArgs a{layers, n_layers, d_params, d_grads, d_x, ldx, d_target, ldt, d_row_valid, n_valid};
+  hipStream_t streams[kFFStepRanges] = {s, s};
+  int grids[kFFStepRanges] = {kRingGrid, kRingGrid};
+  int n_partial = 0, rc;
+  if (p.parts > 1) {
+    SideStream side;
+    rc = side_stream_acquire(&side);
+    if (rc) return rc;
+    streams[1] = side.stream;
+    if (grid) grids[0] = grids[1] = grid;
+    hipError_t e = hipEventRecord(side.fork, s);
+    if (e == hipSuccess) e = hipStreamWaitEvent(side.stream, side.fork, 0);
+    if (e != hipSuccess) {
+      side_stream_release(&side);
+      set_error(std::string("itts_ff_train_step (fork): ") + hipGetErrorString(e));
+      return ITTS_E_HIP;
+    }
+    rc = ff_step_issue(a, p, place, slabs, partial, &n_partial, grids, streams);
+    e = hipEventRecord(side.join, side.stream);
+    if (e == hipSuccess) e = hipStreamWaitEvent(s, side.join, 0);
+    if (e != hipSuccess) (void)hipStreamSynchronize(side.stream);
+    side_stream_release(&side);
+    if (rc) return rc;
+    if (e != hipSuccess) {
+      set_error(std::string("itts_ff_train_step (join): ") + hipGetErrorString(e));
+      return ITTS_E_HIP;
+    }
+  } else {
+    rc = ff_step_issue(a, p, place, slabs, partial, &n_partial, grids, streams);
+    if (rc) return rc;
+  }
+
+  const itts_ff_layer& out = layers[n_layers - 1];
+  t_defer = true;
+  rc = launch_mse_final(partial, n_partial, 1.0 / (n_valid * (double)out.N), d_loss, s);
+  for (int i = n_layers - 1; i >= 0 && !rc; --i) {
+    const itts_ff_layer& L = layers[i];
+    const int64_t n = (int64_t)L.N * L.K;
+    float* dw = d_grads + L.w_off;
+    float* db = d_grads + L.b_off;
+    const bool merged = db == dw + n && L.N % 4 == 0 && n % 4 == 0;
+    rc = launch_reduce_slabs(slabs[i], s_all[i], merged ? n + L.N : n, dw, 0, s);
+    if (!rc && !merged) rc = launch_reduce_slabs(slabs[i] + (int64_t)s_all[i] * n, s_all[i], (int64_t)L.N, db, 0, s);
+  }
+  t_defer = false;
+  if (rc) {
+    t_pending.nseg = 0;
+    return rc;
+  }
+  rc = flush_deferred(s);
+  if (rc) return rc;
+  g_ff_steps[p.parts - 1].fetch_add(1, std::memory_order_relaxed);
+  return ITTS_OK;
 }
 
 static int mse_blocks(int64_t M, int D) {
diff --git a/idiaptts_amd/lib.py b/idiaptts_amd/lib.py
--- a/idiaptts_amd/lib.py
+++ b/idiaptts_amd/lib.py
@@ -13,6 +13,11 @@
 
 
 _P = c_void_p
+
+class FFLayer(ctypes.Structure):
+    _fields_ = [("w_off", c_int64), ("b_off", c_int64), ("N", c_int), ("K", c_int), ("act", c_int),
+                ("reserved", c_int), ("h", c_void_p), ("ldh", c_int64), ("dz", c_void_p), ("lddz", c_int64)]
+
 
 _SIGNATURES = {
     "itts_abi_version": (c_int, []),
@@ -99,6 +104,10 @@
     "itts_linear_bwd_weight_workspace_bytes": (c_int64, [c_int64, c_int, c_int]),
     "itts_linear_bwd_weight": (c_int, [_P, c_int64, _P, c_int64, _P, _P, c_int64, c_int, c_int,
                                        _P, c_int, _P]),
+    "itts_ff_train_step_workspace_bytes": (c_int64, [_P, c_int, c_int64, c_int]),
+    "itts_ff_train_step": (c_int, [_P, c_int, _P, _P, _P, c_int64, _P, c_int64, _P, c_int64, c_double, _P, _P,
+                                   c_int64, c_int, c_int, _P]),
+    "itts_ff_step_counts": (c_int, [POINTER(c_int64)]),
     "itts_linear_bwd": (c_int, [_P, c_int64, _P, c_int64, _P, _P, _P, _P, c_int64, _P, c_int64, c_int,
                                 c_int64, c_int, c_int, _P, c_int, _P]),
     "itts_conv1d_fwd": (c_int, [_P, c_int64, _P, _P, _P, c_int64, c_int, c_int, c_int, c_int, c_int,
diff --git a/idiaptts_amd/native_ff.py b/idiaptts_amd/native_ff.py
--- a/idiaptts_amd/native_ff.py
+++ b/idiaptts_amd/native_ff.py
@@ -1,4 +1,5 @@
 import math
+import os
 
 import torch
 
@@ -34,6 +35,11 @@
         self.exp_avg_sq = torch.zeros_like(self.params)
         self.step_count = 0
         self._buffers = {}
+        self.step_parts = int(os.environ.get("ITTS_FF_STEP_PARTS", "0") or 0)
+        self.step_grid = int(os.environ.get("ITTS_FF_STEP_GRID", "0") or 0)
+        if self.step_parts not in (0, 1, 2):
+            raise ValueError("ITTS_FF_STEP_PARTS must be 1 or 2")
+        self._step_table = None
         if state_dict is None:
             state_dict = self.reference_init(self.dims, seed)
         self.load_layers(state_dict)
@@ -132,13 +138,40 @@
         x = self.pack_input(x)
         if reduce:
             return self._loss_and_backward(x, target, row_valid, n_valid_global, reduce_group, reduce)
+        if self._fused_output() and x.shape[0] > 0:
+            return self._native_step(x, target, row_valid, n_valid_global)
         with ops.deferred_reductions():
             return self._loss_and_backward(x, target, row_valid, n_valid_global, reduce_group, False)
+
+    def _fused_output(self):
+        return self.acts[-1] in (None, ops.ACT_NONE) and len(self.layout) > 1
+
+    def _native_step(self, x, target, row_valid, n_valid_global):
+        M = x.shape[0]
+        n = len(self.layout)
+        hs = [self._rows_buffer("h%d" % i, M, self.layout[i][2]) for i in range(n - 1)]
+        dzs = [None] * n
+        dzs[n - 1] = self._rows_buffer("dz_out", M, self.dims[-1])
+        for i in range(n - 1, 0, -1):
+            dzs[i - 1] = self._rows_buffer("dz%d" % (i & 1), M, self.layout[i][3])
+        key = (M,) + tuple(t.data_ptr() for t in hs + dzs)
+        if self._step_table is None or self._step_table[0] != key:
+            table = ops.ff_layer_table([(w_off, b_off, N, kp, self.acts[i], hs[i] if i < n - 1 else None, dzs[i])
+                                        for i, (w_off, b_off, N, _, kp) in enumerate(self.layout)])
+            nbytes = ops.ff_train_step_workspace_bytes(table, M, self.step_parts)
+            ws = self._buffers.get("step_ws")
+            if ws is None or ws.numel() < nbytes:
+                ws = torch.empty(int(nbytes), dtype=torch.uint8, device=self.device)
+                self._buffers["step_ws"] = ws
+            self._step_table = (key, table, ws)
+        _, table, ws = self._step_table
+        return ops.ff_train_step(table, self.params, self.grads, x, target, row_valid, n_valid_global, ws,
+                                 parts=self.step_parts, grid=self.step_grid)
 
     def _loss_and_backward(self, x, target, row_valid, n_valid_global, reduce_group, reduce):
         M = x.shape[0]
         n = len(self.layout)
-        if self.acts[-1] in (None, ops.ACT_NONE) and n > 1:
+        if self._fused_output():
             hs = self.forward(x, n_layers=n - 1)
             loss, dz = ops.linear_fwd_mse(hs[-1], self.weight_padded(n - 1), self.bias(n - 1), target,
                                           row_valid, n_valid_global,
diff --git a/idiaptts_amd/ops.py b/idiaptts_amd/ops.py
--- a/idiaptts_amd/ops.py
+++ b/idiaptts_amd/ops.py
@@ -720,6 +720,40 @@
     return dw, db, dx
 
 
+def ff_layer_table(layers):
+    table = (_lib.FFLayer * len(layers))()
+    for e, (w_off, b_off, N, K, act, h, dz) in zip(table, layers):
+        e.w_off, e.b_off, e.N, e.K, e.act = w_off, b_off, N, K, int(act if act is not None else ACT_NONE)
+        e.h, e.ldh = (h.data_ptr(), _rows(h, "h")) if h is not None else (None, 0)
+        e.dz, e.lddz = dz.data_ptr(), _rows(dz, "dz")
+    return table
+
+
+def ff_train_step_workspace_bytes(table, M, parts=0):
+    return _lib.load().itts_ff_train_step_workspace_bytes(ctypes.addressof(table), len(table), M, parts)
+
+
+def ff_train_step(table, params, grads, x, target, row_valid, n_valid, workspace, parts=0, grid=0):
+    _need(x, torch.float32, "x")
+    _need(target, torch.float32, "target")
+    _need(row_valid, torch.uint8, "row_valid")
+    M = x.shape[0]
+    if target.shape[0] != M or row_valid.numel() != M or not row_valid.is_contiguous():
+        raise ValueError("x, target and row_valid must have the same number of rows")
+    loss = torch.empty((1,), dtype=torch.float32, device=x.device)
+    _lib.check(_lib.load().itts_ff_train_step(ctypes.addressof(table), len(table), _ptr(params), _ptr(grads), _ptr(x),
+                                              _rows(x, "x"), _ptr(target), _rows(target, "target"), _ptr(row_valid),
+                                              M, float(n_valid), _ptr(loss), _ptr(workspace), workspace.numel(),
+                                              int(parts), int(grid), _stream()), "itts_ff_train_step")
+    return loss
+
+
+def ff_step_counts():
+    out = (ctypes.c_int64 * 2)()
+    _lib.check(_lib.load().itts_ff_step_counts(out), "itts_ff_step_counts")
+    return {"one_range": out[0], "two_ranges": out[1]}
+
+
 def masked_mse(pred, target, row_valid, n_valid, loss_weight=1.0, want_grad=True, grad=None):
     L = _lib.load()
     _need(pred, torch.float32, "pred")
diff --git a/include/idiaptts_amd.h b/include/idiaptts_amd.h
--- a/include/idiaptts_amd.h
+++ b/include/idiaptts_amd.h
@@ -183,6 +183,22 @@
                     int64_t ldyp, int act_prev, int64_t M, int N, int K, void* d_workspace,
                     int accumulate, void* stream);
 
+typedef struct itts_ff_layer {
+  int64_t w_off, b_off;
+  int N, K;
+  int act, reserved;
+  float* h;
+  int64_t ldh;
+  float* dz;
+  int64_t lddz;
+} itts_ff_layer;
+int64_t itts_ff_train_step_workspace_bytes(const itts_ff_layer* layers, int n_layers, int64_t M, int parts);
+int itts_ff_train_step(const itts_ff_layer* layers, int n_layers, const float* d_params, float* d_grads,
+                       const float* d_x, int64_t ldx, const float* d_target, int64_t ldt,
+                       const uint8_t* d_row_valid, int64_t M, double n_valid, float* d_loss,
+                       void* d_workspace, int64_t workspace_bytes, int parts, int grid, void* stream);
+int itts_ff_step_counts(int64_t out[2]);
+
 int itts_conv1d_fwd(const float* d_x, int64_t ldx, const float* d_w, const float* d_b, float* d_y,
                     int64_t ldy, int B, int T_in, int Cin, int Cout, int Kw, int pad, int dil,
                     int batch_first, int act, void* stream);
```

After: 38.44 million. Within noise of the previous version (-0.4%).
